# ClashLuke/LocAtE

Measured on AMD Instinct MI355X. Metric: images/sec (G+D step) 64x64 bs=64, higher is better.
Workload: dtype f32 (contractions fp32-faithful on the matrix cores: 2 x scaled fp16 operand pieces / 3 MFMAs per slice where the operand's largest magnitude comes with it, else 3 x bf16 pieces / 6 MFMAs; fp32 accumulate); 1 GPU; LocAtE G+D step, 64x64 RGB, batch 64 per GPU (the fp32 variant - the reference's own precision - of BASELINE.json configs[1]: 64x64 RGB bs 64), self/feature attention at 16x16 and 64x64, random-init weights; global_batch=64, image_size=64, parallelism=dp1, launch=hipGraph replay, G-step generator pass on a second stream

## Files before the change

### include/locate_hip.h

```cpp
#ifndef LOCATE_HIP_H
#define LOCATE_HIP_H
#include <stddef.h>
#include <stdint.h>
#ifdef __cplusplus
extern "C" {
#endif

const char* locate_last_error(void);
int locate_abi_version(void);
int locate_device_info(char* arch_name, int name_len, int* cu_count, int* wave_size);

int locate_roottanh_fwd(const float* x, float* y, int64_t n, void* absmax , void* stream);
int locate_absmax_words(void);
int locate_roottanh_bwd(const float* x, const float* gy, float* gx, int64_t n, int accumulate, void* absmax, void* stream);
int locate_absmax(const float* x, int64_t n, void* absmax, void* stream);
int locate_act_cat_rows_fwd(const float* latent, const float* pre, float* out, int rows, int z, int w, void* stream);
int locate_act_rows_bwd(const float* pre, const float* g, int64_t g_row_stride, const float* g_add, float* gpre, int rows, int w,
                        void* stream);
int locate_add3(const float* a, int64_t a_bs, const float* b, int64_t b_bs, const float* c, int64_t c_bs, float* out, int batch,
                int64_t per, void* stream);
int locate_tanh_fwd(const float* x, float* y, int64_t n, void* stream);
int locate_tanh_bwd(const float* y, const float* gy, float* gx, int64_t n, void* stream);

size_t locate_norm_stats_workspace_bytes(void);
int locate_norm_stats(const float* x, int64_t n, float* stats, void* workspace, void* stream);
int locate_norm_fwd(const float* x, const float* scale, int scale_per_sample, const float* bias, float* out, int with_act,
                    float* stats_out, int B, int C, int hw, int groups, void* workspace, const double* pre_partial,
                    void* absmax , void* stream);
size_t locate_norm_bwd_workspace_bytes(int B, int C);
int locate_norm_bwd(const float* x, const float* g, const float* stats, const float* scale, int scale_per_sample,
                    const float* bias, int with_act, float* dx, float* dscale, float* dbias, int B, int C, int hw, int groups,
                    void* workspace, int accumulate_dx, void* stream);
size_t locate_norm_bwd_fused_workspace_bytes(int B, int C);
size_t locate_norm_bwd_fused_plane_offset(void);
int locate_norm_bwd_fused(const float* x, const float* g, const float* stats, const float* scale, int scale_per_sample,
                          const float* bias, int with_act, float* dx, float* dscale_sample, int B, int C, int hw, int groups,
                          void* workspace, int accumulate_dx, void* stream);
int locate_norm_bwd_fused_partials(int B, int C);
int locate_norm_bwd_planes(const float* x, const float* g, const float* stats, const float* scale, int scale_per_sample,
                           const float* bias, int with_act, float* dscale_sample, int B, int C, int hw, int groups,
                           void* workspace, void* stream);
int locate_fin_norm_channels(const void* records, int n, void* stream);
size_t locate_channel_sum_workspace_bytes(int B, int C, int hw);
int locate_channel_sum(const float* g, float* out, int B, int C, int hw, int64_t batch_stride, void* workspace, void* stream);

int locate_gate_fwd(const float* x, const float* a, int a_per_plane, const float* gamma, float* out, int64_t planes, int hw,
                    void* stream);
int locate_gate_fwd_stats(const float* x, const float* a, int a_per_plane, const float* gamma, float* out, int64_t planes,
                          int hw, int groups, double* stats_partial, void* stream);
size_t locate_gate_bwd_workspace_bytes(int64_t planes);
int locate_gate_bwd_partials(int64_t planes, int hw);
int locate_gate_bwd(const float* x, const float* a, int a_per_plane, const float* gamma, const float* g, float* dx, float* da,
                    float* dgamma, int64_t planes, int hw, void* workspace, int accumulate_dx,
                    void* da_absmax , void* stream);
enum { LOCATE_GATE_TERM_NONE = 0, LOCATE_GATE_TERM_NORM = 1, LOCATE_GATE_TERM_ROOTTANH = 2 };
typedef struct {
    int32_t kind, with_act, per_sample, has_share;
    const float* go;
    const float* stats;
    const float* scale;
    const float* bias;
    const double* partial;
    int32_t npartial, B, C, groups;
} LocateGateTerm;
int locate_gate_bwd_term(const float* x, const float* a, int a_per_plane, const float* gamma, const float* g, float* dx, float* da,
                         float* dgamma, int64_t planes, int hw, void* workspace, int accumulate_dx, void* da_absmax,
                         LocateGateTerm term, void* stream);

int locate_softmax_fwd(const float* x, float* y, int64_t rows, int n, void* stream);
int locate_softmax_bwd(const float* y, const float* gy, float* gx, int64_t rows, int n, void* stream);

int locate_upsample2x_fwd(const float* x, float* y, int64_t planes, int H, int W, void* stream);
int locate_upsample2x_bwd(const float* gy, float* gx, int64_t planes, int H, int W, void* stream);
int locate_pool2_upsample2x_fwd(const float* x, float* y, int64_t planes, int H, int W, void* stream);
int locate_pool2_upsample2x_bwd(const float* gy, float* gx, int64_t planes, int H, int W, int accumulate, void* stream);
int locate_avgpool2_fwd(const float* x, float* y, int64_t planes, int H, int W, void* stream);
int locate_avgpool2_bwd(const float* gy, float* gx, int64_t planes, int H, int W, int accumulate, void* stream);
int locate_feature_pool_fwd(const float* x, float* y, int64_t n_out, int r, void* stream);
int locate_feature_pool_bwd(const float* gy, float* gx, int64_t n_out, int r, int accumulate, void* stream);
int locate_copy_channels(const float* src, float* dst, int B, int C, int hw, int64_t src_batch_stride,
                         int64_t dst_batch_stride, int accumulate, void* stream);

size_t locate_sn_workspace_bytes(int h, int wd);
int locate_sn_power_iter(const float* w, float* u, float* v, float* sigma, float* wv, int h, int wd, void* workspace,
                         void* stream);
size_t locate_sn_table_record_bytes(void);
int locate_sn_power_iter_batched(const void* table, int n_layers, int max_h, int max_wd, void* stream);
int locate_sn_weight_bwd(const double* inner_partial, int n_partial, const float* u, const float* v, const float* sigma,
                         const float* wv, float* gw, float* du, float* dsigma_out, int h, int wd, void* stream);
size_t locate_sn_group_workspace_bytes(void);
int locate_sn_weight_bwd_grouped(const float* gy, int64_t gy_bs, const float* y, int64_t y_bs, const float* bias, int groups,
                                 int Bg, int M, int plane, const float* sigma_tab, int sigma_stride, const float* u,
                                 const float* v, const float* wv, int64_t wv_stride, float* gw, float* du,
                                 float* dsigma_total_out, int h, int wd, void* workspace, void* stream);
int locate_sn_dv_batched(const void* table, int n_layers, int max_h, int max_wd, void* stream);

size_t locate_conv_panel_bytes(const int* geom, int adjoint);
int locate_conv_pack_panel(const int* geom, int adjoint, const float* w, float* panel, void* stream);
size_t locate_conv_pack_job_bytes(void);
int locate_conv_pack_job(const int* geom, int adjoint, const float* w, float* panel, int block_start, void* job_out,
                         int* blocks_out, int direct, const void* weight_absmax);
int locate_conv_pack_panels(const void* jobs, int n_jobs, int total_blocks, int any_f16, int passes, void* stream);
int locate_conv_pack_job_is_direct(const void* job);
int locate_conv_pack_job_is_window(const void* job);
int locate_conv_win_ok(const int* geom, int adjoint_fmt, int64_t x_bs, const void* x);
size_t locate_conv_win_workspace_bytes(const int* geom, int adjoint_fmt);
size_t locate_conv_fwd_workspace_bytes(const int* geom);
size_t locate_conv_counter_bytes(void);
int locate_conv_fwd(const int* geom, const float* x, int64_t x_bs, const float* panel, const float* scale,
                    int scale_group_batch, int scale_stride, const float* bias, float* y, int64_t y_bs, void* workspace,
                    void* counters, int precision, const void* x_absmax, const void* act_epilogue, void* stream);
size_t locate_conv_dgrad_workspace_bytes(const int* geom);
int locate_conv_dgrad(const int* geom, const float* gy, int64_t gy_bs, const float* panel, const float* scale,
                      int scale_group_batch, int scale_stride, const float* bias, float* gx, int64_t gx_bs, void* workspace,
                      void* counters, int precision, const void* gy_absmax, const void* act_epilogue, void* stream);
size_t locate_conv_wgrad_workspace_bytes(const int* geom);
int locate_conv_wgrad_partials(const int* geom);
int locate_conv_wgrad(const int* geom, const float* x, int64_t x_bs, const float* gy, int64_t gy_bs, float* gw,
                      const float* w_ref, const float* inv_scale, int scale_group_batch, int scale_stride,
                      double* inner_partial, void* workspace, int precision, const void* x_absmax, const void* gy_absmax,
                      void* deferred_reduce, void* stream);
int locate_conv_wgrad_group_partials(const int* geom, int groups);
size_t locate_conv_wgrad_group_workspace_bytes(const int* geom, int groups);
size_t locate_slab_reduce_record_bytes(void);
int locate_slab_reduce_max(void);
int locate_slab_reduce_record_blocks(const void* record);
int locate_slab_reduce_batch(const void* records, int n, void* stream);

size_t locate_wgrad_batch_record_bytes(void);
int locate_wgrad_batch_max(void);
int locate_wgrad_batch_record(const int* geom, const float* x, int64_t x_bs, const float* gy, int64_t gy_bs, float* gw,
                              const float* w_ref, const float* inv_scale, int scale_group_batch, int scale_stride,
                              double* inner_partial, void* record);
int locate_wgrad_batch(const void* records, int n, void* stream);

int locate_dwconv_fwd(const int* geom, const float* x, int64_t x_bs, const float* w, const float* scale, int scale_group_batch,
                      int scale_stride, float* y, int64_t y_bs, void* stream);
int locate_dwconv_dgrad(const int* geom, const float* gy, int64_t gy_bs, const float* w, const float* scale,
                        int scale_group_batch, int scale_stride, float* gx, int64_t gx_bs, void* stream);
size_t locate_dwconv_wgrad_workspace_bytes(const int* geom);
int locate_dwconv_wgrad_partials(const int* geom);
int locate_dwconv_wgrad(const int* geom, const float* big, int64_t big_bs, const float* small, int64_t small_bs, float* gw,
                        const float* w_ref, const float* inv_scale, int scale_group_batch, int scale_stride,
                        double* inner_partial, void* workspace, void* stream);
int locate_groupdot_fwd(const float* x, int64_t x_bs, const float* w, const float* scale, int scale_group_batch,
                        int scale_stride, float* y, int B, int G, int L, void* stream);
int locate_groupdot_dgrad(const float* gy, const float* w, const float* scale, int scale_group_batch, int scale_stride,
                          float* gx, int64_t gx_bs, int B, int G, int L, void* stream);
int locate_groupdot_wgrad_partials(int G, int L);
int locate_groupdot_wgrad(const float* x, int64_t x_bs, const float* gy, float* gw, const float* w_ref, const float* inv_scale,
                          int scale_group_batch, int scale_stride, double* inner_partial, int B, int G, int L, void* stream);

size_t locate_fin_record_bytes(void);
int locate_fin_sn_dot_partials(int Bg, int M, int plane);
int locate_fin_sn_dots(const void* records, int n, void* stream);
int locate_fin_sn_rank1(const void* records, int n, void* stream);
int locate_fin_sums(const void* records, int n, void* stream);
int locate_fin_channel_slices(int B, int C, int hw);
int locate_fin_channel_sums(const void* records, int n, void* stream);

size_t locate_multi_copy_record_bytes(void);
int locate_multi_copy_chunk_elems(void);
int locate_multi_copy(const void* tensors, const void* chunks, int n_chunks, int direction, float scale, void* stream);

size_t locate_nadam_tensor_record_bytes(void);
int locate_nadam_chunk_elems(void);
int locate_nadam_step(const void* tensors, void* coef, const void* chunks, int n_tensors, int n_chunks, double lr, double beta1,
                      double beta2, double eps, double schedule_decay, double weight_decay, void* stream);

size_t locate_average_record_bytes(void);
int locate_average_chunk_elems(void);
int locate_average_update(const void* tensors, const void* chunks, int n_tensors, int n_chunks, void* stream);

size_t locate_stats_tensor_record_bytes(void);
size_t locate_stats_record_bytes(void);
int locate_stats_chunk_elems(void);
int locate_stats_max_blocks(void);
size_t locate_stats_workspace_bytes(int n_chunks);
int locate_stats_reduce(const void* tensors, const void* chunks, int n_tensors, int n_chunks, void* records, void* summary,
                        void* workspace, void* stream);

size_t locate_guard_tensor_record_bytes(void);
size_t locate_guard_verdict_bytes(void);
int locate_guard_chunk_elems(void);
int locate_guard_max_blocks(void);
size_t locate_guard_workspace_bytes(int n_chunks);
int locate_guarded_nadam_step(const void* grads, const void* grad_chunks, int n_grads, int n_grad_chunks, void* workspace, void* verdict,
                              double max_norm, int skip_nonfinite, const void* tensors, void* coef, const void* chunks, int n_tensors,
                              int n_chunks, double lr, double beta1, double beta2, double eps, double schedule_decay, double weight_decay,
                              void* stream);

size_t locate_snapshot_record_bytes(void);
size_t locate_snapshot_commit_bytes(void);
int locate_snapshot_chunk_elems(void);
int locate_snapshot_take(const void* records, const void* chunks, int n_tensors, int n_chunks, void* slot0, void* slot1, void* commit,
                         long long iteration, void* stream);
int locate_snapshot_restore(const void* records, const void* chunks, int n_tensors, int n_chunks, const void* slot, void* stream);

size_t locate_digest_record_bytes(void);
int locate_digest_chunk_elems(void);
int locate_digest(const void* records, const void* chunks, const void* first, int n_tensors, int n_chunks, void* partials, void* out,
                  void* stream);

size_t locate_dyn_tensor_record_bytes(void);
size_t locate_dyn_record_bytes(void);
int locate_dyn_chunk_elems(void);
int locate_dyn_max_blocks(void);
size_t locate_dyn_workspace_bytes(int n_chunks);
int locate_dyn_pass(const void* tensors, const void* chunks, int n_tensors, int n_chunks, int mode, void* records, void* workspace,
                    void* stream);

int locate_formats_count(void);
const char* locate_formats_name(int i);
int locate_formats_max_views(void);
size_t locate_formats_view_record_bytes(void);
size_t locate_formats_base_record_bytes(void);
size_t locate_formats_format_record_bytes(void);
size_t locate_formats_workspace_bytes(const void* host_views, int n_views);
int locate_formats_audit(const void* host_views, int n_views, const int* row_slots, void* rows, void* workspace, void* stream);

int locate_d_loss(const float* d_true, const float* d_fake, const float* d_aug, int B, float gamma, float* losses,
                  float* g_true, float* g_fake, float* g_aug, void* stream);
int locate_g_loss(const float* d_fake, int B, float* loss, float* g_fake, void* stream);

size_t locate_input_param_record_bytes(void);
int locate_input_mean_blocks(int H, int W);
size_t locate_input_workspace_bytes(int n, int H, int W);
int locate_input_transform(const void* store, int N, int H, int W, const int32_t* idx, const void* params, int n, int n_first,
                           const int32_t* coef, int side_lo, int side_hi, int ktaps, const float* lut, int S, float* out_first,
                           float* out_rest, void* workspace, void* stream);

size_t locate_image_range_workspace_bytes(void);
int locate_image_range(const float* x, int64_t n_elems, float* range, void* workspace, void* stream);
int locate_image_grid(const float* x, int n, int S, int nrow, int padding, float pad_value, const float* range, float divisor,
                      float* grid_f32, uint8_t* grid_u8, void* stream);

int locate_pyr_down(const float* x, int planes, int S, float* out, void* stream);
int locate_pyr_residual(const float* x, const float* coarse, int planes, int S, float* out, void* stream);
size_t locate_swd_stats_workspace_bytes(void);
int locate_swd_stats(const float* level, int N, int S, const int32_t* pos, int P, float* stats, void* workspace, void* stream);
int locate_swd_project(const float* level, int N, int S, const int32_t* pos, int P, const float* dirs, int D, const float* stats,
                       float* proj, void* stream);
size_t locate_swd_distance_workspace_bytes(void);
int locate_swd_distance(const float* a, const float* b, int64_t count, float* out, void* workspace, void* stream);

int locate_nn_row_bytes(int S);
int locate_nn_encode(const float* x, int n, int S, int8_t* codes, int64_t* norms, int32_t* nonfinite, void* stream);
size_t locate_nn_search_workspace_bytes(int Q, int N, int k);
int locate_nn_search(const int8_t* qcodes, const int64_t* qnorms, const int32_t* qflags, int Q, const int8_t* rcodes, const int64_t* rnorms,
                     const int32_t* rflags, int N, int row_bytes, const int32_t* skip, int k, int64_t* d2, int32_t* index, void* workspace,
                     void* stream);

size_t locate_nn_within_workspace_bytes(int Q, int N, int want_covered);
int locate_nn_within(const int8_t* qcodes, const int64_t* qnorms, const int32_t* qflags, int Q, const int8_t* rcodes, const int64_t* rnorms,
                     const int32_t* rflags, int N, int row_bytes, const int64_t* radius2, const int32_t* skip, int32_t* hits, int32_t* covered,
                     void* workspace, void* stream);

size_t locate_nn_group_sums_workspace_bytes(int M, int K, int row_bytes);
int locate_nn_group_sums(const int8_t* codes, int N, int row_bytes, const int32_t* order, int M, const int32_t* starts, int K,
                         int32_t* sums, void* workspace, void* stream);
int locate_nn_centroids(const int32_t* sums, const int32_t* starts, int K, int M, int row_bytes, const int8_t* previous,
                        int8_t* codes, int64_t* norms, int32_t* moved, void* stream);

size_t locate_spectrum_workspace_bytes(int planes, int S);
int locate_spectrum_planes(const float* x, int planes, int S, const float* cos_table, const float* sin_table, const int32_t* slot,
                           const int32_t* start, int R, double* spectra, void* workspace, void* stream);
size_t locate_spectrum_summary_workspace_bytes(int planes);
int locate_spectrum_summary(const double* spectra, int n, int channels, int R, const double* count, double* sums, int32_t* nonfinite,
                            void* workspace, void* stream);

size_t locate_msssim_workspace_bytes(int pairs, int S);
int locate_msssim_pairs(const int8_t* a, const int32_t* aflags, const int8_t* b, const int32_t* bflags, int pairs, int row_bytes, int S,
                        const double* taps, double* out, void* workspace, void* stream);

#ifdef __cplusplus
}
#endif
#endif
```

### locate_amd/_lib.py

```python
import ctypes
import os

import torch

_HERE = os.path.dirname(os.path.abspath(__file__))
LIB_PATH = os.path.join(_HERE, "csrc", "liblocate_hip_dbg.so" if os.environ.get("LOCATE_HIP_DEBUG_LIBRARY") == "1"
                        else "liblocate_hip.so")

c_p = ctypes.c_void_p
c_i = ctypes.c_int
c_i64 = ctypes.c_int64
c_f = ctypes.c_float
c_d = ctypes.c_double
c_sz = ctypes.c_size_t
c_ip = ctypes.POINTER(ctypes.c_int)


class GateTerm(ctypes.Structure):
    NONE, NORM, ROOTTANH = 0, 1, 2
    _fields_ = [("kind", ctypes.c_int32), ("with_act", ctypes.c_int32), ("per_sample", ctypes.c_int32), ("has_share", ctypes.c_int32),
                ("go", c_p), ("stats", c_p), ("scale", c_p), ("bias", c_p), ("partial", c_p),
                ("npartial", ctypes.c_int32), ("B", ctypes.c_int32), ("C", ctypes.c_int32), ("groups", ctypes.c_int32)]


PROTOTYPES = {
    "locate_last_error": (ctypes.c_char_p, []),
    "locate_abi_version": (c_i, []),
    "locate_device_info": (c_i, [ctypes.c_char_p, c_i, c_ip, c_ip]),
    "locate_roottanh_fwd": (c_i, [c_p, c_p, c_i64, c_p, c_p]),
    "locate_roottanh_bwd": (c_i, [c_p, c_p, c_p, c_i64, c_i, c_p, c_p]),
    "locate_act_cat_rows_fwd": (c_i, [c_p, c_p, c_p, c_i, c_i, c_i, c_p]),
    "locate_act_rows_bwd": (c_i, [c_p, c_p, c_i64, c_p, c_p, c_i, c_i, c_p]),
    "locate_add3": (c_i, [c_p, c_i64, c_p, c_i64, c_p, c_i64, c_p, c_i, c_i64, c_p]),
    "locate_absmax_words": (c_i, []),
    "locate_wgrad_batch_record_bytes": (c_sz, []),
    "locate_wgrad_batch_max": (c_i, []),
    "locate_wgrad_batch_record": (c_i, [c_ip, c_p, c_i64, c_p, c_i64, c_p, c_p, c_p, c_i, c_i, c_p, c_p]),
    "locate_wgrad_batch": (c_i, [c_p, c_i, c_p]),
    "locate_absmax": (c_i, [c_p, c_i64, c_p, c_p]),
    "locate_tanh_fwd": (c_i, [c_p, c_p, c_i64, c_p]),
    "locate_tanh_bwd": (c_i, [c_p, c_p, c_p, c_i64, c_p]),
    "locate_norm_stats_workspace_bytes": (c_sz, []),
    "locate_norm_stats": (c_i, [c_p, c_i64, c_p, c_p, c_p]),
    "locate_norm_bwd_workspace_bytes": (c_sz, [c_i, c_i]),
    "locate_norm_fwd": (c_i, [c_p, c_p, c_i, c_p, c_p, c_i, c_p, c_i, c_i, c_i, c_i, c_p, c_p, c_p, c_p]),
    "locate_norm_bwd": (c_i, [c_p, c_p, c_p, c_p, c_i, c_p, c_i, c_p, c_p, c_p, c_i, c_i, c_i, c_i, c_p, c_i, c_p]),
    "locate_norm_bwd_fused_workspace_bytes": (c_sz, [c_i, c_i]),
    "locate_norm_bwd_fused_plane_offset": (c_sz, []),
    "locate_norm_bwd_fused": (c_i, [c_p, c_p, c_p, c_p, c_i, c_p, c_i, c_p, c_p, c_i, c_i, c_i, c_i, c_p, c_i, c_p]),
    "locate_norm_bwd_fused_partials": (c_i, [c_i, c_i]),
    "locate_norm_bwd_planes": (c_i, [c_p, c_p, c_p, c_p, c_i, c_p, c_i, c_p, c_i, c_i, c_i, c_i, c_p, c_p]),
    "locate_fin_norm_channels": (c_i, [c_p, c_i, c_p]),
    "locate_channel_sum_workspace_bytes": (c_sz, [c_i, c_i, c_i]),
    "locate_channel_sum": (c_i, [c_p, c_p, c_i, c_i, c_i, c_i64, c_p, c_p]),
    "locate_gate_fwd": (c_i, [c_p, c_p, c_i, c_p, c_p, c_i64, c_i, c_p]),
    "locate_gate_fwd_stats": (c_i, [c_p, c_p, c_i, c_p, c_p, c_i64, c_i, c_i, c_p, c_p]),
    "locate_gate_bwd_workspace_bytes": (c_sz, [c_i64]),
    "locate_gate_bwd": (c_i, [c_p, c_p, c_i, c_p, c_p, c_p, c_p, c_p, c_i64, c_i, c_p, c_i, c_p, c_p]),
    "locate_gate_bwd_term": (c_i, [c_p, c_p, c_i, c_p, c_p, c_p, c_p, c_p, c_i64, c_i, c_p, c_i, c_p, GateTerm, c_p]),
    "locate_softmax_fwd": (c_i, [c_p, c_p, c_i64, c_i, c_p]),
    "locate_softmax_bwd": (c_i, [c_p, c_p, c_p, c_i64, c_i, c_p]),
    "locate_upsample2x_fwd": (c_i, [c_p, c_p, c_i64, c_i, c_i, c_p]),
    "locate_upsample2x_bwd": (c_i, [c_p, c_p, c_i64, c_i, c_i, c_p]),
    "locate_pool2_upsample2x_fwd": (c_i, [c_p, c_p, c_i64, c_i, c_i, c_p]),
    "locate_pool2_upsample2x_bwd": (c_i, [c_p, c_p, c_i64, c_i, c_i, c_i, c_p]),
    "locate_avgpool2_fwd": (c_i, [c_p, c_p, c_i64, c_i, c_i, c_p]),
    "locate_avgpool2_bwd": (c_i, [c_p, c_p, c_i64, c_i, c_i, c_i, c_p]),
    "locate_feature_pool_fwd": (c_i, [c_p, c_p, c_i64, c_i, c_p]),
    "locate_feature_pool_bwd": (c_i, [c_p, c_p, c_i64, c_i, c_i, c_p]),
    "locate_copy_channels": (c_i, [c_p, c_p, c_i, c_i, c_i, c_i64, c_i64, c_i, c_p]),
    "locate_sn_workspace_bytes": (c_sz, [c_i, c_i]),
    "locate_sn_power_iter": (c_i, [c_p, c_p, c_p, c_p, c_p, c_i, c_i, c_p, c_p]),
    "locate_sn_table_record_bytes": (c_sz, []),
    "locate_sn_power_iter_batched": (c_i, [c_p, c_i, c_i, c_i, c_p]),
    "locate_sn_weight_bwd": (c_i, [c_p, c_i, c_p, c_p, c_p, c_p, c_p, c_p, c_p, c_i, c_i, c_p]),
    "locate_sn_group_workspace_bytes": (c_sz, []),
    "locate_sn_weight_bwd_grouped": (c_i, [c_p, c_i64, c_p, c_i64, c_p, c_i, c_i, c_i, c_i, c_p, c_i, c_p, c_p, c_p, c_i64, c_p,
                                           c_p, c_p, c_i, c_i, c_p, c_p]),
    "locate_sn_dv_batched": (c_i, [c_p, c_i, c_i, c_i, c_p]),
    "locate_conv_panel_bytes": (c_sz, [c_ip, c_i]),
    "locate_conv_pack_panel": (c_i, [c_ip, c_i, c_p, c_p, c_p]),
    "locate_conv_pack_job_bytes": (c_sz, []),
    "locate_conv_pack_job": (c_i, [c_ip, c_i, c_p, c_p, c_i, c_p, c_ip, c_i, c_p]),
    "locate_conv_pack_panels": (c_i, [c_p, c_i, c_i, c_i, c_i, c_p]),
    "locate_conv_pack_job_is_direct": (c_i, [c_p]),
    "locate_conv_pack_job_is_window": (c_i, [c_p]),
    "locate_conv_win_ok": (c_i, [c_ip, c_i, c_i64, c_p]),
    "locate_conv_win_workspace_bytes": (c_sz, [c_ip, c_i]),
    "locate_conv_fwd_workspace_bytes": (c_sz, [c_ip]),
    "locate_conv_counter_bytes": (c_sz, []),
    "locate_conv_fwd": (c_i, [c_ip, c_p, c_i64, c_p, c_p, c_i, c_i, c_p, c_p, c_i64, c_p, c_p, c_i, c_p, c_p, c_p]),
    "locate_conv_dgrad_workspace_bytes": (c_sz, [c_ip]),
    "locate_conv_dgrad": (c_i, [c_ip, c_p, c_i64, c_p, c_p, c_i, c_i, c_p, c_p, c_i64, c_p, c_p, c_i, c_p, c_p, c_p]),
    "locate_conv_wgrad_workspace_bytes": (c_sz, [c_ip]),
    "locate_conv_wgrad_partials": (c_i, [c_ip]),
    "locate_conv_wgrad": (c_i, [c_ip, c_p, c_i64, c_p, c_i64, c_p, c_p, c_p, c_i, c_i, c_p, c_p, c_i, c_p, c_p, c_p, c_p]),
    "locate_conv_wgrad_group_partials": (c_i, [c_ip, c_i]),
    "locate_conv_wgrad_group_workspace_bytes": (c_sz, [c_ip, c_i]),
    "locate_slab_reduce_record_bytes": (c_sz, []),
    "locate_slab_reduce_max": (c_i, []),
    "locate_slab_reduce_record_blocks": (c_i, [c_p]),
    "locate_slab_reduce_batch": (c_i, [c_p, c_i, c_p]),
    "locate_dwconv_fwd": (c_i, [c_ip, c_p, c_i64, c_p, c_p, c_i, c_i, c_p, c_i64, c_p]),
    "locate_dwconv_dgrad": (c_i, [c_ip, c_p, c_i64, c_p, c_p, c_i, c_i, c_p, c_i64, c_p]),
    "locate_dwconv_wgrad_workspace_bytes": (c_sz, [c_ip]),
    "locate_dwconv_wgrad_partials": (c_i, [c_ip]),
    "locate_dwconv_wgrad": (c_i, [c_ip, c_p, c_i64, c_p, c_i64, c_p, c_p, c_p, c_i, c_i, c_p, c_p, c_p]),
    "locate_groupdot_fwd": (c_i, [c_p, c_i64, c_p, c_p, c_i, c_i, c_p, c_i, c_i, c_i, c_p]),
    "locate_groupdot_dgrad": (c_i, [c_p, c_p, c_p, c_i, c_i, c_p, c_i64, c_i, c_i, c_i, c_p]),
    "locate_groupdot_wgrad_partials": (c_i, [c_i, c_i]),
    "locate_groupdot_wgrad": (c_i, [c_p, c_i64, c_p, c_p, c_p, c_p, c_i, c_i, c_p, c_i, c_i, c_i, c_p]),
    "locate_fin_record_bytes": (c_sz, []),
    "locate_fin_sn_dot_partials": (c_i, [c_i, c_i, c_i]),
    "locate_fin_sn_dots": (c_i, [c_p, c_i, c_p]),
    "locate_fin_sn_rank1": (c_i, [c_p, c_i, c_p]),
    "locate_fin_sums": (c_i, [c_p, c_i, c_p]),
    "locate_fin_channel_slices": (c_i, [c_i, c_i, c_i]),
    "locate_fin_channel_sums": (c_i, [c_p, c_i, c_p]),
    "locate_gate_bwd_partials": (c_i, [c_i64, c_i]),
    "locate_multi_copy_record_bytes": (c_sz, []),
    "locate_multi_copy_chunk_elems": (c_i, []),
    "locate_multi_copy": (c_i, [c_p, c_p, c_i, c_i, c_f, c_p]),
    "locate_nadam_tensor_record_bytes": (c_sz, []),
    "locate_nadam_chunk_elems": (c_i, []),
    "locate_nadam_step": (c_i, [c_p, c_p, c_p, c_i, c_i, c_d, c_d, c_d, c_d, c_d, c_d, c_p]),
    "locate_average_record_bytes": (c_sz, []),
    "locate_average_chunk_elems": (c_i, []),
    "locate_average_update": (c_i, [c_p, c_p, c_i, c_i, c_p]),
    "locate_stats_tensor_record_bytes": (c_sz, []),
    "locate_stats_record_bytes": (c_sz, []),
    "locate_stats_chunk_elems": (c_i, []),
    "locate_stats_max_blocks": (c_i, []),
    "locate_stats_workspace_bytes": (c_sz, [c_i]),
    "locate_stats_reduce": (c_i, [c_p, c_p, c_i, c_i, c_p, c_p, c_p, c_p]),
    "locate_guard_tensor_record_bytes": (c_sz, []),
    "locate_guard_verdict_bytes": (c_sz, []),
    "locate_guard_chunk_elems": (c_i, []),
    "locate_guard_max_blocks": (c_i, []),
    "locate_guard_workspace_bytes": (c_sz, [c_i]),
    "locate_guarded_nadam_step": (c_i, [c_p, c_p, c_i, c_i, c_p, c_p, c_d, c_i, c_p, c_p, c_p, c_i, c_i, c_d, c_d, c_d, c_d, c_d, c_d, c_p]),
    "locate_snapshot_record_bytes": (c_sz, []),
    "locate_snapshot_commit_bytes": (c_sz, []),
    "locate_snapshot_chunk_elems": (c_i, []),
    "locate_snapshot_take": (c_i, [c_p, c_p, c_i, c_i, c_p, c_p, c_p, c_i64, c_p]),
    "locate_snapshot_restore": (c_i, [c_p, c_p, c_i, c_i, c_p, c_p]),
    "locate_digest_record_bytes": (c_sz, []),
    "locate_digest_chunk_elems": (c_i, []),
    "locate_digest": (c_i, [c_p, c_p, c_p, c_i, c_i, c_p, c_p, c_p]),
    "locate_dyn_tensor_record_bytes": (c_sz, []),
    "locate_dyn_record_bytes": (c_sz, []),
    "locate_dyn_chunk_elems": (c_i, []),
    "locate_dyn_max_blocks": (c_i, []),
    "locate_dyn_workspace_bytes": (c_sz, [c_i]),
    "locate_dyn_pass": (c_i, [c_p, c_p, c_i, c_i, c_i, c_p, c_p, c_p]),
    "locate_formats_count": (c_i, []),
    "locate_formats_name": (ctypes.c_char_p, [c_i]),
    "locate_formats_max_views": (c_i, []),
    "locate_formats_view_record_bytes": (c_sz, []),
    "locate_formats_base_record_bytes": (c_sz, []),
    "locate_formats_format_record_bytes": (c_sz, []),
    "locate_formats_workspace_bytes": (c_sz, [c_p, c_i]),
    "locate_formats_audit": (c_i, [c_p, c_i, c_p, c_p, c_p, c_p]),
    "locate_d_loss": (c_i, [c_p, c_p, c_p, c_i, c_f, c_p, c_p, c_p, c_p, c_p]),
    "locate_g_loss": (c_i, [c_p, c_i, c_p, c_p, c_p]),
    "locate_input_param_record_bytes": (c_sz, []),
    "locate_input_mean_blocks": (c_i, [c_i, c_i]),
    "locate_input_workspace_bytes": (c_sz, [c_i, c_i, c_i]),
    "locate_input_transform": (c_i, [c_p, c_i, c_i, c_i, c_p, c_p, c_i, c_i, c_p, c_i, c_i, c_i, c_p, c_i, c_p, c_p, c_p, c_p]),
    "locate_image_range_workspace_bytes": (c_sz, []),
    "locate_image_range": (c_i, [c_p, c_i64, c_p, c_p, c_p]),
    "locate_image_grid": (c_i, [c_p, c_i, c_i, c_i, c_i, c_f, c_p, c_f, c_p, c_p, c_p]),
    "locate_pyr_down": (c_i, [c_p, c_i, c_i, c_p, c_p]),
    "locate_pyr_residual": (c_i, [c_p, c_p, c_i, c_i, c_p, c_p]),
    "locate_swd_stats_workspace_bytes": (c_sz, []),
    "locate_swd_stats": (c_i, [c_p, c_i, c_i, c_p, c_i, c_p, c_p, c_p]),
    "locate_swd_project": (c_i, [c_p, c_i, c_i, c_p, c_i, c_p, c_i, c_p, c_p, c_p]),
    "locate_swd_distance_workspace_bytes": (c_sz, []),
    "locate_swd_distance": (c_i, [c_p, c_p, c_i64, c_p, c_p, c_p]),
    "locate_spectrum_workspace_bytes": (c_sz, [c_i, c_i]),
    "locate_spectrum_planes": (c_i, [c_p, c_i, c_i, c_p, c_p, c_p, c_p, c_i, c_p, c_p, c_p]),
    "locate_spectrum_summary_workspace_bytes": (c_sz, [c_i]),
    "locate_spectrum_summary": (c_i, [c_p, c_i, c_i, c_i, c_p, c_p, c_p, c_p, c_p]),
    "locate_msssim_workspace_bytes": (c_sz, [c_i, c_i]),
    "locate_msssim_pairs": (c_i, [c_p, c_p, c_p, c_p, c_i, c_i, c_i, c_p, c_p, c_p, c_p]),
    "locate_nn_row_bytes": (c_i, [c_i]),
    "locate_nn_encode": (c_i, [c_p, c_i, c_i, c_p, c_p, c_p, c_p]),
    "locate_nn_search_workspace_bytes": (c_sz, [c_i, c_i, c_i]),
    "locate_nn_search": (c_i, [c_p, c_p, c_p, c_i, c_p, c_p, c_p, c_i, c_i, c_p, c_i, c_p, c_p, c_p, c_p]),
    "locate_nn_within_workspace_bytes": (c_sz, [c_i, c_i, c_i]),
    "locate_nn_within": (c_i, [c_p, c_p, c_p, c_i, c_p, c_p, c_p, c_i, c_i, c_p, c_p, c_p, c_p, c_p, c_p]),
    "locate_nn_group_sums_workspace_bytes": (c_sz, [c_i, c_i, c_i]),
    "locate_nn_group_sums": (c_i, [c_p, c_i, c_i, c_p, c_i, c_p, c_i, c_p, c_p, c_p]),
    "locate_nn_centroids": (c_i, [c_p, c_p, c_i, c_i, c_i, c_p, c_p, c_p, c_p, c_p]),
}


class LocateError(RuntimeError):
    pass


EXPECTED_ABI = 21


_lib = None


def lib():
    global _lib
    if _lib is None:
        if not os.path.exists(LIB_PATH):
            raise LocateError("%s is missing: run `python -m locate_amd.build` (hipcc, gfx950). "
                              "There is no CPU fallback for the MI355X kernels." % LIB_PATH)
        handle = ctypes.CDLL(LIB_PATH)
        for name, (res, args) in PROTOTYPES.items():
            fn = getattr(handle, name)
            fn.restype = res
            fn.argtypes = args
        got = handle.locate_abi_version()
        if got != EXPECTED_ABI:
            raise LocateError("%s reports ABI version %d, this package binds version %d: rebuild it (`python -m locate_amd.build`)"
                              % (LIB_PATH, got, EXPECTED_ABI))
        _lib = handle
    return _lib


def check(status, what=""):
    if status != 0:
        msg = lib().locate_last_error()
        raise LocateError("%s failed (status %d): %s" % (what, status, msg.decode() if msg else "?"))


def require_gpu():
    if not torch.cuda.is_available():
        raise LocateError("no HIP device: locate_amd computes only on MI355X (gfx950); there is no CPU path")
    name = ctypes.create_string_buffer(64)
    cu, wave = ctypes.c_int(0), ctypes.c_int(0)
    check(lib().locate_device_info(name, 64, ctypes.byref(cu), ctypes.byref(wave)), "locate_device_info")
    arch = name.value.decode()
    if not arch.startswith("gfx950"):
        raise LocateError("device architecture %r: the kernels are built for gfx950 only" % arch)
    return arch, cu.value, wave.value
```

### locate_amd/csrc/elementwise.hip

```cpp
#include "common.h"
#include "normterm.h"

template <int OP>
__global__ void __launch_bounds__(256) unary_fwd_kernel(const float* __restrict__ x, float* __restrict__ y, int64_t n,
                                                        unsigned* __restrict__ absmax) {
    __shared__ float amax_scratch[16];
    float am = 0.0f;
    const int64_t n4 = n >> 2;
    const int64_t stride = (int64_t)gridDim.x * blockDim.x;
    const float4* x4 = reinterpret_cast<const float4*>(x);
    float4* y4 = reinterpret_cast<float4*>(y);
    for (int64_t i = (int64_t)blockIdx.x * blockDim.x + threadIdx.x; i < n4; i += stride) {
        float4 v = x4[i], o;
        if (OP == 0) {
            o.x = roottanh_f(v.x); o.y = roottanh_f(v.y); o.z = roottanh_f(v.z); o.w = roottanh_f(v.w);
        } else {
            o.x = tanhf(v.x); o.y = tanhf(v.y); o.z = tanhf(v.z); o.w = tanhf(v.w);
        }
        y4[i] = o;
        am = fmaxf(fmaxf(am, fmaxf(fabsf(o.x), fabsf(o.y))), fmaxf(fabsf(o.z), fabsf(o.w)));
    }
    for (int64_t i = (n4 << 2) + (int64_t)blockIdx.x * blockDim.x + threadIdx.x; i < n; i += stride) {
        const float o = OP == 0 ? roottanh_f(x[i]) : tanhf(x[i]);
        y[i] = o;
        am = fmaxf(am, fabsf(o));
    }
    if (absmax) absmax_publish(am, amax_scratch, absmax);
}

template <int OP>
__global__ void __launch_bounds__(256) unary_bwd_kernel(const float* __restrict__ a, const float* __restrict__ g,
                                                        float* __restrict__ gx, int64_t n, int accumulate,
                                                        unsigned* __restrict__ absmax) {
    __shared__ float amax_scratch[16];
    float am = 0.0f;
    const int64_t n4 = n >> 2;
    const int64_t stride = (int64_t)gridDim.x * blockDim.x;
    const float4* a4 = reinterpret_cast<const float4*>(a);
    const float4* g4 = reinterpret_cast<const float4*>(g);
    float4* o4 = reinterpret_cast<float4*>(gx);
    for (int64_t i = (int64_t)blockIdx.x * blockDim.x + threadIdx.x; i < n4; i += stride) {
        float4 v = a4[i], w = g4[i], o;
        if (OP == 0) {
            o.x = roottanh_grad_f(v.x, w.x); o.y = roottanh_grad_f(v.y, w.y);
            o.z = roottanh_grad_f(v.z, w.z); o.w = roottanh_grad_f(v.w, w.w);
        } else {
            o.x = w.x * (1.0f - v.x * v.x); o.y = w.y * (1.0f - v.y * v.y);
            o.z = w.z * (1.0f - v.z * v.z); o.w = w.w * (1.0f - v.w * v.w);
        }
        if (accumulate) {
            const float4 c = o4[i];
            o.x += c.x; o.y += c.y; o.z += c.z; o.w += c.w;
        }
        o4[i] = o;
        am = fmaxf(fmaxf(am, fmaxf(fabsf(o.x), fabsf(o.y))), fmaxf(fabsf(o.z), fabsf(o.w)));
    }
    for (int64_t i = (n4 << 2) + (int64_t)blockIdx.x * blockDim.x + threadIdx.x; i < n; i += stride) {
        float o = OP == 0 ? roottanh_grad_f(a[i], g[i]) : g[i] * (1.0f - a[i] * a[i]);
        o = accumulate ? gx[i] + o : o;
        gx[i] = o;
        am = fmaxf(am, fabsf(o));
    }
    if (absmax) absmax_publish(am, amax_scratch, absmax);
}

static bool aligned16(const void* p) { return (reinterpret_cast<uintptr_t>(p) & 15) == 0; }

LOCATE_API int locate_roottanh_fwd(const float* x, float* y, int64_t n, void* absmax, void* stream) {
    LOCATE_REQUIRE(n >= 0 && aligned16(x) && aligned16(y), "locate_roottanh_fwd: bad size or unaligned pointer");
    if (n == 0) return LOCATE_OK;
    unary_fwd_kernel<0><<<stream_grid(n, 1024), 256, 0, as_stream(stream)>>>(x, y, n, static_cast<unsigned*>(absmax));
    LOCATE_LAUNCH_CHECK("locate_roottanh_fwd");
    return LOCATE_OK;
}

LOCATE_API int locate_roottanh_bwd(const float* x, const float* gy, float* gx, int64_t n, int accumulate, void* absmax, void* stream) {
    LOCATE_REQUIRE(n >= 0 && aligned16(x) && aligned16(gy) && aligned16(gx), "locate_roottanh_bwd: bad size or unaligned pointer");
    if (n == 0) return LOCATE_OK;
    unary_bwd_kernel<0><<<stream_grid(n, 1024), 256, 0, as_stream(stream)>>>(x, gy, gx, n, accumulate, static_cast<unsigned*>(absmax));
    LOCATE_LAUNCH_CHECK("locate_roottanh_bwd");
    return LOCATE_OK;
}

__global__ void __launch_bounds__(256) act_cat_rows_kernel(const float* __restrict__ latent, const float* __restrict__ pre,
                                                           float* __restrict__ out, int rows, int z, int w) {
    const int total = rows * (z + w);
    for (int i = blockIdx.x * blockDim.x + threadIdx.x; i < total; i += gridDim.x * blockDim.x) {
        const int r = i / (z + w), c = i - r * (z + w);
        out[i] = c < z ? latent[r * z + c] : roottanh_f(pre[r * w + (c - z)]);
    }
}

__global__ void __launch_bounds__(256) act_rows_bwd_kernel(const float* __restrict__ pre, const float* __restrict__ g, int g_rs,
                                                           const float* __restrict__ g_add, float* __restrict__ gpre, int rows, int w) {
    const int total = rows * w;
    for (int i = blockIdx.x * blockDim.x + threadIdx.x; i < total; i += gridDim.x * blockDim.x) {
        const int r = i / w, j = i - r * w;
        const float v = roottanh_grad_f(pre[i], g[(int64_t)r * g_rs + j]);
        gpre[i] = g_add ? __fadd_rn(g_add[i], v) : v;
    }
}

LOCATE_API int locate_act_cat_rows_fwd(const float* latent, const float* pre, float* out, int rows, int z, int w, void* stream) {
    LOCATE_REQUIRE(latent && pre && out && rows > 0 && z >= 0 && w > 0 && (int64_t)rows * (z + w) < (1ll << 31), "locate_act_cat_rows_fwd: bad arguments");
    act_cat_rows_kernel<<<stream_grid((int64_t)rows * (z + w), 256), 256, 0, as_stream(stream)>>>(latent, pre, out, rows, z, w);
    LOCATE_LAUNCH_CHECK("locate_act_cat_rows_fwd");
    return LOCATE_OK;
}

LOCATE_API int locate_act_rows_bwd(const float* pre, const float* g, int64_t g_row_stride, const float* g_add, float* gpre, int rows,
                                   int w, void* stream) {
    LOCATE_REQUIRE(pre && g && gpre && rows > 0 && w > 0 && g_row_stride >= w && g_row_stride < (1ll << 31), "locate_act_rows_bwd: bad arguments");
    act_rows_bwd_kernel<<<stream_grid((int64_t)rows * w, 256), 256, 0, as_stream(stream)>>>(pre, g, (int)g_row_stride, g_add, gpre, rows, w);
    LOCATE_LAUNCH_CHECK("locate_act_rows_bwd");
    return LOCATE_OK;
}

template <bool VEC>
__global__ void __launch_bounds__(256) add3_kernel(const float* __restrict__ a, long long a_bs, const float* __restrict__ b, long long b_bs,
                                                   const float* __restrict__ c, long long c_bs, float* __restrict__ out, unsigned per,
                                                   long long total) {
    const DivU32 dv(per);
    const long long stride = (long long)gridDim.x * blockDim.x;
    for (long long i = (long long)blockIdx.x * blockDim.x + threadIdx.x; i < total; i += stride) {
        unsigned q, r;
        dv.divmod((unsigned)i, q, r);
        if constexpr (VEC) {
            const float4 x = *reinterpret_cast<const float4*>(a + q * a_bs + 4ll * r);
            const float4 y = *reinterpret_cast<const float4*>(b + q * b_bs + 4ll * r);
            const float4 z = *reinterpret_cast<const float4*>(c + q * c_bs + 4ll * r);
            float4 o;
            o.x = __fadd_rn(__fadd_rn(x.x, y.x), z.x); o.y = __fadd_rn(__fadd_rn(x.y, y.y), z.y);
            o.z = __fadd_rn(__fadd_rn(x.z, y.z), z.z); o.w = __fadd_rn(__fadd_rn(x.w, y.w), z.w);
            *reinterpret_cast<float4*>(out + 4ll * i) = o;
        } else {
            out[i] = __fadd_rn(__fadd_rn(a[q * a_bs + r], b[q * b_bs + r]), c[q * c_bs + r]);
        }
    }
}

LOCATE_API int locate_add3(const float* a, int64_t a_bs, const float* b, int64_t b_bs, const float* c, int64_t c_bs, float* out, int batch,
                           int64_t per, void* stream) {
    LOCATE_REQUIRE(a && b && c && out && batch > 0 && per > 0 && a_bs >= per && b_bs >= per && c_bs >= per &&
                   (int64_t)batch * per < (1ll << 32), "locate_add3: bad arguments");
    const bool vec = (per & 3) == 0 && ((a_bs | b_bs | c_bs) & 3) == 0 && aligned16(a) && aligned16(b) && aligned16(c) && aligned16(out);
    if (vec) {
        const int64_t total = (int64_t)batch * (per / 4);
        add3_kernel<true><<<stream_grid(total, 2048), 256, 0, as_stream(stream)>>>(a, a_bs, b, b_bs, c, c_bs, out, (unsigned)(per / 4), total);
    } else {
        const int64_t total = (int64_t)batch * per;
        add3_kernel<false><<<stream_grid(total, 2048), 256, 0, as_stream(stream)>>>(a, a_bs, b, b_bs, c, c_bs, out, (unsigned)per, total);
    }
    LOCATE_LAUNCH_CHECK("locate_add3");
    return LOCATE_OK;
}

LOCATE_API int locate_absmax_words(void) { return AMAX_WORDS; }

__global__ void __launch_bounds__(256) absmax_kernel(const float* __restrict__ x, int64_t n, unsigned* __restrict__ slot) {
    __shared__ float scratch[16];
    float m = 0.0f;
    const int64_t stride = (int64_t)gridDim.x * blockDim.x;
    for (int64_t i = (int64_t)blockIdx.x * blockDim.x + threadIdx.x; i < n; i += stride) m = fmaxf(m, fabsf(x[i]));
    absmax_publish(m, scratch, slot);
}

LOCATE_API int locate_absmax(const float* x, int64_t n, void* slot, void* stream) {
    LOCATE_REQUIRE(x && slot && n > 0, "locate_absmax: bad arguments");
    absmax_kernel<<<stream_grid(n, 2048), 256, 0, as_stream(stream)>>>(x, n, static_cast<unsigned*>(slot));
    LOCATE_LAUNCH_CHECK("locate_absmax");
    return LOCATE_OK;
}

LOCATE_API int locate_tanh_fwd(const float* x, float* y, int64_t n, void* stream) {
    LOCATE_REQUIRE(n >= 0 && aligned16(x) && aligned16(y), "locate_tanh_fwd: bad size or unaligned pointer");
    if (n == 0) return LOCATE_OK;
    unary_fwd_kernel<1><<<stream_grid(n, 1024), 256, 0, as_stream(stream)>>>(x, y, n, nullptr);
    LOCATE_LAUNCH_CHECK("locate_tanh_fwd");
    return LOCATE_OK;
}

LOCATE_API int locate_tanh_bwd(const float* y, const float* gy, float* gx, int64_t n, void* stream) {
    LOCATE_REQUIRE(n >= 0 && aligned16(y) && aligned16(gy) && aligned16(gx), "locate_tanh_bwd: bad size or unaligned pointer");
    if (n == 0) return LOCATE_OK;
    unary_bwd_kernel<1><<<stream_grid(n, 1024), 256, 0, as_stream(stream)>>>(y, gy, gx, n, 0, nullptr);
    LOCATE_LAUNCH_CHECK("locate_tanh_bwd");
    return LOCATE_OK;
}

__global__ void __launch_bounds__(256) gate_fwd_kernel(const float* __restrict__ x, const float* __restrict__ a,
                                                       const float* __restrict__ gamma, float* __restrict__ out,
                                                       int64_t n, int hw, int a_per_plane) {
    const float gm = gamma[0];
    const int64_t stride = (int64_t)gridDim.x * blockDim.x;
    if (!a_per_plane && (n & 3) == 0) {
        const float4* x4 = reinterpret_cast<const float4*>(x);
        const float4* a4 = reinterpret_cast<const float4*>(a);
        float4* o4 = reinterpret_cast<float4*>(out);
        for (int64_t i = (int64_t)blockIdx.x * blockDim.x + threadIdx.x; i < (n >> 2); i += stride) {
            float4 xv = x4[i], av = a4[i], o;
            o.x = fmaf(gm, av.x, 1.0f) * xv.x; o.y = fmaf(gm, av.y, 1.0f) * xv.y;
            o.z = fmaf(gm, av.z, 1.0f) * xv.z; o.w = fmaf(gm, av.w, 1.0f) * xv.w;
            o4[i] = o;
        }
        return;
    }
    if (a_per_plane && (hw & 3) == 0) {
        const float4* x4 = reinterpret_cast<const float4*>(x);
        float4* o4 = reinterpret_cast<float4*>(out);
        const unsigned hw4 = (unsigned)(hw >> 2);
        for (int64_t i = (int64_t)blockIdx.x * blockDim.x + threadIdx.x; i < (n >> 2); i += stride) {
            const float m = fmaf(gm, a[(unsigned)i / hw4], 1.0f);
            const float4 xv = x4[i];
            o4[i] = make_float4(m * xv.x, m * xv.y, m * xv.z, m * xv.w);
        }
        return;
    }
    const DivU32 dhw((unsigned)hw);
    for (int64_t i = (int64_t)blockIdx.x * blockDim.x + threadIdx.x; i < n; i += stride) {
        const float av = a_per_plane ? a[dhw.div((unsigned)i)] : a[i];
        out[i] = fmaf(gm, av, 1.0f) * x[i];
    }
}

__global__ void __launch_bounds__(256) gate_fwd_stats_kernel(const float* __restrict__ x, const float* __restrict__ a,
                                                             const float* __restrict__ gamma, float* __restrict__ out,
                                                             int64_t n_group, int hw, int a_per_plane,
                                                             double* __restrict__ partial) {
    __shared__ double scratch[16];
    const float gm = gamma[0];
    const int64_t g0 = (int64_t)blockIdx.y * n_group;
    x += g0; out += g0;
    if (!a_per_plane) a += g0;
    partial += (int64_t)blockIdx.y * 2 * gridDim.x;
    const int64_t stride = (int64_t)gridDim.x * blockDim.x;
    double s = 0.0, q = 0.0;
    if (!a_per_plane && (n_group & 3) == 0) {
        const float4* x4 = reinterpret_cast<const float4*>(x);
        const float4* a4 = reinterpret_cast<const float4*>(a);
        float4* o4 = reinterpret_cast<float4*>(out);
        for (int64_t i = (int64_t)blockIdx.x * blockDim.x + threadIdx.x; i < (n_group >> 2); i += stride) {
            float4 xv = x4[i], av = a4[i], o;
            o.x = fmaf(gm, av.x, 1.0f) * xv.x; o.y = fmaf(gm, av.y, 1.0f) * xv.y;
            o.z = fmaf(gm, av.z, 1.0f) * xv.z; o.w = fmaf(gm, av.w, 1.0f) * xv.w;
            o4[i] = o;
            const double a_ = o.x, b_ = o.y, c_ = o.z, d_ = o.w;
            s += (a_ + b_) + (c_ + d_);
            q += (a_ * a_ + b_ * b_) + (c_ * c_ + d_ * d_);
        }
    } else if (a_per_plane && (hw & 3) == 0 && (n_group & 3) == 0 && n_group < (1ll << 33)) {
        const float4* x4 = reinterpret_cast<const float4*>(x);
        float4* o4 = reinterpret_cast<float4*>(out);
        const unsigned hw4 = (unsigned)(hw >> 2);
        const float* ap = a + g0 / hw;
        for (int64_t i = (int64_t)blockIdx.x * blockDim.x + threadIdx.x; i < (n_group >> 2); i += stride) {
            const float m = fmaf(gm, ap[(unsigned)i / hw4], 1.0f);
            const float4 xv = x4[i];
            float4 o;
            o.x = m * xv.x; o.y = m * xv.y; o.z = m * xv.z; o.w = m * xv.w;
            o4[i] = o;
            const double a_ = o.x, b_ = o.y, c_ = o.z, d_ = o.w;
            s += (a_ + b_) + (c_ + d_);
            q += (a_ * a_ + b_ * b_) + (c_ * c_ + d_ * d_);
        }
    } else {
        const DivU32 dhw((unsigned)hw);
        for (int64_t i = (int64_t)blockIdx.x * blockDim.x + threadIdx.x; i < n_group; i += stride) {
            const float av = a_per_plane ? a[dhw.div((unsigned)(g0 + i))] : a[i];
            const float o = fmaf(gm, av, 1.0f) * x[i];
            out[i] = o;
            s += (double)o;
            q += (double)o * (double)o;
        }
    }
    s = block_sum<double>(s, scratch);
    q = block_sum<double>(q, scratch);
    if (threadIdx.x == 0) {
        partial[2 * blockIdx.x] = s;
        partial[2 * blockIdx.x + 1] = q;
    }
}

__device__ __noinline__ float gate_plane_da_nonfinite(const float* __restrict__ x, const float* __restrict__ g, int hw, float gm) {
    float s = 0.0f;
    for (int i = 0; i < hw; ++i) s += (x[i] * g[i]) * gm;
    return s;
}
__device__ __forceinline__ bool gate_gamma_finite(float gm) { return fabsf(gm) <= 3.402823466e38f; }

constexpr bool gate_term_is_norm(int term) { return term == GATE_TERM_NORM || term == GATE_TERM_NORM_ACT; }

struct GateTermPlane { float mu, inv_s, y, b, k, m; };

template <int TERM>
__device__ __forceinline__ GateTermPlane gate_term_plane(const LocateGateTerm& t, const float (*tc)[2], unsigned p, unsigned planes_g) {
    GateTermPlane tp = {0.0f, 1.0f, 0.0f, 0.0f, 0.0f, 0.0f};
    if constexpr (gate_term_is_norm(TERM)) {
        const unsigned grp = p / planes_g, c = p % (unsigned)t.C;
        tp.mu = t.stats[2 * grp];
        tp.inv_s = 1.0f / t.stats[2 * grp + 1];
        tp.y = t.scale[t.per_sample ? p : c];
        tp.b = TERM == GATE_TERM_NORM_ACT ? t.bias[c] : 0.0f;
        tp.m = tc[grp][0];
        tp.k = tc[grp][1];
    }
    return tp;
}

__device__ __forceinline__ float gate_mul_g_first(float g, float m) {
    float r;
    asm("v_mul_f32 %0, %1, %2" : "=v"(r) : "v"(g), "v"(m));
    return r;
}

template <int TERM>
__device__ __forceinline__ float gate_term_g(const GateTermPlane& tp, float out, float gin, float share, int has_share) {
    if constexpr (TERM == GATE_TERM_ROOTTANH) return roottanh_grad_f(out, gin);
    const float o = norm_dx<TERM == GATE_TERM_NORM_ACT>(out, gin, tp.mu, tp.inv_s, tp.y, tp.b, tp.k, tp.m);
    return has_share ? o + share : o;
}

template <int TERM>
__device__ __forceinline__ void gate_term_consts(const LocateGateTerm& t, int64_t n_group, float (*tc)[2]) {
    if constexpr (gate_term_is_norm(TERM)) {
        const int wid = threadIdx.x >> 6;
        if (wid < t.groups) norm_group_consts(t.partial, t.npartial, wid, t.stats[2 * wid + 1], n_group, (int)(threadIdx.x & 63), tc[wid]);
        __syncthreads();
    }
}

template <int TERM>
__device__ __noinline__ float gate_plane_da_nonfinite_term(const float* __restrict__ x, const float* __restrict__ gs,
                                                           const float* __restrict__ share, int hw, float gm, float ap,
                                                           GateTermPlane tp, int has_share) {
    float s = 0.0f;
    const float mv = fmaf(gm, ap, 1.0f);
    for (int i = 0; i < hw; ++i) {
        const float g = gate_term_g<TERM>(tp, mul_pinned(mv, x[i]), gs[i], has_share ? share[i] : 0.0f, has_share);
        s += (x[i] * g) * gm;
    }
    return s;
}

template <int WPP, int TERM, bool ELEM = false>
__global__ void __launch_bounds__(256) gate_bwd_plane_kernel(const float* __restrict__ x, const float* __restrict__ a,
                                                             const float* __restrict__ gamma, const float* __restrict__ g,
                                                             float* __restrict__ dx, float* __restrict__ da_full,
                                                             float* __restrict__ da_plane, double* __restrict__ block_x2g,
                                                             int64_t planes, int hw, int a_per_plane, int accumulate_dx,
                                                             unsigned* __restrict__ da_absmax, const LocateGateTerm t) {
    __shared__ double wsum[4], px2g[4];
    __shared__ float pxg[4];
    __shared__ float amax_scratch[16];
    __shared__ float tc[NORM_MAX_GROUPS][2];
    float am = 0.0f;
    double wacc = 0.0;
    const float gm = gamma[0];
    const int lane = threadIdx.x & 63, wid = threadIdx.x >> 6;
    const int sub = WPP == 1 ? lane : (int)threadIdx.x;
    const int nsub = WPP == 1 ? 64 : 256;
    const int64_t first = WPP == 1 ? (((int64_t)blockIdx.x * blockDim.x + threadIdx.x) >> 6) : (int64_t)blockIdx.x;
    const int64_t step = WPP == 1 ? (((int64_t)gridDim.x * blockDim.x) >> 6) : (int64_t)gridDim.x;
    const float* __restrict__ gs = gate_term_is_norm(TERM) ? t.go : g;
    constexpr bool elem = ELEM;
    const unsigned planes_g = gate_term_is_norm(TERM) ? (unsigned)((int64_t)t.B * t.C / t.groups) : 1u;
    const int has_share = gate_term_is_norm(TERM) ? t.has_share : 0;
    if constexpr (gate_term_is_norm(TERM)) gate_term_consts<TERM>(t, (int64_t)planes_g * (elem ? 1 : hw), tc);
    bool vec = (hw & 3) == 0 && ((reinterpret_cast<uintptr_t>(x) | reinterpret_cast<uintptr_t>(g) | reinterpret_cast<uintptr_t>(dx) |
                                  (a_per_plane ? 0 : (reinterpret_cast<uintptr_t>(a) | reinterpret_cast<uintptr_t>(da_full)))) & 15) == 0;
    if constexpr (gate_term_is_norm(TERM)) vec = vec && (reinterpret_cast<uintptr_t>(gs) & 15) == 0;
    for (int64_t p = first; p < planes; p += step) {
        const int64_t base = p * hw;
        const float ap = a_per_plane ? a[p] : 0.0f;
        float sxg = 0.0f, sx2g = 0.0f;
        GateTermPlane tp = {0.0f, 1.0f, 0.0f, 0.0f, 0.0f, 0.0f};
        if constexpr (gate_term_is_norm(TERM))
            if (!elem) tp = gate_term_plane<TERM>(t, tc, (unsigned)p, planes_g);
        if (vec) {
            for (int i = sub; i < (hw >> 2); i += nsub) {
                const float4 xv = reinterpret_cast<const float4*>(x + base)[i];
                float4 gv = reinterpret_cast<const float4*>(gs + base)[i];
                float4 av = make_float4(ap, ap, ap, ap);
                if (!a_per_plane) av = reinterpret_cast<const float4*>(a + base)[i];
                if constexpr (TERM != GATE_TERM_NONE) {
                    const float4 ov = make_float4(mul_pinned(fmaf(gm, av.x, 1.0f), xv.x), mul_pinned(fmaf(gm, av.y, 1.0f), xv.y),
                                                  mul_pinned(fmaf(gm, av.z, 1.0f), xv.z), mul_pinned(fmaf(gm, av.w, 1.0f), xv.w));
                    float4 sh = make_float4(0.0f, 0.0f, 0.0f, 0.0f);
                    if (has_share) sh = reinterpret_cast<const float4*>(g + base)[i];
                    if (elem) {
                        const unsigned e = (unsigned)(base + 4 * i);
                        gv.x = gate_term_g<TERM>(gate_term_plane<TERM>(t, tc, e, planes_g), ov.x, gv.x, sh.x, has_share);
                        gv.y = gate_term_g<TERM>(gate_term_plane<TERM>(t, tc, e + 1, planes_g), ov.y, gv.y, sh.y, has_share);
                        gv.z = gate_term_g<TERM>(gate_term_plane<TERM>(t, tc, e + 2, planes_g), ov.z, gv.z, sh.z, has_share);
                        gv.w = gate_term_g<TERM>(gate_term_plane<TERM>(t, tc, e + 3, planes_g), ov.w, gv.w, sh.w, has_share);
                    } else {
                        gv.x = gate_term_g<TERM>(tp, ov.x, gv.x, sh.x, has_share); gv.y = gate_term_g<TERM>(tp, ov.y, gv.y, sh.y, has_share);
                        gv.z = gate_term_g<TERM>(tp, ov.z, gv.z, sh.z, has_share); gv.w = gate_term_g<TERM>(tp, ov.w, gv.w, sh.w, has_share);
                    }
                }
                const float4 xg = make_float4(xv.x * gv.x, xv.y * gv.y, xv.z * gv.z, xv.w * gv.w);
                float4 o = make_float4(fmaf(gm, av.x, 1.0f) * gv.x, fmaf(gm, av.y, 1.0f) * gv.y, fmaf(gm, av.z, 1.0f) * gv.z,
                                       fmaf(gm, av.w, 1.0f) * gv.w);
                if constexpr (TERM != GATE_TERM_NONE)
                    o = make_float4(gate_mul_g_first(gv.x, fmaf(gm, av.x, 1.0f)), gate_mul_g_first(gv.y, fmaf(gm, av.y, 1.0f)),
                                    gate_mul_g_first(gv.z, fmaf(gm, av.z, 1.0f)), gate_mul_g_first(gv.w, fmaf(gm, av.w, 1.0f)));
                if (accumulate_dx) {
                    const float4 old = reinterpret_cast<const float4*>(dx + base)[i];
                    o.x += old.x; o.y += old.y; o.z += old.z; o.w += old.w;
                }
                reinterpret_cast<float4*>(dx + base)[i] = o;
                if (!a_per_plane) {
                    const float4 dav = make_float4(xg.x * gm, xg.y * gm, xg.z * gm, xg.w * gm);
                    reinterpret_cast<float4*>(da_full + base)[i] = dav;
                    am = fmaxf(fmaxf(am, fmaxf(fabsf(dav.x), fabsf(dav.y))), fmaxf(fabsf(dav.z), fabsf(dav.w)));
                }
                sxg += (xg.x + xg.y) + (xg.z + xg.w);
                sx2g += (xg.x * xv.x + xg.y * xv.y) + (xg.z * xv.z + xg.w * xv.w);
            }
        } else {
            for (int i = sub; i < hw; i += nsub) {
                const float xv = x[base + i];
                float gv = gs[base + i];
                const float av = a_per_plane ? ap : a[base + i];
                if constexpr (TERM != GATE_TERM_NONE) {
                    if (elem) tp = gate_term_plane<TERM>(t, tc, (unsigned)(base + i), planes_g);
                    gv = gate_term_g<TERM>(tp, mul_pinned(fmaf(gm, av, 1.0f), xv), gv, has_share ? g[base + i] : 0.0f, has_share);
                }
                const float xg = xv * gv;
                float o = fmaf(gm, av, 1.0f) * gv;
                if constexpr (TERM != GATE_TERM_NONE) o = gate_mul_g_first(gv, fmaf(gm, av, 1.0f));
                dx[base + i] = accumulate_dx ? dx[base + i] + o : o;
                if (!a_per_plane) { da_full[base + i] = xg * gm; am = fmaxf(am, fabsf(xg * gm)); }
                sxg += xg;
                sx2g = fmaf(xg, xv, sx2g);
            }
        }
        sxg = wave_sum(sxg);
        const double s2 = wave_sum_d((double)sx2g);
        if (WPP == 1) {
            wacc += s2;
            if (lane == 0 && a_per_plane) {
                if (gate_gamma_finite(gm)) da_plane[p] = gm * sxg;
                else if constexpr (TERM == GATE_TERM_NONE) da_plane[p] = gate_plane_da_nonfinite(x + base, g + base, hw, gm);
                else da_plane[p] = gate_plane_da_nonfinite_term<TERM>(x + base, gs + base, g + base, hw, gm, ap, tp, has_share);
            }
        } else {
            __syncthreads();
            if (lane == 0) { pxg[wid] = sxg; px2g[wid] = s2; }
            __syncthreads();
            if (threadIdx.x == 0) {
                wacc += (px2g[0] + px2g[1]) + (px2g[2] + px2g[3]);
                if (a_per_plane) {
                    if (gate_gamma_finite(gm)) da_plane[p] = gm * ((pxg[0] + pxg[1]) + (pxg[2] + pxg[3]));
                    else if constexpr (TERM == GATE_TERM_NONE) da_plane[p] = gate_plane_da_nonfinite(x + base, g + base, hw, gm);
                    else da_plane[p] = gate_plane_da_nonfinite_term<TERM>(x + base, gs + base, g + base, hw, gm, ap, tp, has_share);
                }
            }
        }
    }
    if (WPP == 1) {
        if (lane == 0) wsum[wid] = wacc;
        __syncthreads();
        if (threadIdx.x == 0) block_x2g[blockIdx.x] = (wsum[0] + wsum[1]) + (wsum[2] + wsum[3]);
    } else if (threadIdx.x == 0) {
        block_x2g[blockIdx.x] = wacc;
    }
    if (da_absmax && !a_per_plane) absmax_publish(am, amax_scratch, da_absmax);
}

template <int LP, int TERM, bool ELEM = false>
__global__ void __launch_bounds__(256) gate_bwd_small_kernel(const float* __restrict__ x, const float* __restrict__ a,
                                                             const float* __restrict__ gamma, const float* __restrict__ g,
                                                             float* __restrict__ dx, float* __restrict__ da_full,
                                                             float* __restrict__ da_plane, double* __restrict__ block_x2g,
                                                             int64_t planes, int hw, int a_per_plane, int accumulate_dx,
                                                             unsigned* __restrict__ da_absmax, const LocateGateTerm t) {
    __shared__ double wsum[4];
    __shared__ float amax_scratch[16];
    __shared__ float tc[NORM_MAX_GROUPS][2];
    constexpr int PW = 64 / LP;
    float am = 0.0f;
    double wacc = 0.0;
    const float gm = gamma[0];
    const int lane = threadIdx.x & 63, wid = threadIdx.x >> 6;
    const int gid = lane / LP, li = lane % LP;
    const int q4 = hw >> 2;
    const int64_t wave = ((int64_t)blockIdx.x * blockDim.x + threadIdx.x) >> 6;
    const int64_t nwaves = ((int64_t)gridDim.x * blockDim.x) >> 6;
    const float* __restrict__ gs = gate_term_is_norm(TERM) ? t.go : g;
    constexpr bool elem = ELEM;
    const unsigned planes_g = gate_term_is_norm(TERM) ? (unsigned)((int64_t)t.B * t.C / t.groups) : 1u;
    const int has_share = gate_term_is_norm(TERM) ? t.has_share : 0;
    if constexpr (gate_term_is_norm(TERM)) gate_term_consts<TERM>(t, (int64_t)planes_g * (elem ? 1 : hw), tc);
    for (int64_t p0 = wave * PW; p0 < planes; p0 += nwaves * PW) {
        const int64_t p = p0 + gid;
        const bool live = p < planes;
        float sxg = 0.0f, sx2g = 0.0f;
        float ap = 0.0f;
        GateTermPlane tp = {0.0f, 1.0f, 0.0f, 0.0f, 0.0f, 0.0f};
        if (live && li < q4) {
            const int64_t base = p * hw;
            ap = a_per_plane ? a[p] : 0.0f;
            const float4 xv = reinterpret_cast<const float4*>(x + base)[li];
            float4 gv = reinterpret_cast<const float4*>(gs + base)[li];
            float4 av = make_float4(ap, ap, ap, ap);
            if (!a_per_plane) av = reinterpret_cast<const float4*>(a + base)[li];
            if constexpr (TERM != GATE_TERM_NONE) {
                const float4 ov = make_float4(mul_pinned(fmaf(gm, av.x, 1.0f), xv.x), mul_pinned(fmaf(gm, av.y, 1.0f), xv.y),
                                              mul_pinned(fmaf(gm, av.z, 1.0f), xv.z), mul_pinned(fmaf(gm, av.w, 1.0f), xv.w));
                float4 sh = make_float4(0.0f, 0.0f, 0.0f, 0.0f);
                if (has_share) sh = reinterpret_cast<const float4*>(g + base)[li];
                if (elem) {
                    const unsigned e = (unsigned)(base + 4 * li);
                    gv.x = gate_term_g<TERM>(gate_term_plane<TERM>(t, tc, e, planes_g), ov.x, gv.x, sh.x, has_share);
                    gv.y = gate_term_g<TERM>(gate_term_plane<TERM>(t, tc, e + 1, planes_g), ov.y, gv.y, sh.y, has_share);
                    gv.z = gate_term_g<TERM>(gate_term_plane<TERM>(t, tc, e + 2, planes_g), ov.z, gv.z, sh.z, has_share);
                    gv.w = gate_term_g<TERM>(gate_term_plane<TERM>(t, tc, e + 3, planes_g), ov.w, gv.w, sh.w, has_share);
                } else {
                    tp = gate_term_plane<TERM>(t, tc, (unsigned)p, planes_g);
                    gv.x = gate_term_g<TERM>(tp, ov.x, gv.x, sh.x, has_share); gv.y = gate_term_g<TERM>(tp, ov.y, gv.y, sh.y, has_share);
                    gv.z = gate_term_g<TERM>(tp, ov.z, gv.z, sh.z, has_share); gv.w = gate_term_g<TERM>(tp, ov.w, gv.w, sh.w, has_share);
                }
            }
            const float4 xg = make_float4(xv.x * gv.x, xv.y * gv.y, xv.z * gv.z, xv.w * gv.w);
            float4 o = make_float4(fmaf(gm, av.x, 1.0f) * gv.x, fmaf(gm, av.y, 1.0f) * gv.y, fmaf(gm, av.z, 1.0f) * gv.z,
                                   fmaf(gm, av.w, 1.0f) * gv.w);
            if constexpr (TERM != GATE_TERM_NONE)
                o = make_float4(gate_mul_g_first(gv.x, fmaf(gm, av.x, 1.0f)), gate_mul_g_first(gv.y, fmaf(gm, av.y, 1.0f)),
                                gate_mul_g_first(gv.z, fmaf(gm, av.z, 1.0f)), gate_mul_g_first(gv.w, fmaf(gm, av.w, 1.0f)));
            if (accumulate_dx) {
                const float4 old = reinterpret_cast<const float4*>(dx + base)[li];
                o.x += old.x; o.y += old.y; o.z += old.z; o.w += old.w;
            }
            reinterpret_cast<float4*>(dx + base)[li] = o;
            if (!a_per_plane) {
                const float4 dav = make_float4(xg.x * gm, xg.y * gm, xg.z * gm, xg.w * gm);
                reinterpret_cast<float4*>(da_full + base)[li] = dav;
                am = fmaxf(fmaxf(am, fmaxf(fabsf(dav.x), fabsf(dav.y))), fmaxf(fabsf(dav.z), fabsf(dav.w)));
            }
            sxg = (xg.x + xg.y) + (xg.z + xg.w);
            sx2g = (xg.x * xv.x + xg.y * xv.y) + (xg.z * xv.z + xg.w * xv.w);
        }
        double s2 = (double)sx2g;
#pragma unroll
        for (int o = LP / 2; o > 0; o >>= 1) {
            sxg += __shfl_xor(sxg, o, 64);
            s2 += __shfl_xor(s2, o, 64);
        }
        if (live && li == 0) {
            wacc += s2;
            if (a_per_plane) {
                if (gate_gamma_finite(gm)) da_plane[p] = gm * sxg;
                else if constexpr (TERM == GATE_TERM_NONE) da_plane[p] = gate_plane_da_nonfinite(x + p * hw, g + p * hw, hw, gm);
                else da_plane[p] = gate_plane_da_nonfinite_term<TERM>(x + p * hw, gs + p * hw, g + p * hw, hw, gm, ap, tp, has_share);
            }
        }
    }
    wacc = wave_sum_d(wacc);
    if (lane == 0) wsum[wid] = wacc;
    __syncthreads();
    if (threadIdx.x == 0) block_x2g[blockIdx.x] = (wsum[0] + wsum[1]) + (wsum[2] + wsum[3]);
    if (da_absmax && !a_per_plane) absmax_publish(am, amax_scratch, da_absmax);
}

__global__ void __launch_bounds__(256) gate_bwd_final_kernel(const double* __restrict__ block_x2g, float* __restrict__ dgamma,
                                                             int nblocks) {
    __shared__ double scratch[16];
    double acc = 0.0;
    for (int i = threadIdx.x; i < nblocks; i += blockDim.x) acc += block_x2g[i];
    acc = block_sum<double>(acc, scratch);
    if (threadIdx.x == 0) dgamma[0] = (float)acc;
}

LOCATE_API int locate_gate_fwd(const float* x, const float* a, int a_per_plane, const float* gamma, float* out,
                               int64_t planes, int hw, void* stream) {
    LOCATE_REQUIRE(planes >= 0 && hw > 0 && planes * hw < (1ll << 31), "locate_gate_fwd: bad shape");
    const int64_t n = planes * hw;
    if (n == 0) return LOCATE_OK;
    gate_fwd_kernel<<<stream_grid(n, 1024), 256, 0, as_stream(stream)>>>(x, a, gamma, out, n, hw, a_per_plane);
    LOCATE_LAUNCH_CHECK("locate_gate_fwd");
    return LOCATE_OK;
}

LOCATE_API int locate_gate_fwd_stats(const float* x, const float* a, int a_per_plane, const float* gamma, float* out,
                                     int64_t planes, int hw, int groups, double* stats_partial, void* stream) {
    LOCATE_REQUIRE(planes > 0 && hw > 0 && planes * hw < (1ll << 31) && stats_partial, "locate_gate_fwd_stats: bad arguments");
    LOCATE_REQUIRE(groups >= 1 && groups <= 4 && planes % groups == 0, "locate_gate_fwd_stats: bad group count");
    const int64_t n_g = planes / groups * hw;
    LOCATE_REQUIRE(n_g > 1 && (groups == 1 || (n_g & 3) == 0), "locate_gate_fwd_stats: group size must be a multiple of 4");
    int np = stream_grid(n_g, 256 * 16);
    if (np > 512) np = 512;
    gate_fwd_stats_kernel<<<dim3(np, groups), 256, 0, as_stream(stream)>>>(x, a, gamma, out, n_g, hw, a_per_plane, stats_partial);
    LOCATE_LAUNCH_CHECK("locate_gate_fwd_stats");
    return LOCATE_OK;
}

LOCATE_API size_t locate_gate_bwd_workspace_bytes(int64_t planes) { (void)planes; return 4096 * sizeof(double); }

static int64_t gate_bwd_blocks(int64_t planes, int hw) {
    int64_t blocks = hw >= 1024 ? planes : cdiv64(planes, 4);
    return blocks > 4096 ? 4096 : blocks;
}
LOCATE_API int locate_gate_bwd_partials(int64_t planes, int hw) { return (int)gate_bwd_blocks(planes, hw); }

template <int TERM>
static void gate_bwd_launch(const float* x, const float* a, int a_per_plane, const float* gamma, const float* g, float* dx, float* da,
                            double* block_x2g, int64_t planes, int hw, int64_t blocks, int accumulate_dx, void* da_absmax,
                            const LocateGateTerm& t, hipStream_t st) {
    const bool whole_block = hw >= 1024;
    uintptr_t bits = reinterpret_cast<uintptr_t>(x) | reinterpret_cast<uintptr_t>(g) | reinterpret_cast<uintptr_t>(dx) |
                     (a_per_plane ? 0 : (reinterpret_cast<uintptr_t>(a) | reinterpret_cast<uintptr_t>(da)));
    if (gate_term_is_norm(TERM)) bits |= reinterpret_cast<uintptr_t>(t.go);
    const bool vec = (hw & 3) == 0 && (bits & 15) == 0;
    if constexpr (gate_term_is_norm(TERM)) {
        if (planes != (int64_t)t.B * t.C) {
            if (vec)
                gate_bwd_small_kernel<16, TERM, true><<<(int)blocks, 256, 0, st>>>(x, a, gamma, g, dx, da, nullptr, block_x2g, planes, hw, 0,
                                                                                  accumulate_dx, static_cast<unsigned*>(da_absmax), t);
            else
                gate_bwd_plane_kernel<1, TERM, true><<<(int)blocks, 256, 0, st>>>(x, a, gamma, g, dx, da, nullptr, block_x2g, planes, hw, 0,
                                                                                 accumulate_dx, static_cast<unsigned*>(da_absmax), t);
            return;
        }
    }
#define GATE_SMALL(LPV) gate_bwd_small_kernel<LPV, TERM><<<(int)blocks, 256, 0, st>>>(x, a, gamma, g, dx, a_per_plane ? nullptr : da, \
        a_per_plane ? da : nullptr, block_x2g, planes, hw, a_per_plane, accumulate_dx, static_cast<unsigned*>(da_absmax), t)
    if (vec && hw <= 128) {
        const int q4 = hw >> 2;
        if (q4 <= 1) GATE_SMALL(1);
        else if (q4 <= 2) GATE_SMALL(2);
        else if (q4 <= 4) GATE_SMALL(4);
        else if (q4 <= 8) GATE_SMALL(8);
        else if (q4 <= 16) GATE_SMALL(16);
        else GATE_SMALL(32);
    } else if (whole_block)
        gate_bwd_plane_kernel<4, TERM><<<(int)blocks, 256, 0, st>>>(x, a, gamma, g, dx, a_per_plane ? nullptr : da,
                                                                   a_per_plane ? da : nullptr, block_x2g, planes, hw,
                                                                   a_per_plane, accumulate_dx, static_cast<unsigned*>(da_absmax), t);
    else
        gate_bwd_plane_kernel<1, TERM><<<(int)blocks, 256, 0, st>>>(x, a, gamma, g, dx, a_per_plane ? nullptr : da,
                                                                   a_per_plane ? da : nullptr, block_x2g, planes, hw,
                                                                   a_per_plane, accumulate_dx, static_cast<unsigned*>(da_absmax), t);
#undef GATE_SMALL
}

LOCATE_API int locate_gate_bwd_term(const float* x, const float* a, int a_per_plane, const float* gamma, const float* g,
                                    float* dx, float* da, float* dgamma, int64_t planes, int hw, void* workspace,
                                    int accumulate_dx, void* da_absmax, LocateGateTerm term, void* stream) {
    LOCATE_REQUIRE(planes > 0 && hw > 0 && workspace, "locate_gate_bwd: bad shape or missing workspace");
    LOCATE_REQUIRE(term.kind == GATE_TERM_NONE || term.kind == GATE_TERM_NORM || term.kind == GATE_TERM_ROOTTANH,
                   "locate_gate_bwd_term: unknown term %d", term.kind);
    if (term.kind == GATE_TERM_NORM) {
        LOCATE_REQUIRE(term.go && term.stats && term.scale && term.partial && term.npartial > 0 && (!term.with_act || term.bias),
                       "locate_gate_bwd_term: the norm term needs go, stats, scale, the plane pass's partials (and the bias with_act)");
        LOCATE_REQUIRE(term.groups >= 1 && term.groups <= NORM_MAX_GROUPS && term.B > 0 && term.C > 0 && term.B % term.groups == 0 &&
                       (int64_t)term.B * term.C == planes && planes * hw < (1ll << 31), "locate_gate_bwd_term: the norm's B x C must be the gate's planes");
        LOCATE_REQUIRE(!term.has_share || g, "locate_gate_bwd_term: has_share needs the share in g");
    } else {
        LOCATE_REQUIRE(g, "locate_gate_bwd_term: missing gradient");
    }
    double* block_x2g = static_cast<double*>(workspace);
    const int64_t blocks = gate_bwd_blocks(planes, hw);
    if (hw == 1 && (planes & 63) == 0) {
        if (a_per_plane) { a_per_plane = 0; da_absmax = nullptr; }
        planes >>= 6; hw = 64;
    }
    hipStream_t st = as_stream(stream);
    if (term.kind == GATE_TERM_NONE)
        gate_bwd_launch<GATE_TERM_NONE>(x, a, a_per_plane, gamma, g, dx, da, block_x2g, planes, hw, blocks, accumulate_dx, da_absmax, term, st);
    else if (term.kind == GATE_TERM_ROOTTANH)
        gate_bwd_launch<GATE_TERM_ROOTTANH>(x, a, a_per_plane, gamma, g, dx, da, block_x2g, planes, hw, blocks, accumulate_dx, da_absmax, term, st);
    else if (term.with_act)
        gate_bwd_launch<GATE_TERM_NORM_ACT>(x, a, a_per_plane, gamma, g, dx, da, block_x2g, planes, hw, blocks, accumulate_dx, da_absmax, term, st);
    else
        gate_bwd_launch<GATE_TERM_NORM>(x, a, a_per_plane, gamma, g, dx, da, block_x2g, planes, hw, blocks, accumulate_dx, da_absmax, term, st);
    LOCATE_LAUNCH_CHECK("locate_gate_bwd(plane)");
    if (!dgamma) return LOCATE_OK;
    gate_bwd_final_kernel<<<1, 256, 0, st>>>(block_x2g, dgamma, (int)blocks);
    LOCATE_LAUNCH_CHECK("locate_gate_bwd(final)");
    return LOCATE_OK;
}

LOCATE_API int locate_gate_bwd(const float* x, const float* a, int a_per_plane, const float* gamma, const float* g,
                               float* dx, float* da, float* dgamma, int64_t planes, int hw, void* workspace,
                               int accumulate_dx, void* da_absmax, void* stream) {
    LocateGateTerm none = {};
    return locate_gate_bwd_term(x, a, a_per_plane, gamma, g, dx, da, dgamma, planes, hw, workspace, accumulate_dx, da_absmax, none, stream);
}

__global__ void __launch_bounds__(256) copy_planes_kernel(const float* __restrict__ src, float* __restrict__ dst, int B,
                                                          int64_t chw, int64_t src_bs, int64_t dst_bs, int accumulate) {
    const int b = blockIdx.y;
    const float* s = src + (int64_t)b * src_bs;
    float* d = dst + (int64_t)b * dst_bs;
    const int64_t stride = (int64_t)gridDim.x * blockDim.x;
    const bool vec = ((chw | src_bs | dst_bs) & 3) == 0 && ((reinterpret_cast<uintptr_t>(src) | reinterpret_cast<uintptr_t>(dst)) & 15) == 0;
    if (vec) {
        const float4* s4 = reinterpret_cast<const float4*>(s);
        float4* d4 = reinterpret_cast<float4*>(d);
        for (int64_t i = (int64_t)blockIdx.x * blockDim.x + threadIdx.x; i < (chw >> 2); i += stride) {
            float4 v = s4[i];
            if (accumulate) { const float4 o = d4[i]; v.x += o.x; v.y += o.y; v.z += o.z; v.w += o.w; }
            d4[i] = v;
        }
        return;
    }
    for (int64_t i = (int64_t)blockIdx.x * blockDim.x + threadIdx.x; i < chw; i += stride) d[i] = accumulate ? d[i] + s[i] : s[i];
}

LOCATE_API int locate_copy_channels(const float* src, float* dst, int B, int C, int hw, int64_t src_batch_stride,
                                    int64_t dst_batch_stride, int accumulate, void* stream) {
    LOCATE_REQUIRE(B >= 0 && C >= 0 && hw >= 0, "locate_copy_channels: bad shape");
    const int64_t chw = (int64_t)C * hw;
    if ((int64_t)B * chw == 0) return LOCATE_OK;
    LOCATE_REQUIRE(src_batch_stride >= chw && dst_batch_stride >= chw, "locate_copy_channels: batch stride smaller than slice");
    int gx = stream_grid(chw, 1024);
    if (gx > 64) gx = 64;
    copy_planes_kernel<<<dim3(gx, B), 256, 0, as_stream(stream)>>>(src, dst, B, chw, src_batch_stride, dst_batch_stride,
                                                                   accumulate);
    LOCATE_LAUNCH_CHECK("locate_copy_channels");
    return LOCATE_OK;
}
```

### locate_amd/csrc/normterm.h

```cpp
#pragma once
#include "common.h"

#define NORM_MAX_GROUPS 4

struct LocateGateTerm {
    int32_t kind;
    int32_t with_act;
    int32_t per_sample;
    int32_t has_share;
    const float* go;
    const float* stats;
    const float* scale;
    const float* bias;
    const double* partial;
    int32_t npartial, B, C, groups;
};
enum { GATE_TERM_NONE = 0, GATE_TERM_NORM = 1, GATE_TERM_ROOTTANH = 2, GATE_TERM_NORM_ACT = 3  };

#ifdef __HIPCC__
__device__ __forceinline__ float mul_pinned(float a, float b) {
    float r = a * b;
    asm("" : "+v"(r));
    return r;
}

template <bool ACT>
__device__ __forceinline__ float norm_go(float xv, float gv, float mu, float inv_s, float y, float b) {
    if (!ACT) return gv;
    const float o = fmaf(xv - mu, y * inv_s, b);
    return roottanh_grad_f(o, gv);
}

__device__ __forceinline__ void norm_group_consts(const double* __restrict__ partial, int npartial, int grp, float s, int64_t n,
                                                  int lane, float* consts) {
    double a = 0.0, b2 = 0.0;
    for (int i = lane; i < npartial; i += 64) {
        a += partial[((int64_t)i * NORM_MAX_GROUPS + grp) * 2];
        b2 += partial[((int64_t)i * NORM_MAX_GROUPS + grp) * 2 + 1];
    }
    a = wave_sum_d(a);
    b2 = wave_sum_d(b2);
    if (lane == 0) {
        const double sd = (double)s, nn = (double)n;
        consts[0] = (float)(a / sd / nn);
        consts[1] = (float)(-b2 / (sd * sd) / ((nn - 1.0) * sd));
    }
}

template <bool ACT>
__device__ __forceinline__ float norm_dx(float xv, float gv, float mu, float inv_s, float y, float b, float k, float m) {
    const float go = norm_go<ACT>(xv, gv, mu, inv_s, y, b);
    return fmaf(y * inv_s, go, fmaf(k, xv - mu, -m));
}
#endif
```

### locate_amd/csrc/runtime.hip

```cpp
#include "common.h"
#include <stdarg.h>
#include <stdio.h>

static thread_local char g_last_error[512] = "";

void locate_set_error(const char* fmt, ...) {
    va_list ap;
    va_start(ap, fmt);
    vsnprintf(g_last_error, sizeof(g_last_error), fmt, ap);
    va_end(ap);
}

LOCATE_API const char* locate_last_error(void) { return g_last_error; }

LOCATE_API int locate_abi_version(void) { return 21; }

LOCATE_API int locate_device_info(char* arch_name, int name_len, int* cu_count, int* wave_size) {
    int dev = 0;
    hipDeviceProp_t prop;
    if (hipGetDevice(&dev) != hipSuccess || hipGetDeviceProperties(&prop, dev) != hipSuccess) {
        locate_set_error("locate_device_info: no HIP device");
        return LOCATE_ERR_LAUNCH;
    }
    if (arch_name && name_len > 0) snprintf(arch_name, name_len, "%s", prop.gcnArchName);
    if (cu_count) *cu_count = prop.multiProcessorCount;
    if (wave_size) *wave_size = prop.warpSize;
    return LOCATE_OK;
}
```

### locate_amd/ops.py

```python
import ctypes
import os

import torch

from ._lib import GateTerm, check, lib

_IntArr12 = ctypes.c_int * 12


class _ActEpilogue(ctypes.Structure):
    _fields_ = [("act_out", ctypes.c_void_p), ("act_bs", ctypes.c_int64), ("lat", ctypes.c_void_p), ("lat_bs", ctypes.c_int64),
                ("lat_z", ctypes.c_int32), ("pad", ctypes.c_int32), ("mul_pre", ctypes.c_void_p), ("mul_bs", ctypes.c_int64),
                ("out_absmax", ctypes.c_void_p)]


ACT_LINKS = [os.environ.get("LOCATE_ACT_LINKS", "1") != "0"]
ACT_LINK_MAX_NUMEL = [int(os.environ.get("LOCATE_ACT_LINK_MAX", str(1 << 22)))]


GATE_FOLD = [os.environ.get("LOCATE_GATE_FOLD", "1") != "0"]
GATE_FOLD_ACT_MIN_NUMEL = [int(os.environ.get("LOCATE_GATE_FOLD_ACT_MIN", str(1 << 22)))]


class ActLink:
    __slots__ = ("pre", "premultiplied")

    def __init__(self):
        self.pre = None
        self.premultiplied = False


def _stream():
    return torch.cuda.current_stream().cuda_stream


def _chk(t, what):
    if not (t.is_cuda and t.dtype == torch.float32):
        raise TypeError("%s must be a float32 CUDA/HIP tensor (the kernels run on MI355X only), got %s on %s"
                        % (what, t.dtype, t.device))
    return t


def _c(t, what="tensor"):
    _chk(t, what)
    return t if t.is_contiguous() else t.contiguous()


def _ws(nbytes, device):
    return torch.empty(max(int(nbytes), 16), dtype=torch.uint8, device=device)


def _p(t):
    return t.data_ptr() if t is not None else None


class _AmaxArena:
    SLOTS = 32
    STEP_SLOTS = 160

    def __init__(self):
        self.block, self.used, self.cap = None, 0, 0
        self.enabled = True
        self.words = None
        self._step = False
        self._step_used = 0

    def new_pass(self):
        if not self._step:
            self.block = None

    def new_step(self, device=None):
        if not self._step:
            self.block = None
            self._step = True
            self._step_used = 0
        if device is not None and self.enabled and (self.block is None or self.block.device != device):
            if self.words is None:
                self.words = lib().locate_absmax_words()
            self.cap = self.STEP_SLOTS
            self.block = torch.zeros(self.cap * self.words, dtype=torch.int32, device=device)
            self.used = 0

    def end_step(self):
        if self._step and self._step_used + 16 > self.STEP_SLOTS:
            self.STEP_SLOTS = self._step_used + self._step_used // 4 + 16
        self._step = False

    def slot(self, device):
        if not self.enabled:
            return None
        if self.words is None:
            self.words = lib().locate_absmax_words()
        if self.block is None or self.used >= self.cap or self.block.device != device:
            overflow = self._step and self.block is not None and self.block.device == device
            if overflow and torch.cuda.is_current_stream_capturing():
                raise RuntimeError("hipGraph capture needs more largest-magnitude word sets (%d) than the iteration's block holds: "
                                   "run one eager iteration of this configuration first (the block is sized from it)" % (self._step_used + 1))
            self.cap = self.STEP_SLOTS if self._step else self.SLOTS
            self.block = torch.zeros(self.cap * self.words, dtype=torch.int32, device=device)
            self.used = 0
            if overflow:
                torch.cuda.synchronize()
        s = self.block[self.used * self.words:(self.used + 1) * self.words]
        self.used += 1
        if self._step:
            self._step_used += 1
        return s


AMAX = _AmaxArena()
F16_MIN_FLOPS = 0.5e9


F16_CALLS = {"fwd": 0, "dgrad": 0, "wgrad": 0}
AMAX_MIN_NUMEL = [1 << 16]


def _tag(t, words):
    t._locate_amax = (words, t._version)
    return t


def _amax_of(t):
    if not AMAX.enabled:
        return None
    a = getattr(t, "_locate_amax", None)
    if a is None:
        base = t._base
        if base is not None and base.numel() == t.numel() and base.data_ptr() == t.data_ptr():
            a = getattr(base, "_locate_amax", None)
    if a is None or a[1] != t._version:
        return None
    return a[0]


def carry_amax(src, view):
    if view is not src and view.numel() == src.numel() and view.data_ptr() == src.data_ptr():
        a = getattr(src, "_locate_amax", None)
        if a is not None and a[1] == src._version:
            view._locate_amax = (a[0], view._version)
    return view


def _ensure_amax(t):
    a = _amax_of(t)
    if a is None:
        a = AMAX.slot(t.device)
        if a is None:
            raise RuntimeError("fp8 contractions need the largest-magnitude arena (ops.AMAX.enabled)")
        tc = t if _dense_planes(t) and t.is_contiguous() else t.contiguous()
        check(lib().locate_absmax(_p(tc), tc.numel(), _p(a), _stream()), "locate_absmax")
    return a


def tag_amax(t):
    slot = AMAX.slot(t.device)
    if slot is not None:
        check(lib().locate_absmax(_p(_c(t)), t.numel(), _p(slot), _stream()), "locate_absmax")
        _tag(t, slot)
    return t


class RootTanhFn(torch.autograd.Function):
    @staticmethod
    def forward(ctx, x, slot=None, amax=None, token=None):
        ctx.slot = slot
        ctx.token = token
        x = _c(x, "root_tanh input")
        y = torch.empty_like(x)
        check(lib().locate_roottanh_fwd(_p(x), _p(y), x.numel(), _p(amax), _stream()), "locate_roottanh_fwd")
        ctx.save_for_backward(x)
        return y

    @staticmethod
    def backward(ctx, g):
        x, = ctx.saved_tensors
        g = _c(g)
        token = ctx.token
        if token is not None and token.record is None and GATE_FOLD[0] and token.rt.defer_finalisers and ctx.slot is None:
            token.leave(_FoldRecord(GateTerm.ROOTTANH, g, (g,)))
            return g, None, None, None
        gx, acc = ctx.slot.claim(x) if ctx.slot is not None else (torch.empty_like(x), 0)
        amax = AMAX.slot(x.device) if (ctx.slot is None and x.dim() >= 3 and x.numel() >= AMAX_MIN_NUMEL[0]) else None
        check(lib().locate_roottanh_bwd(_p(x), _p(g), _p(gx), x.numel(), acc, _p(amax), _stream()), "locate_roottanh_bwd")
        if amax is not None:
            _tag(gx, amax)
        return gx, None, None, None


class TanhFn(torch.autograd.Function):
    @staticmethod
    def forward(ctx, x):
        x = _c(x, "tanh input")
        y = torch.empty_like(x)
        check(lib().locate_tanh_fwd(_p(x), _p(y), x.numel(), _stream()), "locate_tanh_fwd")
        ctx.save_for_backward(y)
        return y

    @staticmethod
    def backward(ctx, g):
        y, = ctx.saved_tensors
        g = _c(g)
        gx = torch.empty_like(y)
        check(lib().locate_tanh_bwd(_p(y), _p(g), _p(gx), y.numel(), _stream()), "locate_tanh_bwd")
        return gx


class ActCatFn(torch.autograd.Function):

    @staticmethod
    def forward(ctx, latent, pre):
        latent, pre = _c(latent, "style latent"), _c(pre, "style pre-activation")
        rows, z = latent.shape
        w = pre.shape[1]
        out = torch.empty(rows, z + w, dtype=torch.float32, device=pre.device)
        check(lib().locate_act_cat_rows_fwd(_p(latent), _p(pre), _p(out), rows, z, w, _stream()), "locate_act_cat_rows_fwd")
        ctx.save_for_backward(pre)
        ctx.z = z
        return out, pre.view(rows, w, 1, 1)

    @staticmethod
    def backward(ctx, g, g_scale):
        pre, = ctx.saved_tensors
        z = ctx.z
        if g is None:
            return None, (None if g_scale is None else g_scale.reshape(pre.shape))
        g = _chk(g, "style chain gradient")
        if g.stride(1) != 1:
            g = g.contiguous()
        add = None if g_scale is None else _c(g_scale, "style scale gradient")
        gpre = torch.empty_like(pre)
        check(lib().locate_act_rows_bwd(_p(pre), g.data_ptr() + 4 * z, g.stride(0), _p(add), _p(gpre), pre.shape[0], pre.shape[1],
                                        _stream()), "locate_act_rows_bwd")
        return (g[:, :z] if ctx.needs_input_grad[0] else None), gpre


def root_tanh(x):
    amax = AMAX.slot(x.device) if x.dim() >= 3 and x.numel() >= AMAX_MIN_NUMEL[0] else None
    slot = _slot_of(x) if x.is_contiguous() else None
    token = _token_of(x) if (slot is None and x.is_cuda and x.is_contiguous()) else None
    y = RootTanhFn.apply(x, slot, amax, token)
    if amax is not None:
        _tag(y, amax)
    return y
tanh = TanhFn.apply


def act_cat(latent, pre):
    return ActCatFn.apply(latent, pre)[0]


class Runtime:

    def __init__(self):
        self.precision = 0
        self.stacked = 1
        self.weight_grad_stream = None
        self.weight_grad_side_min_flops = float(os.environ.get("LOCATE_WGRAD_SIDE_MIN_GFLOP", "0")) * 1e9
        self._dv_layers = {}
        self._dv_tables = {}
        self._end_scheduled = False
        self._side = None
        self._side_results = []
        self._keep = []
        self.defer_finalisers = True
        self._fin_dots = []
        self._fin_rank1 = []
        self._fin_sums = []
        self._fin_chan = []
        self._fin_norm = []
        self._fin_wgrad = []
        self._fin_slab = []
        self._streams = {}
        self._homes_taken = set()
        self._fold_pending = []

    def __deepcopy__(self, memo):
        rt = Runtime()
        rt.precision = self.precision
        rt.defer_finalisers = self.defer_finalisers
        return rt

    def stacked_calls(self, n):
        return _Stacked(self, n)

    def weight_grads_on(self, stream):
        return _OnStream(self, stream)

    def finalisers_deferred(self, on):
        return _Deferral(self, on)

    def reset(self):
        self._end_scheduled = False
        self._side = None
        self._side_results = []
        self._keep = []
        self._streams = {}
        self._homes_taken = set()
        for rec in self._fold_pending:
            rec.drop()
        self._fold_pending = []
        AMAX.new_pass()
        self._fin_dots, self._fin_rank1, self._fin_sums, self._fin_chan, self._fin_norm = [], [], [], [], []
        self._fin_wgrad, self._fin_slab = [], []
        for entry in self._dv_layers.values():
            entry[5]["k"] = 0
        self._dv_layers = {}

    def _schedule_end(self):
        st = torch.cuda.current_stream()
        self._streams[st.cuda_stream] = st
        if not self._end_scheduled:
            torch.autograd.Variable._execution_engine.queue_callback(self._end_of_backward)
            self._end_scheduled = True

    def _end_of_backward(self):
        self._end_scheduled = False
        side, self._side = self._side, None
        cur = torch.cuda.current_stream()
        if side is not None:
            cur.wait_stream(side)
        used, self._streams = self._streams, {}
        for sid, st_ in used.items():
            if sid != cur.cuda_stream:
                cur.wait_stream(st_)
        L = lib()
        st = _stream()
        if self._fin_wgrad:
            cap = L.locate_wgrad_batch_max()
            for i in range(0, len(self._fin_wgrad), cap):
                chunk = self._fin_wgrad[i:i + cap]
                check(L.locate_wgrad_batch(b"".join(chunk), len(chunk), st), "locate_wgrad_batch")
            self._fin_wgrad = []
        if self._fin_slab:
            cap = L.locate_slab_reduce_max()
            for i in range(0, len(self._fin_slab), cap):
                chunk = self._fin_slab[i:i + cap]
                check(L.locate_slab_reduce_batch(b"".join(chunk), len(chunk), st), "locate_slab_reduce_batch")
            self._fin_slab = []
        for queue, fn, name in ((self._fin_dots, L.locate_fin_sn_dots, "locate_fin_sn_dots"),
                                (self._fin_rank1, L.locate_fin_sn_rank1, "locate_fin_sn_rank1"),
                                (self._fin_sums, L.locate_fin_sums, "locate_fin_sums"),
                                (self._fin_chan, L.locate_fin_channel_sums, "locate_fin_channel_sums"),
                                (self._fin_norm, L.locate_fin_norm_channels, "locate_fin_norm_channels")):
            if queue:
                blob = b"".join(queue)
                check(fn(blob, len(queue), st), name)
        self._fin_dots, self._fin_rank1, self._fin_sums, self._fin_chan, self._fin_norm = [], [], [], [], []
        results, self._side_results = self._side_results, []
        self._keep = []
        for param, grad in results:
            if param.grad is None or param.grad.data_ptr() == grad.data_ptr():
                param.grad = grad
            else:
                param.grad.add_(grad)
        self._homes_taken = set()
        self._finalize_dv()
        pending, self._fold_pending = self._fold_pending, []
        left = [rec for rec in pending if not rec.done]
        for rec in left:
            rec.drop()
        if left:
            raise RuntimeError("gate fold: %d consumer(s) of a gate's output left their input gradient to the gate's backward kernel, "
                               "which never ran in this pass - that gradient was not computed" % len(left))

    _FIN = __import__("struct").Struct("<8Q2q8i")

    @classmethod
    def _rec(cls, ptrs, longs=(), ints=()):
        ptrs = [0 if t is None else (t if isinstance(t, int) else t.data_ptr()) for t in ptrs]
        return cls._FIN.pack(*(ptrs + [0] * (8 - len(ptrs))), *(list(longs) + [0] * (2 - len(longs))), *(list(ints) + [0] * (8 - len(ints))))

    def queue_sn_dots(self, gy, y, bias, groups, Bg, M, plane, partial):
        self._fin_dots.append(self._rec([gy, y, bias, partial], [gy.stride(0), y.stride(0)], [groups, Bg, M, plane]))
        self._keep.append((gy, y, bias, partial))
        self._schedule_end()

    def queue_sn_rank1(self, partial, npartial, groups, sigma, sigma_stride, u, v, wv, wv_stride, gw, gu, dsig, h, wd):
        self._fin_rank1.append(self._rec([partial, sigma, u, v, wv, gw, gu, dsig], [wv_stride], [npartial, groups, sigma_stride, h, wd]))
        self._keep.append((partial, sigma, u, v, wv, gw, gu, dsig))
        self._schedule_end()

    def queue_sum(self, partial, count, out):
        self._fin_sums.append(self._rec([partial, out], [], [count]))
        self._keep.append((partial, out))
        self._schedule_end()

    def queue_channel_sum(self, g, out):
        Bn, Cn = g.shape[0], g.shape[1]
        hw = g.numel() // (Bn * Cn)
        slices = lib().locate_fin_channel_slices(Bn, Cn, hw)
        part = torch.empty(slices * Cn, dtype=torch.float32, device=g.device) if slices > 1 else None
        self._fin_chan.append(self._rec([g, out, part], [g.stride(0)], [Bn, Cn, hw]))
        self._keep.append((g, out, part))
        self._schedule_end()

    def queue_norm_channels(self, ws, plane_offset, planes, stats, dscale, dbias, B, C, groups):
        s1 = ws.data_ptr() + plane_offset
        self._fin_norm.append(self._rec([s1, s1 + 4 * planes, stats, dscale, dbias], [], [B, C, groups]))
        self._keep.append((ws, stats, dscale, dbias))
        self._schedule_end()

    def queue_small_wgrad(self, record, operands):
        self._fin_wgrad.append(record)
        self._keep.append(operands)
        self._schedule_end()

    def queue_slab_reduce(self, record, operands):
        self._fin_slab.append(record)
        self._keep.append(operands)
        self._schedule_end()

    def fold_pending(self, rec):
        self._fold_pending.append(rec)
        self._schedule_end()

    def late_grad(self, param, grad):
        self._side_results.append((param, grad))
        self._schedule_end()

    def defer_dv(self, v_param, u_param, w, h, wd):
        st = v_param.__dict__.get("_locate_dv")
        if st is None or st["dv"].device != v_param.device:
            nch = (h + 63) // 64
            st = {"dv": torch.empty_like(v_param.detach()), "dsig": torch.zeros(4, dtype=torch.float32, device=v_param.device),
                  "scratch": torch.empty(wd + h + nch * wd, dtype=torch.float32, device=v_param.device), "k": 0}
            v_param.__dict__["_locate_dv"] = st
        home = v_param.__dict__.get("_locate_grad_buf")
        if home is not None and home.device == v_param.device and st["dv"].data_ptr() != home.data_ptr():
            st["dv"] = home.view(st["dv"].shape)
        k = st["k"]
        if k >= 4:
            raise RuntimeError("a spectral-norm layer was differentiated through more than 4 forwards in one backward pass")
        st["k"] = k + 1
        self._dv_layers[id(v_param)] = (v_param, u_param, w, h, wd, st)
        self._schedule_end()
        return st["dsig"][k:]

    def _finalize_dv(self):
        import struct
        layers = list(self._dv_layers.values())
        self._dv_layers = {}
        if not layers:
            return
        key = tuple((w.data_ptr(), u.data_ptr(), st["dv"].data_ptr(), st["dsig"].data_ptr(), st["scratch"].data_ptr(), h, wd)
                    for _, u, w, h, wd, st in layers)
        tab = self._dv_tables.get(key)
        if tab is None:
            rec = struct.Struct("<8Q4i")
            buf = bytearray()
            for v, u, w, h, wd, st in layers:
                base = st["scratch"].data_ptr()
                buf += rec.pack(w.data_ptr(), u.data_ptr(), st["dv"].data_ptr(), st["dsig"].data_ptr(), 0, base, base + 4 * wd,
                                base + 4 * (wd + h), h, wd, (h + 63) // 64, 0)
            host = torch.frombuffer(buf, dtype=torch.uint8).clone()
            tab = (host.to(layers[0][0].device), max(l[3] for l in layers), max(l[4] for l in layers))
            if len(self._dv_tables) > 8:
                self._dv_tables.clear()
            self._dv_tables[key] = tab
        check(lib().locate_sn_dv_batched(tab[0].data_ptr(), len(layers), tab[1], tab[2], _stream()), "locate_sn_dv_batched")
        for v, u, w, h, wd, st in layers:
            st["k"] = 0
            if v.grad is None or v.grad is st["dv"]:
                v.grad = st["dv"]
            else:
                v.grad.add_(st["dv"])


class _Stacked:

    def __init__(self, rt, n):
        self.rt, self.n = rt, int(n)

    def __enter__(self):
        self.prev = self.rt.stacked
        self.rt.stacked = self.n

    def __exit__(self, *exc):
        self.rt.stacked = self.prev
        return False


class _OnStream:

    def __init__(self, rt, stream):
        self.rt, self.stream = rt, stream

    def __enter__(self):
        self.prev = self.rt.weight_grad_stream
        self.rt.weight_grad_stream = self.stream

    def __exit__(self, *exc):
        self.rt.weight_grad_stream = self.prev
        return False


class _Deferral:

    def __init__(self, rt, on):
        self.rt, self.on = rt, bool(on)

    def __enter__(self):
        self.prev = self.rt.defer_finalisers
        self.rt.defer_finalisers = self.on

    def __exit__(self, *exc):
        self.rt.defer_finalisers = self.prev
        return False


def _grad_home(rt, param, shape=None):
    shape = tuple(param.shape if shape is None else shape)
    home = param.__dict__.get("_locate_grad_buf") if param is not None and hasattr(param, "__dict__") else None
    if home is not None and home.device == param.device and home.numel() == param.numel() and id(param) not in rt._homes_taken:
        rt._homes_taken.add(id(param))
        return home.view(shape)
    return torch.empty(shape, dtype=torch.float32, device=param.device)


DEFAULT_RUNTIME = Runtime()
DEFAULT_RUNTIME.defer_finalisers = False


def stacked_calls(n):
    return DEFAULT_RUNTIME.stacked_calls(n)


def weight_grad_stream(stream):
    return DEFAULT_RUNTIME.weight_grads_on(stream)


def reset_backward_state(*runtimes):
    for rt in runtimes or (DEFAULT_RUNTIME,):
        rt.reset()


class _GradSlot:
    __slots__ = ("buf", "claims", "written", "deferred")

    def __init__(self):
        self.buf = None
        self.claims = 0
        self.written = False
        self.deferred = None

    def _take(self, like, shape):
        shape = tuple(like.shape if shape is None else shape)
        self.claims += 1
        if self.claims > 2:
            raise RuntimeError("fork: more than two backward kernels claimed one fan-out buffer - each alias of a forked tensor "
                               "must feed exactly one participating consumer")
        if self.buf is None:
            self.buf = like.new_empty(shape)
        return self.buf if tuple(self.buf.shape) == shape else self.buf.view(shape)

    def claim(self, like, shape=None):
        buf = self._take(like, shape)
        acc, self.written = int(self.written), True
        return buf, acc

    def claim_deferred(self, like, rec):
        buf = self._take(like, None)
        self.deferred = rec
        return buf


class ForkFn(torch.autograd.Function):

    @staticmethod
    def forward(ctx, x, slot):
        ctx.slot = slot
        return x.view_as(x), x.view_as(x)

    @staticmethod
    def backward(ctx, ga, gb):
        slot, ctx.slot = ctx.slot, None
        buf, claims, rec, written = slot.buf, slot.claims, slot.deferred, slot.written
        slot.buf, slot.claims, slot.deferred, slot.written = None, 0, None, False
        if rec is not None:
            foreign = [g for g in (ga, gb) if g is not None and g.data_ptr() != buf.data_ptr()]
            delivered = sum(1 for g in (ga, gb) if g is not None and g.data_ptr() == buf.data_ptr())
            if delivered != claims or (foreign and written):
                raise RuntimeError("fork: %d consumer(s) claimed the shared gradient buffer but %d branch(es) delivered it - an "
                                   "alias of a forked tensor fed more than one op" % (claims, delivered))
            if foreign:
                buf.copy_(foreign[0])
                written = True
            rec.has_share = written
            return buf, None
        if ga is None or gb is None:
            return (gb if ga is None else ga), None
        shared = [g for g in (ga, gb) if buf is not None and g.data_ptr() == buf.data_ptr()]
        if len(shared) != claims:
            raise RuntimeError("fork: %d consumer(s) accumulated into the shared gradient buffer but %d branch(es) delivered it - an "
                               "alias of a forked tensor fed more than one op" % (claims, len(shared)))
        if ga.data_ptr() == gb.data_ptr():
            return ga, None
        return ga + gb, None


def fork(x):
    if not (torch.is_grad_enabled() and x.requires_grad):
        return x, x
    slot = _GradSlot()
    a, b = ForkFn.apply(x, slot)
    a._locate_slot = b._locate_slot = slot
    stats = getattr(x, "_locate_stats", None)
    if stats is not None:
        a._locate_stats = b._locate_stats = stats
    token = _token_of(x)
    if token is not None:
        a._locate_gate = b._locate_gate = token
    return a, b


class Fork3Fn(torch.autograd.Function):

    @staticmethod
    def forward(ctx, x):
        return x.view_as(x), x.view_as(x), x.view_as(x)

    @staticmethod
    def backward(ctx, g_identity, g_conv, g_norm):
        gs = [g for g in (g_norm, g_identity, g_conv) if g is not None]
        if len(gs) == 3 and all(_batch_strided(g) for g in gs) and gs[0].shape == gs[1].shape == gs[2].shape:
            a, b, c = gs
            out = torch.empty(a.shape, dtype=a.dtype, device=a.device)
            per = a[0].numel()
            check(lib().locate_add3(_p(a), a.stride(0), _p(b), b.stride(0), _p(c), c.stride(0), _p(out), a.shape[0], per, _stream()),
                  "locate_add3")
            return out
        total = None
        for g in gs:
            total = g if total is None else total + g
        return total


def _batch_strided(g):
    return (g.is_cuda and g.dtype == torch.float32 and g.dim() >= 2 and g.shape[0] > 0 and g[0].is_contiguous()
            and (g.shape[0] == 1 or g.stride(0) >= g[0].numel()))


def fork3(x):
    if not (torch.is_grad_enabled() and x.requires_grad):
        return x, x, x
    a, b, c = Fork3Fn.apply(x)
    stats = getattr(x, "_locate_stats", None)
    if stats is not None:
        a._locate_stats = b._locate_stats = c._locate_stats = stats
    return a, b, c


def _slot_of(x):
    return getattr(x, "_locate_slot", None)


class _FoldRecord:
    __slots__ = ("kind", "buf", "keep", "fields", "has_share", "done", "token", "stream")

    def __init__(self, kind, buf, keep, **fields):
        self.kind, self.buf, self.keep, self.fields = kind, buf, keep, fields
        self.has_share = False
        self.done = False
        self.token = None
        self.stream = _stream()

    def drop(self):
        if self.token is not None and self.token.record is self:
            self.token.record = None
        self.keep = self.buf = None

    def term(self):
        return GateTerm(kind=self.kind, has_share=int(self.has_share), **self.fields)


class _GateToken:
    __slots__ = ("rt", "record")

    def __init__(self, rt):
        self.rt = rt
        self.record = None

    def leave(self, rec):
        rec.token = self
        self.record = rec
        self.rt.fold_pending(rec)


def _token_of(x):
    return getattr(x, "_locate_gate", None)


class InPlaceNormFn(torch.autograd.Function):

    @staticmethod
    def forward(ctx, x, scale, bias, with_act, groups, pre_partial=None, slot=None, amax=None, rt=None, token=None):
        ctx.slot = slot
        ctx.token = token
        ctx.rt = rt or DEFAULT_RUNTIME
        ctx.scale_in, ctx.bias_in = scale, bias
        x = _c(x, "norm input")
        B, C = x.shape[0], x.shape[1]
        hw = x.numel() // (B * C)
        if B % groups:
            raise ValueError("norm: batch %d does not split into %d stacked calls" % (B, groups))
        per_sample = scale.numel() == B * C and (B > 1 and scale.shape[0] == B)
        if not per_sample and scale.numel() != C:
            raise ValueError("norm scale must have C or B*C elements, got %s for input %s" % (tuple(scale.shape), tuple(x.shape)))
        scale_c, bias_c = _c(scale, "norm scale"), _c(bias, "norm bias")
        L = lib()
        st = _stream()
        stats = torch.empty(2 * groups, dtype=torch.float32, device=x.device)
        ws = _ws(L.locate_norm_stats_workspace_bytes(), x.device) if pre_partial is None else None
        out = torch.empty_like(x)
        check(L.locate_norm_fwd(_p(x), _p(scale_c), int(per_sample), _p(bias_c), _p(out), int(bool(with_act)), _p(stats), B, C, hw,
                                groups, _p(ws), _p(pre_partial), _p(amax), st), "locate_norm_fwd")
        ctx.per_sample, ctx.with_act, ctx.groups = per_sample, bool(with_act), groups
        ctx.scale_shape, ctx.bias_shape = scale.shape, bias.shape
        ctx.save_for_backward(x, scale_c, bias_c, stats)
        return out

    @staticmethod
    def backward(ctx, g):
        L = lib()
        st = _stream()
        g = _c(g)
        x, scale, bias, stats = ctx.saved_tensors
        B, C = x.shape[0], x.shape[1]
        hw = x.numel() // (B * C)
        rt = ctx.rt
        need_scale, need_bias = ctx.needs_input_grad[1], ctx.needs_input_grad[2]
        per_channel_scale_ok = ctx.per_sample or not need_scale or ctx.scale_in.is_leaf
        if rt.defer_finalisers and per_channel_scale_ok and (not need_bias or ctx.bias_in.is_leaf):
            ws = _ws(L.locate_norm_bwd_fused_workspace_bytes(B, C), x.device)
            dscale = torch.empty(ctx.scale_shape, dtype=torch.float32, device=x.device) if ctx.per_sample else None
            token = ctx.token
            if (token is not None and token.record is None and GATE_FOLD[0] and ctx.slot is not None and ctx.needs_input_grad[0]
                    and token.rt.defer_finalisers and (not ctx.with_act or x.numel() >= GATE_FOLD_ACT_MIN_NUMEL[0])):
                check(L.locate_norm_bwd_planes(_p(x), _p(g), _p(stats), _p(scale), int(ctx.per_sample), _p(bias), int(ctx.with_act),
                                               _p(dscale), B, C, hw, ctx.groups, _p(ws), st), "locate_norm_bwd_planes")
                rec = _FoldRecord(GateTerm.NORM, None, (g, stats, scale, bias, ws), with_act=int(ctx.with_act),
                                  per_sample=int(ctx.per_sample), go=_p(g), stats=_p(stats), scale=_p(scale), bias=_p(bias), partial=_p(ws),
                                  npartial=L.locate_norm_bwd_fused_partials(B, C), B=B, C=C, groups=ctx.groups)
                dx = rec.buf = ctx.slot.claim_deferred(x, rec)
                token.leave(rec)
            else:
                dx, acc = ctx.slot.claim(x) if ctx.slot is not None else (torch.empty_like(x), 0)
                check(L.locate_norm_bwd_fused(_p(x), _p(g), _p(stats), _p(scale), int(ctx.per_sample), _p(bias), int(ctx.with_act),
                                              _p(dx), _p(dscale), B, C, hw, ctx.groups, _p(ws), acc, st), "locate_norm_bwd_fused")
            late_scale = _grad_home(rt, ctx.scale_in, ctx.scale_shape) if (need_scale and not ctx.per_sample) else None
            late_bias = _grad_home(rt, ctx.bias_in, ctx.bias_shape) if need_bias else None
            if late_scale is not None or late_bias is not None:
                rt.queue_norm_channels(ws, L.locate_norm_bwd_fused_plane_offset(), B * C, stats, late_scale, late_bias, B, C, ctx.groups)
                if late_scale is not None:
                    rt.late_grad(ctx.scale_in, late_scale)
                if late_bias is not None:
                    rt.late_grad(ctx.bias_in, late_bias)
            return dx, dscale, None, None, None, None, None, None, None, None
        dx, acc = ctx.slot.claim(x) if ctx.slot is not None else (torch.empty_like(x), 0)
        dscale = torch.empty(ctx.scale_shape, dtype=torch.float32, device=x.device)
        dbias = torch.empty(ctx.bias_shape, dtype=torch.float32, device=x.device)
        ws = _ws(L.locate_norm_bwd_workspace_bytes(B, C), x.device)
        check(L.locate_norm_bwd(_p(x), _p(g), _p(stats), _p(scale), int(ctx.per_sample), _p(bias), int(ctx.with_act), _p(dx),
                                _p(dscale), _p(dbias), B, C, hw, ctx.groups, _p(ws), acc, st), "locate_norm_bwd")
        return dx, dscale, dbias, None, None, None, None, None, None, None


def inplace_norm(x, scale, bias, with_act=False, runtime=None):
    groups = (runtime or DEFAULT_RUNTIME).stacked
    pre = getattr(x, "_locate_stats", None)
    pre_partial = pre[0] if (pre is not None and pre[1] == groups and x.is_contiguous()) else None
    amax = AMAX.slot(x.device) if x.numel() >= AMAX_MIN_NUMEL[0] else None
    slot = _slot_of(x) if x.is_contiguous() else None
    token = _token_of(x) if (slot is not None and x.is_cuda) else None
    out = InPlaceNormFn.apply(x, scale, bias, with_act, groups, pre_partial, slot, amax, runtime, token)
    if amax is not None:
        _tag(out, amax)
    return out


class GateFn(torch.autograd.Function):

    @staticmethod
    def forward(ctx, x, a, gamma, stats_groups=0, holder=None, slot=None, rt=None, token=None):
        ctx.slot = slot
        ctx.token = token
        ctx.rt = rt or DEFAULT_RUNTIME
        ctx.gamma_param = gamma
        x = _c(x, "gate input")
        a = _c(a, "gate attention")
        gamma = _c(gamma, "gate gamma")
        planes = x.shape[0] * x.shape[1]
        hw = x.numel() // planes
        per_plane = a.numel() == planes and x.numel() != planes
        if not per_plane and a.numel() != x.numel():
            raise ValueError("gate: attention shape %s does not match input %s" % (tuple(a.shape), tuple(x.shape)))
        out = torch.empty_like(x)
        L = lib()
        n_g = x.numel() // stats_groups if stats_groups else 0
        if stats_groups and x.shape[0] % stats_groups == 0 and n_g > 1 and (stats_groups == 1 or n_g % 4 == 0):
            partial = torch.empty(L.locate_norm_stats_workspace_bytes() // 8, dtype=torch.float64, device=x.device)
            check(L.locate_gate_fwd_stats(_p(x), _p(a), int(per_plane), _p(gamma), _p(out), planes, hw, stats_groups, _p(partial),
                                          _stream()), "locate_gate_fwd_stats")
            holder.append((partial, stats_groups))
        else:
            check(L.locate_gate_fwd(_p(x), _p(a), int(per_plane), _p(gamma), _p(out), planes, hw, _stream()), "locate_gate_fwd")
        ctx.save_for_backward(x, a, gamma)
        ctx.per_plane = per_plane
        return out

    @staticmethod
    def backward(ctx, g):
        x, a, gamma = ctx.saved_tensors
        rec = ctx.token.record if ctx.token is not None else None
        if rec is not None:
            ctx.token.record = None
            if g.data_ptr() != rec.buf.data_ptr():
                rec.drop()
                raise RuntimeError("gate fold: the gradient that reached the gate is not the buffer its output's consumer handed "
                                   "over - the gate's output fed a further op besides that consumer")
            rec.done = True
        g = _c(g)
        L = lib()
        rt = ctx.rt
        planes = x.shape[0] * x.shape[1]
        hw = x.numel() // planes
        dx, acc = ctx.slot.claim(x) if ctx.slot is not None else (torch.empty_like(x), 0)
        da = torch.empty_like(a)
        need_gamma = ctx.needs_input_grad[2]
        deferred = need_gamma and rt.defer_finalisers and ctx.gamma_param.is_leaf
        dgamma = (_grad_home(rt, ctx.gamma_param, gamma.shape) if deferred else torch.empty_like(gamma)) if need_gamma else None
        ws = _ws(L.locate_gate_bwd_workspace_bytes(planes), x.device)
        amax = AMAX.slot(x.device) if (not ctx.per_plane and da.numel() >= AMAX_MIN_NUMEL[0]) else None
        if rec is not None:
            if rec.stream != _stream():
                for t in rec.keep:
                    t.record_stream(torch.cuda.current_stream())
            check(L.locate_gate_bwd_term(_p(x), _p(a), int(ctx.per_plane), _p(gamma), _p(g), _p(dx), _p(da), None if deferred else _p(dgamma),
                                         planes, hw, _p(ws), acc, _p(amax), rec.term(), _stream()), "locate_gate_bwd_term")
            rec.keep = rec.buf = None
        else:
            check(L.locate_gate_bwd(_p(x), _p(a), int(ctx.per_plane), _p(gamma), _p(g), _p(dx), _p(da), None if deferred else _p(dgamma),
                                    planes, hw, _p(ws), acc, _p(amax), _stream()), "locate_gate_bwd")
        if amax is not None:
            _tag(da, amax)
        if deferred:
            rt.queue_sum(ws, L.locate_gate_bwd_partials(planes, hw), dgamma)
            rt.late_grad(ctx.gamma_param, dgamma.view(ctx.gamma_param.shape))
            dgamma = None
        return dx, da, dgamma, None, None, None, None, None


def residual_gate(x, a, gamma, runtime=None, with_stats=True):
    slot = _slot_of(x) if x.is_contiguous() else None
    token = _GateToken(runtime or DEFAULT_RUNTIME) if (GATE_FOLD[0] and x.is_cuda and torch.is_grad_enabled()) else None
    holder = []
    out = GateFn.apply(x, a, gamma, (runtime or DEFAULT_RUNTIME).stacked if with_stats else 0, holder if with_stats else None, slot,
                       runtime, token)
    if holder:
        out._locate_stats = holder[0]
    if token is not None and out.requires_grad:
        out._locate_gate = token
    return out




class SoftmaxFn(torch.autograd.Function):
    @staticmethod
    def forward(ctx, x):
        x = _c(x, "softmax input")
        n = x.shape[-1]
        y = torch.empty_like(x)
        check(lib().locate_softmax_fwd(_p(x), _p(y), x.numel() // n, n, _stream()), "locate_softmax_fwd")
        ctx.save_for_backward(y)
        return y

    @staticmethod
    def backward(ctx, g):
        y, = ctx.saved_tensors
        g = _c(g)
        n = y.shape[-1]
        gx = torch.empty_like(y)
        check(lib().locate_softmax_bwd(_p(y), _p(g), _p(gx), y.numel() // n, n, _stream()), "locate_softmax_bwd")
        return gx


softmax_lastdim = SoftmaxFn.apply


class Upsample2xFn(torch.autograd.Function):
    @staticmethod
    def forward(ctx, x):
        x = _c(x, "upsample input")
        B, C, H, W = x.shape
        y = torch.empty(B, C, 2 * H, 2 * W, dtype=x.dtype, device=x.device)
        check(lib().locate_upsample2x_fwd(_p(x), _p(y), B * C, H, W, _stream()), "locate_upsample2x_fwd")
        ctx.shape = (B, C, H, W)
        return y

    @staticmethod
    def backward(ctx, g):
        B, C, H, W = ctx.shape
        g = _c(g)
        gx = torch.empty(B, C, H, W, dtype=g.dtype, device=g.device)
        check(lib().locate_upsample2x_bwd(_p(g), _p(gx), B * C, H, W, _stream()), "locate_upsample2x_bwd")
        return gx


class PoolUpsampleFn(torch.autograd.Function):

    @staticmethod
    def forward(ctx, x, slot=None):
        ctx.slot = slot
        x = _c(x, "feature pooling input")
        B, C, H, W = x.shape
        y = torch.empty(B, C // 2, 2 * H, 2 * W, dtype=x.dtype, device=x.device)
        check(lib().locate_pool2_upsample2x_fwd(_p(x), _p(y), B * (C // 2), H, W, _stream()), "locate_pool2_upsample2x_fwd")
        ctx.in_shape = (B, C, H, W)
        return y

    @staticmethod
    def backward(ctx, g):
        B, C, H, W = ctx.in_shape
        g = _c(g)
        if ctx.slot is not None:
            gx, acc = ctx.slot.claim(g, ctx.in_shape)
        else:
            gx, acc = torch.empty(ctx.in_shape, dtype=g.dtype, device=g.device), 0
        check(lib().locate_pool2_upsample2x_bwd(_p(g), _p(gx), B * (C // 2), H, W, acc, _stream()), "locate_pool2_upsample2x_bwd")
        return gx, None


def pool_upsample_ok(x, out_features):
    return x.is_cuda and x.dim() == 4 and x.dtype == torch.float32 and x.shape[1] == 2 * out_features and POOL_UPSAMPLE[0]


def pool_upsample(x, out_features):
    return PoolUpsampleFn.apply(x, _slot_of(x) if x.is_contiguous() else None)


POOL_UPSAMPLE = [os.environ.get("LOCATE_POOL_UPSAMPLE", "1") != "0"]


class AvgPool2Fn(torch.autograd.Function):
    @staticmethod
    def forward(ctx, x, slot=None):
        ctx.slot = slot
        x = _c(x, "avgpool input")
        B, C, H, W = x.shape
        y = torch.empty(B, C, H // 2, W // 2, dtype=x.dtype, device=x.device)
        check(lib().locate_avgpool2_fwd(_p(x), _p(y), B * C, H, W, _stream()), "locate_avgpool2_fwd")
        ctx.shape = (B, C, H, W)
        return y

    @staticmethod
    def backward(ctx, g):
        B, C, H, W = ctx.shape
        g = _c(g)
        if ctx.slot is not None:
            gx, acc = ctx.slot.claim(g, (B, C, H, W))
        else:
            gx, acc = torch.empty(B, C, H, W, dtype=g.dtype, device=g.device), 0
        check(lib().locate_avgpool2_bwd(_p(g), _p(gx), B * C, H, W, acc, _stream()), "locate_avgpool2_bwd")
        return gx, None


class FeaturePoolFn(torch.autograd.Function):

    @staticmethod
    def forward(ctx, x, out_features, slot=None):
        ctx.slot = slot
        x = _c(x, "feature pooling input")
        B, C = x.shape[0], x.shape[1]
        if C % out_features:
            raise ValueError("FeaturePooling: %d channels not divisible by %d" % (C, out_features))
        r = C // out_features
        y = torch.empty((B, out_features) + tuple(x.shape[2:]), dtype=x.dtype, device=x.device)
        check(lib().locate_feature_pool_fwd(_p(x), _p(y), y.numel(), r, _stream()), "locate_feature_pool_fwd")
        ctx.in_shape, ctx.r = x.shape, r
        return y

    @staticmethod
    def backward(ctx, g):
        g = _c(g)
        if ctx.slot is not None:
            gx, acc = ctx.slot.claim(g, ctx.in_shape)
        else:
            gx, acc = torch.empty(ctx.in_shape, dtype=g.dtype, device=g.device), 0
        check(lib().locate_feature_pool_bwd(_p(g), _p(gx), g.numel(), ctx.r, acc, _stream()), "locate_feature_pool_bwd")
        return gx, None, None


upsample2x = Upsample2xFn.apply


def avgpool2(x):
    return AvgPool2Fn.apply(x, _slot_of(x) if x.is_contiguous() else None)


def feature_pool(x, out_features):
    return FeaturePoolFn.apply(x, out_features, _slot_of(x) if x.is_contiguous() else None)


def _copy_channels(src, dst, accumulate=False):
    B, C = src.shape[0], src.shape[1]
    hw = src[0, 0].numel() if src.dim() > 2 else 1
    check(lib().locate_copy_channels(_p(src), _p(dst), B, C, hw, src.stride(0), dst.stride(0), int(accumulate), _stream()),
          "locate_copy_channels")


def _dense_planes(t):
    if t.dim() < 2:
        return False
    expect = 1
    for size, stride in zip(reversed(t.shape[1:]), reversed(t.stride()[1:])):
        if size != 1 and stride != expect:
            return False
        expect *= size
    return True


class CatChannelsFn(torch.autograd.Function):

    @staticmethod
    def forward(ctx, a, b, holder=None):
        a = _c(a, "cat input")
        ca, cb = a.shape[1], b.shape[1]
        buf = holder[0] if holder else None
        if buf is not None and buf.shape[1] == ca + cb and b.data_ptr() == buf[:, ca:].data_ptr() and b.stride() == buf[:, ca:].stride():
            out = buf
        else:
            b = _c(b, "cat input")
            out = torch.empty((a.shape[0], ca + cb) + tuple(a.shape[2:]), dtype=a.dtype, device=a.device)
            _copy_channels(b, out[:, ca:])
        _copy_channels(a, out[:, :ca])
        ctx.split = (ca, cb)
        return out

    @staticmethod
    def backward(ctx, g):
        ca, cb = ctx.split
        return g[:, :ca], g[:, ca:], None


def cat_channels(a, b, holder=None):
    return CatChannelsFn.apply(a, b, holder)


class ConvSpec:
    __slots__ = ("kind", "kh", "kw", "stride", "pad_h", "pad_w", "mode")

    def __init__(self, kind, kh, kw, stride, pad_h, pad_w, mode="dense"):
        self.kind, self.kh, self.kw, self.stride, self.pad_h, self.pad_w, self.mode = kind, kh, kw, stride, pad_h, pad_w, mode

    def geometry(self, x_shape, w_shape):
        B, Cx, H, W = x_shape
        M, C = w_shape[0], w_shape[1]
        s = self.stride
        if self.mode == "groupdot":
            if Cx % M or Cx // M != C or (H, W) != tuple(w_shape[2:]):
                raise ValueError("grouped full-size conv: input %s does not fit weight %s" % (tuple(x_shape), tuple(w_shape)))
            return [B, M, C * H * W] + [0] * 9, (B, M, 1, 1)
        if self.mode == "depthwise":
            if self.kind == "conv":
                if C != 1 or M % Cx:
                    raise ValueError("depthwise conv: input has %d channels, weight is %s" % (Cx, tuple(w_shape)))
                C = Cx
            else:
                if Cx != M:
                    raise ValueError("depthwise convT: input has %d channels, weight expects %d" % (Cx, M))
                C = M * C
        if self.kind == "conv":
            if Cx != C:
                raise ValueError("conv: input has %d channels, weight expects %d" % (Cx, C))
            OH = (H + 2 * self.pad_h - self.kh) // s + 1
            OW = (W + 2 * self.pad_w - self.kw) // s + 1
            return [B, C, H, W, M, self.kh, self.kw, s, self.pad_h, self.pad_w, OH, OW], (B, M, OH, OW)
        if Cx != M:
            raise ValueError("convT: input has %d channels, weight expects %d" % (Cx, M))
        RH = (H - 1) * s - 2 * self.pad_h + self.kh
        RW = (W - 1) * s - 2 * self.pad_w + self.kw
        return [B, C, RH, RW, M, self.kh, self.kw, s, self.pad_h, self.pad_w, H, W], (B, C, RH, RW)


def _geom(arr):
    return _IntArr12(*arr)


def _bs(t):
    return t.stride(0)


def _panel_owner(w):
    base = w._base
    return w if base is None else base


def _panel(owner, w, geom, garr, adjoint):
    L = lib()
    cache = owner.__dict__.setdefault("_locate_panels", {})
    key = (adjoint, tuple(geom[1:10]), w.data_ptr())
    hit = cache.get(key)
    ver = owner._version
    if hit is not None and hit[0] == ver and hit[1].device == w.device:
        return hit[1]
    nbytes = L.locate_conv_panel_bytes(garr, adjoint)
    buf = hit[1] if (hit is not None and hit[1].numel() == max(nbytes, 16) and hit[1].device == w.device) else _ws(nbytes, w.device)
    check(L.locate_conv_pack_panel(garr, adjoint, _p(w), _p(buf), _stream()), "locate_conv_pack_panel")
    cache[key] = (ver, buf, list(geom))
    return buf


DIRECT_REPACK = os.environ.get("LOCATE_DIRECT_REPACK", "1") != "0"


class _PackPlans:
    cache = {}


def refresh_panels(params):
    import ctypes
    L = lib()
    stale = []
    for w in params:
        cache = w.__dict__.get("_locate_panels")
        if not cache:
            continue
        ver = w._version
        for key, (pver, buf, geom) in cache.items():
            if pver != ver and buf.device == w.device and w.is_contiguous():
                stale.append((w, key, buf, geom))
    if not stale:
        return
    def wmax_of(w):
        hold = w.__dict__.get("_locate_wmax") if DIRECT_REPACK else None
        return hold[0].data_ptr() if (hold is not None and hold[1] == w._version and hold[0].device == w.device) else None

    wm = [wmax_of(w) if key[0] & 10 else None for w, key, _, _ in stale]
    direct = int(DIRECT_REPACK)
    sig = tuple((key[2], key[0], buf.data_ptr(), m, direct) + tuple(geom) for (_, key, buf, geom), m in zip(stale, wm))
    plan = _PackPlans.cache.get(sig)
    if plan is None:
        rec = L.locate_conv_pack_job_bytes()
        host = ctypes.create_string_buffer(rec * len(stale))
        start = 0
        two_pass = two_pass_f16 = 0
        for i, (w, key, buf, geom) in enumerate(stale):
            nb = ctypes.c_int(0)
            check(L.locate_conv_pack_job(_geom(geom), key[0], key[2], _p(buf), start, ctypes.addressof(host) + i * rec,
                                         ctypes.byref(nb), direct, wm[i]), "locate_conv_pack_job")
            start += nb.value
            if not L.locate_conv_pack_job_is_direct(ctypes.addressof(host) + i * rec):
                two_pass |= 2 if L.locate_conv_pack_job_is_window(ctypes.addressof(host) + i * rec) else 1
                two_pass_f16 |= int(bool(key[0] & 10))
        table = torch.frombuffer(host, dtype=torch.uint8).clone().to(stale[0][0].device)
        plan = (table, len(stale), start, two_pass_f16, two_pass)
        if len(_PackPlans.cache) > 16:
            _PackPlans.cache.clear()
        _PackPlans.cache[sig] = plan
    check(L.locate_conv_pack_panels(_p(plan[0]), plan[1], plan[2], plan[3], plan[4], _stream()), "locate_conv_pack_panels")
    for w, key, buf, geom in stale:
        w.__dict__["_locate_panels"][key] = (w._version, buf, geom)


def sn_power_iteration(w_bar, u, v):
    L = lib()
    h = w_bar.shape[0]
    wd = w_bar.numel() // h
    w = _c(w_bar.detach(), "weight_bar")
    sigma = torch.empty(2, dtype=torch.float32, device=w.device)
    wv = torch.empty(h, dtype=torch.float32, device=w.device)
    ws = _ws(L.locate_sn_workspace_bytes(h, wd), w.device)
    check(L.locate_sn_power_iter(_p(w), _p(_chk(u.detach(), "weight_u")), _p(_chk(v.detach(), "weight_v")), _p(sigma), _p(wv),
                                 h, wd, _p(ws), _stream()), "locate_sn_power_iter")
    return sigma, wv


def _sigma_args(sigma, batch):
    groups = sigma.shape[0] if sigma.dim() == 2 else 1
    if groups == 1:
        return 1, 0, 0, sigma.reshape(-1)[1:]
    if batch % groups or groups > 4 or sigma.stride(1) != 1:
        raise ValueError("conv: batch %d cannot stack %d calls" % (batch, groups))
    return groups, batch // groups, sigma.stride(0), sigma[0, 1:]


_COUNTER_LANE = [0]


class counter_lane:

    def __init__(self, lane):
        self.lane = int(lane)

    def __enter__(self):
        self.prev = _COUNTER_LANE[0]
        _COUNTER_LANE[0] = self.lane

    def __exit__(self, *exc):
        _COUNTER_LANE[0] = self.prev


def _counters(owner, adjoint):
    cache = owner.__dict__.setdefault("_locate_counters", {})
    sid = torch.cuda.current_stream().cuda_stream
    lane = _COUNTER_LANE[0]
    key = (adjoint, sid) if lane == 0 else (adjoint, "lane%d" % lane)
    buf = cache.get(key)
    if buf is not None and buf.device == owner.device:
        return buf
    if torch.cuda.is_current_stream_capturing():
        buf = cache.get((adjoint, 0)) if lane == 0 else None
        if buf is None or buf.device != owner.device:
            raise RuntimeError("hipGraph capture of a contraction that never ran eagerly: run one eager iteration first (its "
                               "arrival counters must exist before the capture)")
        return buf
    for k in {key, (adjoint, 0), (adjoint, "lane1")}:
        if k not in cache or cache[k].device != owner.device:
            cache[k] = torch.zeros(lib().locate_conv_counter_bytes(), dtype=torch.uint8, device=owner.device)
    return cache[key]


def _flops(geom):
    B, C, H, W, M, KH, KW, s_, ph, pw, OH, OW = geom
    return 2.0 * B * OH * OW * M * C * KH * KW


def _f16_ok(spec, geom, precision, *amax):
    return precision == 0 and spec.mode == "dense" and all(a is not None for a in amax) and _flops(geom) >= F16_MIN_FLOPS


WIN_MODE = {"0": 0, "all": 2}.get(os.environ.get("LOCATE_WINDOW", "1"), 1)
WIN_CALLS = [0]
FP8_CALLS = [0]
_WIN_CACHE = {}


def _win_ok(geom, garr, adjfmt, x):
    if not WIN_MODE:
        return False
    key = (tuple(geom), adjfmt, _bs(x) & 1, x.data_ptr() & 7)
    hit = _WIN_CACHE.get(key)
    if hit is None:
        hit = lib().locate_conv_win_ok(garr, adjfmt, _bs(x), _p(x))
        _WIN_CACHE[key] = hit
    return hit == 1 or (hit == 2 and WIN_MODE == 2)


def _win_ws_bytes(geom, garr, adjfmt):
    key = (tuple(geom), adjfmt, "ws")
    hit = _WIN_CACHE.get(key)
    if hit is None:
        hit = lib().locate_conv_win_workspace_bytes(garr, adjfmt)
        _WIN_CACHE[key] = hit
    return hit


CONTRACTION_TAP = None


def _contract(forward_of_r, x, w, owner, spec, geom, garr, sigma, bias, y, precision=0, amax=None, epilogue=None):
    if CONTRACTION_TAP is not None and spec.mode == "dense":
        CONTRACTION_TAP("fwd" if forward_of_r == (spec.kind == "conv") else "dgrad", w, x, None, forward_of_r)
    L = lib()
    st = _stream()
    _, sbg, sst, inv_sigma = _sigma_args(sigma, x.shape[0])
    if spec.mode == "dense":
        f16 = _f16_ok(spec, geom, precision, amax)
        prec, fmt, am = (2, 2, amax) if f16 else (precision, 0, None)
        if f16:
            F16_CALLS["fwd" if forward_of_r == (spec.kind == "conv") else "dgrad"] += 1
        if precision == 3:
            prec, fmt, am = 3, 8, _ensure_amax(x)
            FP8_CALLS[0] += 1
        adj = 0 if forward_of_r else 1
        win = precision != 3 and _win_ok(geom, garr, adj | fmt, x)
        if win:
            fmt |= 4
            prec |= 16
            WIN_CALLS[0] += 1
            ws = _ws(_win_ws_bytes(geom, garr, adj | (fmt & 2)), x.device)
        if forward_of_r:
            if not win:
                ws = _ws(L.locate_conv_fwd_workspace_bytes(garr), x.device)
            check(L.locate_conv_fwd(garr, _p(x), _bs(x), _p(_panel(owner, w, geom, garr, 0 | fmt)), _p(inv_sigma), sbg, sst, _p(bias), _p(y),
                                    _bs(y), _p(ws), _p(_counters(owner, 0)), prec, _p(am),
                                    ctypes.addressof(epilogue) if epilogue is not None else None, st), "locate_conv_fwd")
        else:
            if not win:
                ws = _ws(L.locate_conv_dgrad_workspace_bytes(garr), x.device)
            check(L.locate_conv_dgrad(garr, _p(x), _bs(x), _p(_panel(owner, w, geom, garr, 1 | fmt)), _p(inv_sigma), sbg, sst, _p(bias), _p(y),
                                      _bs(y), _p(ws), _p(_counters(owner, 1)), prec, _p(am),
                                      ctypes.addressof(epilogue) if epilogue is not None else None, st), "locate_conv_dgrad")
        return y
    if bias is not None:
        raise NotImplementedError("grouped convolutions carry no bias in the reference (libs/conv.py:15, libs/attention.py:18)")
    if spec.mode == "depthwise":
        fn, name = (L.locate_dwconv_fwd, "locate_dwconv_fwd") if forward_of_r else (L.locate_dwconv_dgrad, "locate_dwconv_dgrad")
        check(fn(garr, _p(x), _bs(x), _p(w), _p(inv_sigma), sbg, sst, _p(y), _bs(y), st), name)
        return y
    B, G, Ln = geom[:3]
    if forward_of_r:
        check(L.locate_groupdot_fwd(_p(x), _bs(x), _p(w), _p(inv_sigma), sbg, sst, _p(y), B, G, Ln, st), "locate_groupdot_fwd")
    else:
        check(L.locate_groupdot_dgrad(_p(x), _p(w), _p(inv_sigma), sbg, sst, _p(y), _bs(y), B, G, Ln, st), "locate_groupdot_dgrad")
    return y


def act_epilogue_ok(spec, x_shape):
    return spec.kind == "conv" and spec.mode == "dense" and (spec.kh, spec.kw, spec.stride, spec.pad_h, spec.pad_w) == (1, 1, 1, 0, 0) \
        and tuple(x_shape[2:]) == (1, 1)


def _conv_apply(x, w, owner, spec, geom, garr, sigma, bias, out_shape, precision=0, amax=None, out=None, epilogue=None):
    if out is not None and spec.mode == "dense" and tuple(out.shape) == tuple(out_shape) and _dense_planes(out) and out.dtype == torch.float32:
        y = out
    else:
        y = torch.empty(out_shape, dtype=torch.float32, device=x.device)
    return _contract(spec.kind == "conv", x, w, owner, spec, geom, garr, sigma, bias, y, precision, amax, epilogue)


def _conv_input_grad(gy, x_like, w, owner, spec, geom, garr, sigma, precision=0, amax=None, link=None):
    if spec.mode == "groupdot":
        gy = gy.contiguous()
    gx = torch.empty_like(x_like)
    epi = None
    if link is not None:
        pre = link.pre
        slot = AMAX.slot(gx.device) if (gx.dim() >= 3 and gx.numel() >= AMAX_MIN_NUMEL[0]) else None
        epi = _ActEpilogue(None, 0, None, 0, 0, 0, pre.data_ptr(), _bs(pre), _p(slot))
    _contract(spec.kind != "conv", gy, w, owner, spec, geom, garr, sigma, None, gx, precision, amax, epi)
    if link is not None:
        link.premultiplied = True
        if slot is not None:
            _tag(gx, slot)
    return gx


def _raw_weight_grad(spec, geom, garr, xin, gout, gw, w_ref, inv_sigma, sbg, sst, partial, precision=0, amax_in=None, amax_out=None,
                     rt=None, group_dots=0, w_key=None):
    if CONTRACTION_TAP is not None and spec.mode == "dense":
        CONTRACTION_TAP("wgrad", w_ref if w_ref is not None else w_key, *((xin, gout) if spec.kind == "conv" else (gout, xin)), True)
    L = lib()
    st = _stream()
    if spec.mode == "dense" and rt is not None and rt.defer_finalisers:
        rec = ctypes.create_string_buffer(L.locate_wgrad_batch_record_bytes())
        if L.locate_wgrad_batch_record(garr, _p(xin), _bs(xin), _p(gout), _bs(gout), _p(gw), _p(w_ref), _p(inv_sigma), sbg, sst,
                                       _p(partial), rec) > 0:
            rt.queue_small_wgrad(rec.raw, (xin, gout, gw, w_ref, inv_sigma, partial))
            return
    if spec.mode == "dense":
        nbytes = L.locate_conv_wgrad_group_workspace_bytes(garr, group_dots) if group_dots else L.locate_conv_wgrad_workspace_bytes(garr)
        defer = rt is not None and rt.defer_finalisers and nbytes > 0
        ws = torch.empty(nbytes, dtype=torch.uint8, device=xin.device) if defer else _ws(nbytes, xin.device)
        rec = ctypes.create_string_buffer(L.locate_slab_reduce_record_bytes()) if defer else None
        f16 = _f16_ok(spec, geom, precision, amax_in, amax_out)
        F16_CALLS["wgrad"] += int(f16)
        if precision == 3:
            amax_in, amax_out = _ensure_amax(xin), _ensure_amax(gout)
        scaled = f16 or precision == 3
        check(L.locate_conv_wgrad(garr, _p(xin), _bs(xin), _p(gout), _bs(gout), _p(gw), _p(w_ref), _p(inv_sigma), sbg, sst, _p(partial),
                                  _p(ws), 2 if f16 else precision, _p(amax_in) if scaled else None, _p(amax_out) if scaled else None, rec, st),
              "locate_conv_wgrad")
        if defer and L.locate_slab_reduce_record_blocks(rec) > 0:
            rt.queue_slab_reduce(rec.raw, (ws, gw, w_ref, inv_sigma, partial))
    elif spec.mode == "depthwise":
        ws = _ws(L.locate_dwconv_wgrad_workspace_bytes(garr), xin.device)
        check(L.locate_dwconv_wgrad(garr, _p(xin), _bs(xin), _p(gout), _bs(gout), _p(gw), _p(w_ref), _p(inv_sigma), sbg, sst,
                                    _p(partial), _p(ws), st), "locate_dwconv_wgrad")
    else:
        B, G, Ln = geom[:3]
        gout = gout.contiguous()
        check(L.locate_groupdot_wgrad(_p(xin), _bs(xin), _p(gout), _p(gw), _p(w_ref), _p(inv_sigma), sbg, sst, _p(partial), B, G, Ln,
                                      st), "locate_groupdot_wgrad")


def _weight_grad_partials(spec, geom, garr):
    L = lib()
    if spec.mode == "dense":
        return L.locate_conv_wgrad_partials(garr)
    if spec.mode == "depthwise":
        return L.locate_dwconv_wgrad_partials(garr)
    return L.locate_groupdot_wgrad_partials(geom[1], geom[2])


def _conv_weight_grad(rt, x, gy, y, bias, w, u_param, v_param, sigma, wv, spec, geom, garr, need_u, need_v, amax_x=None, amax_gy=None,
                      owner=None):
    L = lib()
    st = _stream()
    groups, sbg, sst, inv_sigma = _sigma_args(sigma, x.shape[0])
    gw = _grad_home(rt, owner, w.shape) if (owner is not None and owner.is_leaf) else torch.empty_like(w)
    xin, gout = (x, gy) if spec.kind == "conv" else (gy, x)
    am_in, am_out = (amax_x, amax_gy) if spec.kind == "conv" else (amax_gy, amax_x)
    h = w.shape[0]
    wd = w.numel() // h
    u, v = u_param.detach(), v_param.detach()
    gu = (_grad_home(rt, u_param) if u_param.is_leaf else torch.empty_like(u)) if need_u else None
    if groups > 1:
        npg = L.locate_conv_wgrad_group_partials(garr, groups) if (rt.defer_finalisers and spec.mode == "dense") else 0
        if npg > 0:
            partial = torch.empty(groups * npg, dtype=torch.float64, device=x.device)
            _raw_weight_grad(spec, geom, garr, xin, gout, gw, w, inv_sigma, sbg, sst, partial, rt.precision, am_in, am_out, rt, groups)
            dsig = rt.defer_dv(v_param, u_param, w, h, wd) if need_v else None
            rt.queue_sn_rank1(partial, npg, groups, sigma, sigma.stride(0), u, v, wv, wv.stride(0), gw, gu, dsig, h, wd)
            return gw, gu
        _raw_weight_grad(spec, geom, garr, xin, gout, gw, None, inv_sigma, sbg, sst, None, rt.precision, am_in, am_out, rt, w_key=w)
        dsig = rt.defer_dv(v_param, u_param, w, h, wd) if need_v else None
        Bn, Mn = gy.shape[0], gy.shape[1]
        plane = gy.numel() // (Bn * Mn)
        if rt.defer_finalisers:
            npart = L.locate_fin_sn_dot_partials(Bn // groups, Mn, plane)
            partial = torch.empty(groups * npart, dtype=torch.float64, device=x.device)
            rt.queue_sn_dots(gy, y, bias, groups, Bn // groups, Mn, plane, partial)
            rt.queue_sn_rank1(partial, npart, groups, sigma, sigma.stride(0), u, v, wv, wv.stride(0), gw, gu, dsig, h, wd)
            return gw, gu
        gws = _ws(L.locate_sn_group_workspace_bytes(), x.device)
        check(L.locate_sn_weight_bwd_grouped(_p(gy), _bs(gy), _p(y), _bs(y), _p(bias), groups, Bn // groups, Mn, plane,
                                             _p(sigma), sigma.stride(0), _p(u), _p(v), _p(wv),
                                             wv.stride(0), _p(gw), _p(gu), _p(dsig), h, wd, _p(gws), st),
              "locate_sn_weight_bwd_grouped")
        return gw, gu
    npart = _weight_grad_partials(spec, geom, garr)
    partial = torch.empty(npart, dtype=torch.float64, device=x.device)
    _raw_weight_grad(spec, geom, garr, xin, gout, gw, w, inv_sigma, 0, 0, partial, rt.precision, am_in, am_out, rt)
    dsig = rt.defer_dv(v_param, u_param, w, h, wd) if need_v else None
    if rt.defer_finalisers:
        rt.queue_sn_rank1(partial, npart, 0, sigma, 0, u, v, wv, 0, gw, gu, dsig, h, wd)
        return gw, gu
    check(L.locate_sn_weight_bwd(_p(partial), npart, _p(u), _p(v), _p(sigma), _p(wv), _p(gw), _p(gu), _p(dsig), h, wd, st),
          "locate_sn_weight_bwd")
    return gw, gu


def _bias_grad(gy):
    Bn, Cn = gy.shape[0], gy.shape[1]
    gb = torch.empty(Cn, dtype=torch.float32, device=gy.device)
    L = lib()
    hw = gy.numel() // (Bn * Cn)
    ws = _ws(L.locate_channel_sum_workspace_bytes(Bn, Cn, hw), gy.device)
    check(L.locate_channel_sum(_p(gy), _p(gb), Bn, Cn, hw, _bs(gy), _p(ws), _stream()), "locate_channel_sum")
    return gb


def _dense(t, what):
    _chk(t, what)
    return t if _dense_planes(t) else t.contiguous()


class SNConvFn(torch.autograd.Function):

    @staticmethod
    def forward(ctx, x, w_bar, u, v, bias, sigma, wv, spec, rt=None, guard=None, out_holder=None, act=None, in_link=None):
        ctx.guard = guard
        x = _dense(x, "conv input")
        w = _c(w_bar, "weight_bar")
        owner = _panel_owner(w_bar)
        geom, out_shape = spec.geometry(tuple(x.shape), tuple(w.shape))
        garr = _geom(geom)
        b = _c(bias) if bias is not None else None
        rt = rt or DEFAULT_RUNTIME
        ctx.amax_x = _amax_of(x)
        epi = second = second_amax = None
        ctx.act_z = None
        ctx.act_link = act.get("link") if act is not None else None
        ctx.in_link = in_link if (in_link is not None and spec.mode == "dense") else None
        if act is not None:
            Bn, Mn = out_shape[0], out_shape[1]
            lat = act.get("latent")
            z = 0 if lat is None else lat.shape[1]
            second = torch.empty((Bn, z + Mn) if lat is not None else out_shape, dtype=torch.float32, device=x.device)
            if ctx.act_link is not None:
                if lat is not None or out_holder:
                    raise ValueError("an activation link excludes a latent prefix and an output slice")
                plane_elems = second.numel() // Bn
                if second.dim() >= 3 and second.numel() >= AMAX_MIN_NUMEL[0]:
                    second_amax = AMAX.slot(x.device)
                epi = _ActEpilogue(second.data_ptr(), plane_elems, None, 0, 0, 0, None, 0, _p(second_amax))
            else:
                epi = _ActEpilogue(second.data_ptr() + 4 * z, z + Mn, _p(lat), 0 if lat is None else lat.stride(0), z, 0, None, 0, None)
            if lat is not None and (lat.stride(1) != 1 or lat.shape[0] != Bn):
                raise ValueError("style latent must be [B, z] with contiguous rows")
            ctx.act_z = z
        y = _conv_apply(x, w, owner, spec, geom, garr, sigma, b, out_shape, rt.precision, ctx.amax_x, out_holder[0] if out_holder else None, epi)
        if ctx.act_link is not None:
            ctx.act_link.pre = y
            if second_amax is not None:
                _tag(second, second_amax)
        groups = sigma.shape[0] if sigma.dim() == 2 else 1
        ctx.groups = groups
        if groups > 1:
            ctx.save_for_backward(x, w, sigma, wv, y, b)
        elif second is not None:
            ctx.save_for_backward(x, w, sigma, wv, y)
        else:
            ctx.save_for_backward(x, w, sigma, wv)
        if second is not None:
            ctx.set_materialize_grads(False)
        ctx.u, ctx.v = u, v
        ctx.bias_param = bias
        ctx.owner = owner
        ctx.rt = rt
        ctx.geom, ctx.spec, ctx.has_bias = geom, spec, bias is not None
        if second is None:
            return y
        return y, second

    @staticmethod
    def backward(ctx, gy, g_second=None):
        pre = None
        if ctx.groups > 1:
            x, w, sigma, wv, y, bsaved = ctx.saved_tensors
            pre = y
        elif ctx.act_z is not None:
            x, w, sigma, wv, pre = ctx.saved_tensors
            y = bsaved = None
        else:
            x, w, sigma, wv = ctx.saved_tensors
            y = bsaved = None
        if ctx.act_link is not None and g_second is not None and ctx.act_link.premultiplied:
            ctx.act_link.premultiplied = False
            if gy is not None:
                raise RuntimeError("a linked pre-activation has one consumer, its activation")
            gy = g_second.reshape(pre.shape) if g_second.shape != pre.shape else g_second
        elif ctx.act_z is not None and g_second is not None:
            Bn = pre.shape[0]
            Mn = pre.numel() // Bn
            g2 = _chk(g_second, "activated output gradient")
            if g2.dim() != 2:
                g2 = g2.reshape(Bn, -1)
            if g2.stride(1) != 1:
                g2 = g2.contiguous()
            add = None if gy is None else _c(gy, "conv output gradient")
            total = torch.empty(pre.shape, dtype=torch.float32, device=pre.device)
            check(lib().locate_act_rows_bwd(_p(pre), g2.data_ptr() + 4 * ctx.act_z, g2.stride(0), _p(add), _p(total), Bn, Mn, _stream()),
                  "locate_act_rows_bwd")
            gy = total
        if gy is None:
            return (None,) * 13
        spec, garr = ctx.spec, _geom(ctx.geom)
        if ctx.guard is not None:
            ctx.guard[0].check(ctx.guard[1])
        gy = _dense(gy, "conv output gradient")
        amax_gy = _amax_of(gy)
        need_x, need_w, need_u, need_v, need_b = ctx.needs_input_grad[:5]
        gx = gw = gu = gb = None
        if need_x:
            gx = _conv_input_grad(gy, x, w, ctx.owner, spec, ctx.geom, garr, sigma, ctx.rt.precision, amax_gy, ctx.in_link)
        if need_w or need_u or need_v:
            rt = ctx.rt
            side = rt.weight_grad_stream
            if side is not None and spec.mode == "dense" and _flops(ctx.geom) < rt.weight_grad_side_min_flops:
                side = None
            late = side is not None or rt.defer_finalisers
            if side is None:
                sgw, sgu = _conv_weight_grad(rt, x, gy, y, bsaved, w, ctx.u, ctx.v, sigma, wv, spec, ctx.geom, garr, need_u, need_v,
                                             ctx.amax_x, amax_gy, ctx.owner if late else None)
            else:
                side.wait_stream(torch.cuda.current_stream())
                with torch.cuda.stream(side):
                    sgw, sgu = _conv_weight_grad(rt, x, gy, y, bsaved, w, ctx.u, ctx.v, sigma, wv, spec, ctx.geom, garr, need_u, need_v,
                                                 ctx.amax_x, amax_gy, ctx.owner if late else None)
                rt._side = side
            if late:
                rt._keep.append((x, gy, y, bsaved, w, sigma, wv))
                if need_w:
                    rt.late_grad(ctx.owner, sgw.view(ctx.owner.shape))
                if need_u:
                    rt.late_grad(ctx.u, sgu)
                rt._schedule_end()
            else:
                gw, gu = (sgw if need_w else None), sgu
        if ctx.has_bias and need_b:
            if ctx.rt.defer_finalisers and ctx.bias_param.is_leaf:
                late_gb = _grad_home(ctx.rt, ctx.bias_param, (gy.shape[1],))
                ctx.rt.queue_channel_sum(gy, late_gb)
                ctx.rt.late_grad(ctx.bias_param, late_gb.view(ctx.bias_param.shape))
            else:
                gb = _bias_grad(gy)
        return gx, gw, gu, None, gb, None, None, None, None, None, None, None, None


def sn_conv(x, w_bar, u, v, bias, spec, sigma_wv=None, runtime=None, guard=None, out=None, act=None, in_link=None):
    if sigma_wv is None:
        sigma_wv = sn_power_iteration(w_bar, u, v)
    sigma, wv = sigma_wv
    return SNConvFn.apply(x, w_bar, u, v, bias, sigma, wv, spec, runtime, guard, None if out is None else [out], act, in_link)
```

Measured before the change: 7280 images/sec.

## Fold fork3 three-share gradient sum into the gate backward norm-term kernel

When a gate's output fans out three ways (identity, conv, norm) through fork3, the norm's input gradient is now deferred into the producing gate's backward kernel. That kernel reads the identity and conv shares directly and adds them, instead of running a separate add3 kernel and materialising the summed gradient. This removes one elementwise launch and its memory round-trip per fork3 site. In exchange it adds template variants, extra pointer plumbing across autograd functions, and new error paths if the alias feeds further ops.

```diff
diff --git a/include/locate_hip.h b/include/locate_hip.h
--- a/include/locate_hip.h
+++ b/include/locate_hip.h
@@ -66,6 +66,15 @@
 int locate_gate_bwd_term(const float* x, const float* a, int a_per_plane, const float* gamma, const float* g, float* dx, float* da,
                          float* dgamma, int64_t planes, int hw, void* workspace, int accumulate_dx, void* da_absmax,
                          LocateGateTerm term, void* stream);
+typedef struct {
+    LocateGateTerm norm;
+    const float* ident;
+    int64_t ident_bs;
+    const float* conv;
+} LocateGateTerm3;
+int locate_gate_bwd_term3(const float* x, const float* a, int a_per_plane, const float* gamma, float* dx, float* da, float* dgamma,
+                          int64_t planes, int hw, void* workspace, int accumulate_dx, void* da_absmax, LocateGateTerm3 term,
+                          void* stream);
 
 int locate_softmax_fwd(const float* x, float* y, int64_t rows, int n, void* stream);
 int locate_softmax_bwd(const float* y, const float* gy, float* gx, int64_t rows, int n, void* stream);
diff --git a/locate_amd/_lib.py b/locate_amd/_lib.py
--- a/locate_amd/_lib.py
+++ b/locate_amd/_lib.py
@@ -21,6 +21,10 @@
     _fields_ = [("kind", ctypes.c_int32), ("with_act", ctypes.c_int32), ("per_sample", ctypes.c_int32), ("has_share", ctypes.c_int32),
                 ("go", c_p), ("stats", c_p), ("scale", c_p), ("bias", c_p), ("partial", c_p),
                 ("npartial", ctypes.c_int32), ("B", ctypes.c_int32), ("C", ctypes.c_int32), ("groups", ctypes.c_int32)]
+
+
+class GateTerm3(ctypes.Structure):
+    _fields_ = [("norm", GateTerm), ("ident", c_p), ("ident_bs", ctypes.c_int64), ("conv", c_p)]
 
 
 PROTOTYPES = {
@@ -58,6 +62,7 @@
     "locate_gate_bwd_workspace_bytes": (c_sz, [c_i64]),
     "locate_gate_bwd": (c_i, [c_p, c_p, c_i, c_p, c_p, c_p, c_p, c_p, c_i64, c_i, c_p, c_i, c_p, c_p]),
     "locate_gate_bwd_term": (c_i, [c_p, c_p, c_i, c_p, c_p, c_p, c_p, c_p, c_i64, c_i, c_p, c_i, c_p, GateTerm, c_p]),
+    "locate_gate_bwd_term3": (c_i, [c_p, c_p, c_i, c_p, c_p, c_p, c_p, c_i64, c_i, c_p, c_i, c_p, GateTerm3, c_p]),
     "locate_softmax_fwd": (c_i, [c_p, c_p, c_i64, c_i, c_p]),
     "locate_softmax_bwd": (c_i, [c_p, c_p, c_p, c_i64, c_i, c_p]),
     "locate_upsample2x_fwd": (c_i, [c_p, c_p, c_i64, c_i, c_i, c_p]),
@@ -199,7 +204,7 @@
     pass
 
 
-EXPECTED_ABI = 21
+EXPECTED_ABI = 22
 
 
 _lib = None
diff --git a/locate_amd/csrc/elementwise.hip b/locate_amd/csrc/elementwise.hip
--- a/locate_amd/csrc/elementwise.hip
+++ b/locate_amd/csrc/elementwise.hip
@@ -313,11 +313,32 @@
     return r;
 }
 
-template <int TERM>
-__device__ __forceinline__ float gate_term_g(const GateTermPlane& tp, float out, float gin, float share, int has_share) {
+__device__ __forceinline__ float gate_add_a_first(float a, float b) {
+    float r;
+    asm("v_add_f32 %0, %1, %2" : "=v"(r) : "v"(a), "v"(b));
+    return r;
+}
+
+template <int TERM, int SHARES = 1>
+__device__ __forceinline__ float gate_term_g(const GateTermPlane& tp, float out, float gin, float share, int has_share, float share2 = 0.0f) {
     if constexpr (TERM == GATE_TERM_ROOTTANH) return roottanh_grad_f(out, gin);
     const float o = norm_dx<TERM == GATE_TERM_NORM_ACT>(out, gin, tp.mu, tp.inv_s, tp.y, tp.b, tp.k, tp.m);
+    if constexpr (SHARES == 3) return gate_add_a_first(gate_add_a_first(o, share), share2);
     return has_share ? o + share : o;
+}
+
+template <int SHARES> struct GateTermArg { typedef LocateGateTerm type; };
+template <> struct GateTermArg<3> { typedef LocateGateTerm3 type; };
+__host__ __device__ __forceinline__ const LocateGateTerm& gate_norm_term(const LocateGateTerm& t) { return t; }
+__host__ __device__ __forceinline__ const LocateGateTerm& gate_norm_term(const LocateGateTerm3& t) { return t.norm; }
+
+struct GateSharePlane { const float* ident; const float* conv; };
+__device__ __forceinline__ GateSharePlane gate_share_plane(const LocateGateTerm3& t, int64_t p, int hw) {
+    const unsigned b = (unsigned)p / (unsigned)t.norm.C, c = (unsigned)p % (unsigned)t.norm.C;
+    return {t.ident + (int64_t)b * t.ident_bs + (int64_t)c * hw, t.conv + p * hw};
+}
+__device__ __forceinline__ float gate_share_ident_elem(const LocateGateTerm3& t, unsigned e) {
+    return t.ident[(int64_t)(e / (unsigned)t.norm.C) * t.ident_bs + e % (unsigned)t.norm.C];
 }
 
 template <int TERM>
@@ -342,13 +363,28 @@
     return s;
 }
 
-template <int WPP, int TERM, bool ELEM = false>
+template <int TERM>
+__device__ __forceinline__ float gate_plane_da_nonfinite_term3(const float* __restrict__ x, const float* __restrict__ gs,
+                                                            const float* __restrict__ ident, const float* __restrict__ conv, int hw,
+                                                            float gm, float ap, GateTermPlane tp) {
+    float s = 0.0f;
+    const float mv = fmaf(gm, ap, 1.0f);
+    for (int i = 0; i < hw; ++i) {
+        const float g = gate_term_g<TERM, 3>(tp, mul_pinned(mv, x[i]), gs[i], ident[i], 0, conv[i]);
+        s += (x[i] * g) * gm;
+    }
+    return s;
+}
+
+template <int WPP, int TERM, bool ELEM = false, int SHARES = 1>
 __global__ void __launch_bounds__(256) gate_bwd_plane_kernel(const float* __restrict__ x, const float* __restrict__ a,
                                                              const float* __restrict__ gamma, const float* __restrict__ g,
                                                              float* __restrict__ dx, float* __restrict__ da_full,
                                                              float* __restrict__ da_plane, double* __restrict__ block_x2g,
                                                              int64_t planes, int hw, int a_per_plane, int accumulate_dx,
-                                                             unsigned* __restrict__ da_absmax, const LocateGateTerm t) {
+                                                             unsigned* __restrict__ da_absmax, const typename GateTermArg<SHARES>::type tt) {
+    static_assert(SHARES == 1 || (SHARES == 3 && gate_term_is_norm(TERM)), "three shares go with a norm term");
+    const LocateGateTerm& t = gate_norm_term(tt);
     __shared__ double wsum[4], px2g[4];
     __shared__ float pxg[4];
     __shared__ float amax_scratch[16];
@@ -369,6 +405,9 @@
     bool vec = (hw & 3) == 0 && ((reinterpret_cast<uintptr_t>(x) | reinterpret_cast<uintptr_t>(g) | reinterpret_cast<uintptr_t>(dx) |
                                   (a_per_plane ? 0 : (reinterpret_cast<uintptr_t>(a) | reinterpret_cast<uintptr_t>(da_full)))) & 15) == 0;
     if constexpr (gate_term_is_norm(TERM)) vec = vec && (reinterpret_cast<uintptr_t>(gs) & 15) == 0;
+    if constexpr (SHARES == 3)
+        vec = vec && (reinterpret_cast<uintptr_t>(tt.conv) & 15) == 0 &&
+              (elem || ((reinterpret_cast<uintptr_t>(tt.ident) & 15) == 0 && (tt.ident_bs & 3) == 0));
     for (int64_t p = first; p < planes; p += step) {
         const int64_t base = p * hw;
         const float ap = a_per_plane ? a[p] : 0.0f;
@@ -376,6 +415,11 @@
         GateTermPlane tp = {0.0f, 1.0f, 0.0f, 0.0f, 0.0f, 0.0f};
         if constexpr (gate_term_is_norm(TERM))
             if (!elem) tp = gate_term_plane<TERM>(t, tc, (unsigned)p, planes_g);
+        GateSharePlane sp = {nullptr, nullptr};
+        if constexpr (SHARES == 3) {
+            if (elem) sp.conv = tt.conv + base;
+            else sp = gate_share_plane(tt, p, hw);
+        }
         if (vec) {
             for (int i = sub; i < (hw >> 2); i += nsub) {
                 const float4 xv = reinterpret_cast<const float4*>(x + base)[i];
@@ -385,17 +429,30 @@
                 if constexpr (TERM != GATE_TERM_NONE) {
                     const float4 ov = make_float4(mul_pinned(fmaf(gm, av.x, 1.0f), xv.x), mul_pinned(fmaf(gm, av.y, 1.0f), xv.y),
                                                   mul_pinned(fmaf(gm, av.z, 1.0f), xv.z), mul_pinned(fmaf(gm, av.w, 1.0f), xv.w));
-                    float4 sh = make_float4(0.0f, 0.0f, 0.0f, 0.0f);
-                    if (has_share) sh = reinterpret_cast<const float4*>(g + base)[i];
+                    float4 sh = make_float4(0.0f, 0.0f, 0.0f, 0.0f), sh2 = sh;
+                    if constexpr (SHARES == 3) {
+                        if (elem) {
+                            const unsigned e = (unsigned)(base + 4 * i);
+                            sh = make_float4(gate_share_ident_elem(tt, e), gate_share_ident_elem(tt, e + 1), gate_share_ident_elem(tt, e + 2),
+                                             gate_share_ident_elem(tt, e + 3));
+                        } else {
+                            sh = reinterpret_cast<const float4*>(sp.ident)[i];
+                        }
+                        sh2 = reinterpret_cast<const float4*>(sp.conv)[i];
+                    } else if (has_share) {
+                        sh = reinterpret_cast<const float4*>(g + base)[i];
+                    }
                     if (elem) {
                         const unsigned e = (unsigned)(base + 4 * i);
-                        gv.x = gate_term_g<TERM>(gate_term_plane<TERM>(t, tc, e, planes_g), ov.x, gv.x, sh.x, has_share);
-                        gv.y = gate_term_g<TERM>(gate_term_plane<TERM>(t, tc, e + 1, planes_g), ov.y, gv.y, sh.y, has_share);
-                        gv.z = gate_term_g<TERM>(gate_term_plane<TERM>(t, tc, e + 2, planes_g), ov.z, gv.z, sh.z, has_share);
-                        gv.w = gate_term_g<TERM>(gate_term_plane<TERM>(t, tc, e + 3, planes_g), ov.w, gv.w, sh.w, has_share);
+                        gv.x = gate_term_g<TERM, SHARES>(gate_term_plane<TERM>(t, tc, e, planes_g), ov.x, gv.x, sh.x, has_share, sh2.x);
+                        gv.y = gate_term_g<TERM, SHARES>(gate_term_plane<TERM>(t, tc, e + 1, planes_g), ov.y, gv.y, sh.y, has_share, sh2.y);
+                        gv.z = gate_term_g<TERM, SHARES>(gate_term_plane<TERM>(t, tc, e + 2, planes_g), ov.z, gv.z, sh.z, has_share, sh2.z);
+                        gv.w = gate_term_g<TERM, SHARES>(gate_term_plane<TERM>(t, tc, e + 3, planes_g), ov.w, gv.w, sh.w, has_share, sh2.w);
                     } else {
-                        gv.x = gate_term_g<TERM>(tp, ov.x, gv.x, sh.x, has_share); gv.y = gate_term_g<TERM>(tp, ov.y, gv.y, sh.y, has_share);
-                        gv.z = gate_term_g<TERM>(tp, ov.z, gv.z, sh.z, has_share); gv.w = gate_term_g<TERM>(tp, ov.w, gv.w, sh.w, has_share);
+                        gv.x = gate_term_g<TERM, SHARES>(tp, ov.x, gv.x, sh.x, has_share, sh2.x);
+                        gv.y = gate_term_g<TERM, SHARES>(tp, ov.y, gv.y, sh.y, has_share, sh2.y);
+                        gv.z = gate_term_g<TERM, SHARES>(tp, ov.z, gv.z, sh.z, has_share, sh2.z);
+                        gv.w = gate_term_g<TERM, SHARES>(tp, ov.w, gv.w, sh.w, has_share, sh2.w);
                     }
                 }
                 const float4 xg = make_float4(xv.x * gv.x, xv.y * gv.y, xv.z * gv.z, xv.w * gv.w);
@@ -424,7 +481,11 @@
                 const float av = a_per_plane ? ap : a[base + i];
                 if constexpr (TERM != GATE_TERM_NONE) {
                     if (elem) tp = gate_term_plane<TERM>(t, tc, (unsigned)(base + i), planes_g);
-                    gv = gate_term_g<TERM>(tp, mul_pinned(fmaf(gm, av, 1.0f), xv), gv, has_share ? g[base + i] : 0.0f, has_share);
+                    if constexpr (SHARES == 3)
+                        gv = gate_term_g<TERM, 3>(tp, mul_pinned(fmaf(gm, av, 1.0f), xv), gv,
+                                                  elem ? gate_share_ident_elem(tt, (unsigned)(base + i)) : sp.ident[i], 0, sp.conv[i]);
+                    else
+                        gv = gate_term_g<TERM>(tp, mul_pinned(fmaf(gm, av, 1.0f), xv), gv, has_share ? g[base + i] : 0.0f, has_share);
                 }
                 const float xg = xv * gv;
                 float o = fmaf(gm, av, 1.0f) * gv;
@@ -442,6 +503,8 @@
             if (lane == 0 && a_per_plane) {
                 if (gate_gamma_finite(gm)) da_plane[p] = gm * sxg;
                 else if constexpr (TERM == GATE_TERM_NONE) da_plane[p] = gate_plane_da_nonfinite(x + base, g + base, hw, gm);
+                else if constexpr (SHARES == 3)
+                    da_plane[p] = gate_plane_da_nonfinite_term3<TERM>(x + base, gs + base, sp.ident, sp.conv, hw, gm, ap, tp);
                 else da_plane[p] = gate_plane_da_nonfinite_term<TERM>(x + base, gs + base, g + base, hw, gm, ap, tp, has_share);
             }
         } else {
@@ -453,6 +516,8 @@
                 if (a_per_plane) {
                     if (gate_gamma_finite(gm)) da_plane[p] = gm * ((pxg[0] + pxg[1]) + (pxg[2] + pxg[3]));
                     else if constexpr (TERM == GATE_TERM_NONE) da_plane[p] = gate_plane_da_nonfinite(x + base, g + base, hw, gm);
+                    else if constexpr (SHARES == 3)
+                        da_plane[p] = gate_plane_da_nonfinite_term3<TERM>(x + base, gs + base, sp.ident, sp.conv, hw, gm, ap, tp);
                     else da_plane[p] = gate_plane_da_nonfinite_term<TERM>(x + base, gs + base, g + base, hw, gm, ap, tp, has_share);
                 }
             }
@@ -468,13 +533,15 @@
     if (da_absmax && !a_per_plane) absmax_publish(am, amax_scratch, da_absmax);
 }
 
-template <int LP, int TERM, bool ELEM = false>
+template <int LP, int TERM, bool ELEM = false, int SHARES = 1>
 __global__ void __launch_bounds__(256) gate_bwd_small_kernel(const float* __restrict__ x, const float* __restrict__ a,
                                                              const float* __restrict__ gamma, const float* __restrict__ g,
                                                              float* __restrict__ dx, float* __restrict__ da_full,
                                                              float* __restrict__ da_plane, double* __restrict__ block_x2g,
                                                              int64_t planes, int hw, int a_per_plane, int accumulate_dx,
-                                                             unsigned* __restrict__ da_absmax, const LocateGateTerm t) {
+                                                             unsigned* __restrict__ da_absmax, const typename GateTermArg<SHARES>::type tt) {
+    static_assert(SHARES == 1 || (SHARES == 3 && gate_term_is_norm(TERM)), "three shares go with a norm term");
+    const LocateGateTerm& t = gate_norm_term(tt);
     __shared__ double wsum[4];
     __shared__ float amax_scratch[16];
     __shared__ float tc[NORM_MAX_GROUPS][2];
@@ -491,6 +558,12 @@
     constexpr bool elem = ELEM;
     const unsigned planes_g = gate_term_is_norm(TERM) ? (unsigned)((int64_t)t.B * t.C / t.groups) : 1u;
     const int has_share = gate_term_is_norm(TERM) ? t.has_share : 0;
+    if constexpr (SHARES == 3) {
+        if ((int64_t)blockIdx.x * 4 * PW >= planes) {
+            if (threadIdx.x == 0) block_x2g[blockIdx.x] = 0.0;
+            return;
+        }
+    }
     if constexpr (gate_term_is_norm(TERM)) gate_term_consts<TERM>(t, (int64_t)planes_g * (elem ? 1 : hw), tc);
     for (int64_t p0 = wave * PW; p0 < planes; p0 += nwaves * PW) {
         const int64_t p = p0 + gid;
@@ -498,6 +571,13 @@
         float sxg = 0.0f, sx2g = 0.0f;
         float ap = 0.0f;
         GateTermPlane tp = {0.0f, 1.0f, 0.0f, 0.0f, 0.0f, 0.0f};
+        GateSharePlane sp = {nullptr, nullptr};
+        if constexpr (SHARES == 3) {
+            if (live) {
+                if (elem) sp.conv = tt.conv + p * hw;
+                else sp = gate_share_plane(tt, p, hw);
+            }
+        }
         if (live && li < q4) {
             const int64_t base = p * hw;
             ap = a_per_plane ? a[p] : 0.0f;
@@ -508,18 +588,31 @@
             if constexpr (TERM != GATE_TERM_NONE) {
                 const float4 ov = make_float4(mul_pinned(fmaf(gm, av.x, 1.0f), xv.x), mul_pinned(fmaf(gm, av.y, 1.0f), xv.y),
                                               mul_pinned(fmaf(gm, av.z, 1.0f), xv.z), mul_pinned(fmaf(gm, av.w, 1.0f), xv.w));
-                float4 sh = make_float4(0.0f, 0.0f, 0.0f, 0.0f);
-                if (has_share) sh = reinterpret_cast<const float4*>(g + base)[li];
+                float4 sh = make_float4(0.0f, 0.0f, 0.0f, 0.0f), sh2 = sh;
+                if constexpr (SHARES == 3) {
+                    if (elem) {
+                        const unsigned e = (unsigned)(base + 4 * li);
+                        sh = make_float4(gate_share_ident_elem(tt, e), gate_share_ident_elem(tt, e + 1), gate_share_ident_elem(tt, e + 2),
+                                         gate_share_ident_elem(tt, e + 3));
+                    } else {
+                        sh = reinterpret_cast<const float4*>(sp.ident)[li];
+                    }
+                    sh2 = reinterpret_cast<const float4*>(sp.conv)[li];
+                } else if (has_share) {
+                    sh = reinterpret_cast<const float4*>(g + base)[li];
+                }
                 if (elem) {
                     const unsigned e = (unsigned)(base + 4 * li);
-                    gv.x = gate_term_g<TERM>(gate_term_plane<TERM>(t, tc, e, planes_g), ov.x, gv.x, sh.x, has_share);
-                    gv.y = gate_term_g<TERM>(gate_term_plane<TERM>(t, tc, e + 1, planes_g), ov.y, gv.y, sh.y, has_share);
-                    gv.z = gate_term_g<TERM>(gate_term_plane<TERM>(t, tc, e + 2, planes_g), ov.z, gv.z, sh.z, has_share);
-                    gv.w = gate_term_g<TERM>(gate_term_plane<TERM>(t, tc, e + 3, planes_g), ov.w, gv.w, sh.w, has_share);
+                    gv.x = gate_term_g<TERM, SHARES>(gate_term_plane<TERM>(t, tc, e, planes_g), ov.x, gv.x, sh.x, has_share, sh2.x);
+                    gv.y = gate_term_g<TERM, SHARES>(gate_term_plane<TERM>(t, tc, e + 1, planes_g), ov.y, gv.y, sh.y, has_share, sh2.y);
+                    gv.z = gate_term_g<TERM, SHARES>(gate_term_plane<TERM>(t, tc, e + 2, planes_g), ov.z, gv.z, sh.z, has_share, sh2.z);
+                    gv.w = gate_term_g<TERM, SHARES>(gate_term_plane<TERM>(t, tc, e + 3, planes_g), ov.w, gv.w, sh.w, has_share, sh2.w);
                 } else {
                     tp = gate_term_plane<TERM>(t, tc, (unsigned)p, planes_g);
-                    gv.x = gate_term_g<TERM>(tp, ov.x, gv.x, sh.x, has_share); gv.y = gate_term_g<TERM>(tp, ov.y, gv.y, sh.y, has_share);
-                    gv.z = gate_term_g<TERM>(tp, ov.z, gv.z, sh.z, has_share); gv.w = gate_term_g<TERM>(tp, ov.w, gv.w, sh.w, has_share);
+                    gv.x = gate_term_g<TERM, SHARES>(tp, ov.x, gv.x, sh.x, has_share, sh2.x);
+                    gv.y = gate_term_g<TERM, SHARES>(tp, ov.y, gv.y, sh.y, has_share, sh2.y);
+                    gv.z = gate_term_g<TERM, SHARES>(tp, ov.z, gv.z, sh.z, has_share, sh2.z);
+                    gv.w = gate_term_g<TERM, SHARES>(tp, ov.w, gv.w, sh.w, has_share, sh2.w);
                 }
             }
             const float4 xg = make_float4(xv.x * gv.x, xv.y * gv.y, xv.z * gv.z, xv.w * gv.w);
@@ -552,6 +645,8 @@
             if (a_per_plane) {
                 if (gate_gamma_finite(gm)) da_plane[p] = gm * sxg;
                 else if constexpr (TERM == GATE_TERM_NONE) da_plane[p] = gate_plane_da_nonfinite(x + p * hw, g + p * hw, hw, gm);
+                else if constexpr (SHARES == 3)
+                    da_plane[p] = gate_plane_da_nonfinite_term3<TERM>(x + p * hw, gs + p * hw, sp.ident, sp.conv, hw, gm, ap, tp);
                 else da_plane[p] = gate_plane_da_nonfinite_term<TERM>(x + p * hw, gs + p * hw, g + p * hw, hw, gm, ap, tp, has_share);
             }
         }
@@ -603,28 +698,33 @@
 }
 LOCATE_API int locate_gate_bwd_partials(int64_t planes, int hw) { return (int)gate_bwd_blocks(planes, hw); }
 
-template <int TERM>
+template <int TERM, int SHARES = 1>
 static void gate_bwd_launch(const float* x, const float* a, int a_per_plane, const float* gamma, const float* g, float* dx, float* da,
                             double* block_x2g, int64_t planes, int hw, int64_t blocks, int accumulate_dx, void* da_absmax,
-                            const LocateGateTerm& t, hipStream_t st) {
+                            const typename GateTermArg<SHARES>::type& tt, hipStream_t st) {
+    const LocateGateTerm& t = gate_norm_term(tt);
     const bool whole_block = hw >= 1024;
     uintptr_t bits = reinterpret_cast<uintptr_t>(x) | reinterpret_cast<uintptr_t>(g) | reinterpret_cast<uintptr_t>(dx) |
                      (a_per_plane ? 0 : (reinterpret_cast<uintptr_t>(a) | reinterpret_cast<uintptr_t>(da)));
     if (gate_term_is_norm(TERM)) bits |= reinterpret_cast<uintptr_t>(t.go);
+    if constexpr (SHARES == 3) {
+        bits |= reinterpret_cast<uintptr_t>(tt.conv);
+        if (planes == (int64_t)t.B * t.C) bits |= reinterpret_cast<uintptr_t>(tt.ident) | (uintptr_t)((tt.ident_bs & 3) << 2);
+    }
     const bool vec = (hw & 3) == 0 && (bits & 15) == 0;
     if constexpr (gate_term_is_norm(TERM)) {
         if (planes != (int64_t)t.B * t.C) {
             if (vec)
-                gate_bwd_small_kernel<16, TERM, true><<<(int)blocks, 256, 0, st>>>(x, a, gamma, g, dx, da, nullptr, block_x2g, planes, hw, 0,
-                                                                                  accumulate_dx, static_cast<unsigned*>(da_absmax), t);
+                gate_bwd_small_kernel<16, TERM, true, SHARES><<<(int)blocks, 256, 0, st>>>(x, a, gamma, g, dx, da, nullptr, block_x2g, planes, hw, 0,
+                                                                                          accumulate_dx, static_cast<unsigned*>(da_absmax), tt);
             else
-                gate_bwd_plane_kernel<1, TERM, true><<<(int)blocks, 256, 0, st>>>(x, a, gamma, g, dx, da, nullptr, block_x2g, planes, hw, 0,
-                                                                                 accumulate_dx, static_cast<unsigned*>(da_absmax), t);
+                gate_bwd_plane_kernel<1, TERM, true, SHARES><<<(int)blocks, 256, 0, st>>>(x, a, gamma, g, dx, da, nullptr, block_x2g, planes, hw, 0,
+                                                                                         accumulate_dx, static_cast<unsigned*>(da_absmax), tt);
             return;
         }
     }
-#define GATE_SMALL(LPV) gate_bwd_small_kernel<LPV, TERM><<<(int)blocks, 256, 0, st>>>(x, a, gamma, g, dx, a_per_plane ? nullptr : da, \
-        a_per_plane ? da : nullptr, block_x2g, planes, hw, a_per_plane, accumulate_dx, static_cast<unsigned*>(da_absmax), t)
+#define GATE_SMALL(LPV) gate_bwd_small_kernel<LPV, TERM, false, SHARES><<<(int)blocks, 256, 0, st>>>(x, a, gamma, g, dx, a_per_plane ? nullptr : da, \
+        a_per_plane ? da : nullptr, block_x2g, planes, hw, a_per_plane, accumulate_dx, static_cast<unsigned*>(da_absmax), tt)
     if (vec && hw <= 128) {
         const int q4 = hw >> 2;
         if (q4 <= 1) GATE_SMALL(1);
@@ -634,13 +734,13 @@
         else if (q4 <= 16) GATE_SMALL(16);
         else GATE_SMALL(32);
     } else if (whole_block)
-        gate_bwd_plane_kernel<4, TERM><<<(int)blocks, 256, 0, st>>>(x, a, gamma, g, dx, a_per_plane ? nullptr : da,
-                                                                   a_per_plane ? da : nullptr, block_x2g, planes, hw,
-                                                                   a_per_plane, accumulate_dx, static_cast<unsigned*>(da_absmax), t);
+        gate_bwd_plane_kernel<4, TERM, false, SHARES><<<(int)blocks, 256, 0, st>>>(x, a, gamma, g, dx, a_per_plane ? nullptr : da,
+                                                                                  a_per_plane ? da : nullptr, block_x2g, planes, hw,
+                                                                                  a_per_plane, accumulate_dx, static_cast<unsigned*>(da_absmax), tt);
     else
-        gate_bwd_plane_kernel<1, TERM><<<(int)blocks, 256, 0, st>>>(x, a, gamma, g, dx, a_per_plane ? nullptr : da,
-                                                                   a_per_plane ? da : nullptr, block_x2g, planes, hw,
-                                                                   a_per_plane, accumulate_dx, static_cast<unsigned*>(da_absmax), t);
+        gate_bwd_plane_kernel<1, TERM, false, SHARES><<<(int)blocks, 256, 0, st>>>(x, a, gamma, g, dx, a_per_plane ? nullptr : da,
+                                                                                  a_per_plane ? da : nullptr, block_x2g, planes, hw,
+                                                                                  a_per_plane, accumulate_dx, static_cast<unsigned*>(da_absmax), tt);
 #undef GATE_SMALL
 }
 
@@ -681,6 +781,35 @@
     return LOCATE_OK;
 }
 
+LOCATE_API int locate_gate_bwd_term3(const float* x, const float* a, int a_per_plane, const float* gamma, float* dx, float* da,
+                                     float* dgamma, int64_t planes, int hw, void* workspace, int accumulate_dx, void* da_absmax,
+                                     LocateGateTerm3 term, void* stream) {
+    const LocateGateTerm& nt = term.norm;
+    LOCATE_REQUIRE(planes > 0 && hw > 0 && workspace, "locate_gate_bwd_term3: bad shape or missing workspace");
+    LOCATE_REQUIRE(nt.kind == GATE_TERM_NORM, "locate_gate_bwd_term3: the term must be a norm, got %d", nt.kind);
+    LOCATE_REQUIRE(nt.go && nt.stats && nt.scale && nt.partial && nt.npartial > 0 && (!nt.with_act || nt.bias),
+                   "locate_gate_bwd_term3: the norm term needs go, stats, scale, the plane pass's partials (and the bias with_act)");
+    LOCATE_REQUIRE(nt.groups >= 1 && nt.groups <= NORM_MAX_GROUPS && nt.B > 0 && nt.C > 0 && nt.B % nt.groups == 0 &&
+                   (int64_t)nt.B * nt.C == planes && planes * hw < (1ll << 31), "locate_gate_bwd_term3: the norm's B x C must be the gate's planes");
+    LOCATE_REQUIRE(term.ident && term.conv && term.ident_bs >= (int64_t)nt.C * hw, "locate_gate_bwd_term3: missing share or bad batch stride");
+    double* block_x2g = static_cast<double*>(workspace);
+    const int64_t blocks = gate_bwd_blocks(planes, hw);
+    if (hw == 1 && (planes & 63) == 0) {
+        if (a_per_plane) { a_per_plane = 0; da_absmax = nullptr; }
+        planes >>= 6; hw = 64;
+    }
+    hipStream_t st = as_stream(stream);
+    if (nt.with_act)
+        gate_bwd_launch<GATE_TERM_NORM_ACT, 3>(x, a, a_per_plane, gamma, nullptr, dx, da, block_x2g, planes, hw, blocks, accumulate_dx, da_absmax, term, st);
+    else
+        gate_bwd_launch<GATE_TERM_NORM, 3>(x, a, a_per_plane, gamma, nullptr, dx, da, block_x2g, planes, hw, blocks, accumulate_dx, da_absmax, term, st);
+    LOCATE_LAUNCH_CHECK("locate_gate_bwd_term3(plane)");
+    if (!dgamma) return LOCATE_OK;
+    gate_bwd_final_kernel<<<1, 256, 0, st>>>(block_x2g, dgamma, (int)blocks);
+    LOCATE_LAUNCH_CHECK("locate_gate_bwd_term3(final)");
+    return LOCATE_OK;
+}
+
 LOCATE_API int locate_gate_bwd(const float* x, const float* a, int a_per_plane, const float* gamma, const float* g,
                                float* dx, float* da, float* dgamma, int64_t planes, int hw, void* workspace,
                                int accumulate_dx, void* da_absmax, void* stream) {
diff --git a/locate_amd/csrc/normterm.h b/locate_amd/csrc/normterm.h
--- a/locate_amd/csrc/normterm.h
+++ b/locate_amd/csrc/normterm.h
@@ -16,6 +16,13 @@
     int32_t npartial, B, C, groups;
 };
 enum { GATE_TERM_NONE = 0, GATE_TERM_NORM = 1, GATE_TERM_ROOTTANH = 2, GATE_TERM_NORM_ACT = 3  };
+
+struct LocateGateTerm3 {
+    LocateGateTerm norm;
+    const float* ident;
+    int64_t ident_bs;
+    const float* conv;
+};
 
 #ifdef __HIPCC__
 __device__ __forceinline__ float mul_pinned(float a, float b) {
diff --git a/locate_amd/csrc/runtime.hip b/locate_amd/csrc/runtime.hip
--- a/locate_amd/csrc/runtime.hip
+++ b/locate_amd/csrc/runtime.hip
@@ -13,7 +13,7 @@
 
 LOCATE_API const char* locate_last_error(void) { return g_last_error; }
 
-LOCATE_API int locate_abi_version(void) { return 21; }
+LOCATE_API int locate_abi_version(void) { return 22; }
 
 LOCATE_API int locate_device_info(char* arch_name, int name_len, int* cu_count, int* wave_size) {
     int dev = 0;
diff --git a/locate_amd/ops.py b/locate_amd/ops.py
--- a/locate_amd/ops.py
+++ b/locate_amd/ops.py
@@ -3,7 +3,7 @@
 
 import torch
 
-from ._lib import GateTerm, check, lib
+from ._lib import GateTerm, GateTerm3, check, lib
 
 _IntArr12 = ctypes.c_int * 12
 
@@ -20,6 +20,8 @@
 
 GATE_FOLD = [os.environ.get("LOCATE_GATE_FOLD", "1") != "0"]
 GATE_FOLD_ACT_MIN_NUMEL = [int(os.environ.get("LOCATE_GATE_FOLD_ACT_MIN", str(1 << 22)))]
+GATE_FOLD3 = [os.environ.get("LOCATE_GATE_FOLD3", "1") != "0"]
+GATE_FOLD3_MIN_NUMEL = [int(os.environ.get("LOCATE_GATE_FOLD3_MIN", "0"))]
 
 
 class ActLink:
@@ -617,11 +619,31 @@
 class Fork3Fn(torch.autograd.Function):
 
     @staticmethod
-    def forward(ctx, x):
+    def forward(ctx, x, slot=None):
+        ctx.slot = slot
         return x.view_as(x), x.view_as(x), x.view_as(x)
 
     @staticmethod
     def backward(ctx, g_identity, g_conv, g_norm):
+        slot, ctx.slot = ctx.slot, None
+        rec = None
+        if slot is not None:
+            rec, slot.deferred = slot.deferred, None
+        if rec is not None:
+            if g_norm is None or g_norm.data_ptr() != rec.buf.data_ptr():
+                rec.drop()
+                raise RuntimeError("fork3: the norm behind the third alias left its input gradient to the producing gate's backward "
+                                   "kernel, but what came back is not the buffer it handed over - the alias fed a further op")
+            if g_identity is None or g_conv is None or g_identity.shape != rec.buf.shape or g_conv.shape != rec.buf.shape:
+                rec.drop()
+                raise RuntimeError("fork3: the three-share gate backward needs the gradients of all three aliases")
+            ident = _chk(g_identity, "fork3 identity share")
+            if not _batch_strided(ident):
+                ident = ident.contiguous()
+            conv = _c(g_conv, "fork3 conv share")
+            rec.fields3 = dict(ident=_p(ident), ident_bs=ident.stride(0) if ident.shape[0] > 1 else ident[0].numel(), conv=_p(conv))
+            rec.keep = tuple(rec.keep) + (ident, conv)
+            return rec.buf, None
         gs = [g for g in (g_norm, g_identity, g_conv) if g is not None]
         if len(gs) == 3 and all(_batch_strided(g) for g in gs) and gs[0].shape == gs[1].shape == gs[2].shape:
             a, b, c = gs
@@ -629,11 +651,11 @@
             per = a[0].numel()
             check(lib().locate_add3(_p(a), a.stride(0), _p(b), b.stride(0), _p(c), c.stride(0), _p(out), a.shape[0], per, _stream()),
                   "locate_add3")
-            return out
+            return out, None
         total = None
         for g in gs:
             total = g if total is None else total + g
-        return total
+        return total, None
 
 
 def _batch_strided(g):
@@ -644,11 +666,29 @@
 def fork3(x):
     if not (torch.is_grad_enabled() and x.requires_grad):
         return x, x, x
-    a, b, c = Fork3Fn.apply(x)
+    token = _token_of(x) if (GATE_FOLD[0] and GATE_FOLD3[0] and x.is_cuda and x.is_contiguous()) else None
+    slot = _Fork3Slot() if token is not None else None
+    a, b, c = Fork3Fn.apply(x, slot)
     stats = getattr(x, "_locate_stats", None)
     if stats is not None:
         a._locate_stats = b._locate_stats = c._locate_stats = stats
+    if token is not None:
+        c._locate_fork3 = (slot, token)
     return a, b, c
+
+
+class _Fork3Slot:
+    __slots__ = ("deferred",)
+
+    def __init__(self):
+        self.deferred = None
+
+    def claim(self, like, shape=None):
+        return like.new_empty(tuple(like.shape if shape is None else shape)), 0
+
+    def claim_deferred(self, like, rec):
+        self.deferred = rec
+        return torch.empty_like(like)
 
 
 def _slot_of(x):
@@ -656,10 +696,11 @@
 
 
 class _FoldRecord:
-    __slots__ = ("kind", "buf", "keep", "fields", "has_share", "done", "token", "stream")
+    __slots__ = ("kind", "buf", "keep", "fields", "has_share", "done", "token", "stream", "fields3")
 
     def __init__(self, kind, buf, keep, **fields):
         self.kind, self.buf, self.keep, self.fields = kind, buf, keep, fields
+        self.fields3 = None
         self.has_share = False
         self.done = False
         self.token = None
@@ -672,6 +713,9 @@
 
     def term(self):
         return GateTerm(kind=self.kind, has_share=int(self.has_share), **self.fields)
+
+    def term3(self):
+        return GateTerm3(norm=GateTerm(kind=self.kind, has_share=0, **self.fields), **self.fields3)
 
 
 class _GateToken:
@@ -735,13 +779,18 @@
             ws = _ws(L.locate_norm_bwd_fused_workspace_bytes(B, C), x.device)
             dscale = torch.empty(ctx.scale_shape, dtype=torch.float32, device=x.device) if ctx.per_sample else None
             token = ctx.token
+            three = isinstance(ctx.slot, _Fork3Slot)
+            big_enough = (GATE_FOLD3[0] and x.numel() >= GATE_FOLD3_MIN_NUMEL[0]) if three else (
+                not ctx.with_act or x.numel() >= GATE_FOLD_ACT_MIN_NUMEL[0])
             if (token is not None and token.record is None and GATE_FOLD[0] and ctx.slot is not None and ctx.needs_input_grad[0]
-                    and token.rt.defer_finalisers and (not ctx.with_act or x.numel() >= GATE_FOLD_ACT_MIN_NUMEL[0])):
+                    and token.rt.defer_finalisers and big_enough):
                 check(L.locate_norm_bwd_planes(_p(x), _p(g), _p(stats), _p(scale), int(ctx.per_sample), _p(bias), int(ctx.with_act),
                                                _p(dscale), B, C, hw, ctx.groups, _p(ws), st), "locate_norm_bwd_planes")
                 rec = _FoldRecord(GateTerm.NORM, None, (g, stats, scale, bias, ws), with_act=int(ctx.with_act),
                                   per_sample=int(ctx.per_sample), go=_p(g), stats=_p(stats), scale=_p(scale), bias=_p(bias), partial=_p(ws),
                                   npartial=L.locate_norm_bwd_fused_partials(B, C), B=B, C=C, groups=ctx.groups)
+                if three:
+                    rec.fields3 = {}
                 dx = rec.buf = ctx.slot.claim_deferred(x, rec)
                 token.leave(rec)
             else:
@@ -773,6 +822,9 @@
     amax = AMAX.slot(x.device) if x.numel() >= AMAX_MIN_NUMEL[0] else None
     slot = _slot_of(x) if x.is_contiguous() else None
     token = _token_of(x) if (slot is not None and x.is_cuda) else None
+    three = getattr(x, "_locate_fork3", None)
+    if slot is None and three is not None and x.is_contiguous():
+        slot, token = three
     out = InPlaceNormFn.apply(x, scale, bias, with_act, groups, pre_partial, slot, amax, runtime, token)
     if amax is not None:
         _tag(out, amax)
@@ -836,8 +888,15 @@
             if rec.stream != _stream():
                 for t in rec.keep:
                     t.record_stream(torch.cuda.current_stream())
-            check(L.locate_gate_bwd_term(_p(x), _p(a), int(ctx.per_plane), _p(gamma), _p(g), _p(dx), _p(da), None if deferred else _p(dgamma),
-                                         planes, hw, _p(ws), acc, _p(amax), rec.term(), _stream()), "locate_gate_bwd_term")
+            if rec.fields3 is not None:
+                if not rec.fields3:
+                    raise RuntimeError("gate fold: the three-way fan-out behind the gate never added its two shares to the record")
+                check(L.locate_gate_bwd_term3(_p(x), _p(a), int(ctx.per_plane), _p(gamma), _p(dx), _p(da), None if deferred else _p(dgamma),
+                                              planes, hw, _p(ws), acc, _p(amax), rec.term3(), _stream()), "locate_gate_bwd_term3")
+            else:
+                check(L.locate_gate_bwd_term(_p(x), _p(a), int(ctx.per_plane), _p(gamma), _p(g), _p(dx), _p(da),
+                                             None if deferred else _p(dgamma), planes, hw, _p(ws), acc, _p(amax), rec.term(), _stream()),
+                      "locate_gate_bwd_term")
             rec.keep = rec.buf = None
         else:
             check(L.locate_gate_bwd(_p(x), _p(a), int(ctx.per_plane), _p(gamma), _p(g), _p(dx), _p(da), None if deferred else _p(dgamma),
```

Result: no change. 7333 images/sec, median of 6 (+0.7%).
